# hsinnan75/GSAlign

Measured on AMD Instinct MI355X. Metric: aligned query Gbp/s (whole node), higher is better.
Workload: dtype u8; 1 GPU; full-human-sized pair (BASELINE configs[4]): 24 contigs with GRCh38 chromosome lengths, 3.08 Gbp, repeat injection, vs 1; inflight_contexts_per_gpu=8, world_size=1, parallelism=one GPU

## Files before the change

gsalign_amd/csrc/gsa_api.hip:

```cpp
#include <algorithm>
#include <atomic>
#include <chrono>
#include <cstring>
#include <mutex>
#include <thread>
#include <pthread.h>
#include <sched.h>
#include "gsa_ctx.h"

static thread_local std::string g_create_error;

int gsa_fail(gsa_ctx *ctx, int code, const std::string &msg)
{
	if (ctx) ctx->err = msg; else g_create_error = msg;
	return code;
}

int host_stage4_5_6(gsa_ctx *c, int stage);
int host_stage8_finish(gsa_ctx *c);
int build_block_view(gsa_ctx *c);
void bundle_split_lists(gsa_ctx *c);
void bundle_join_lists(gsa_ctx *c);

void collect_events(gsa_ctx *c)
{
	if (!c->profiling && !c->prof_seed) { c->ev_pending = 0; return; }
	float ms;
	if ((c->ev_pending & 1) && !c->profiling) { if (hipEventElapsedTime(&ms, c->ev[0], c->ev[1]) == hipSuccess) { c->kernel_ms[0] = ms; c->acc_seed_ms += ms; } c->ev_pending = 0; (void)hipGetLastError(); return; }
	if (c->ev_pending & 1) {
		if (hipEventElapsedTime(&ms, c->ev[0], c->ev[1]) == hipSuccess) c->kernel_ms[0] = ms;
		if (hipEventElapsedTime(&ms, c->ev[1], c->ev[2]) == hipSuccess) c->kernel_ms[1] = ms;
		if (hipEventElapsedTime(&ms, c->ev[2], c->ev[3]) == hipSuccess) c->kernel_ms[2] = ms;
	}
	if (c->ev_pending & 2) { if (hipEventElapsedTime(&ms, c->ev[4], c->ev[5]) == hipSuccess) c->kernel_ms[3] = ms; }
	c->ev_pending = 0;
	(void)hipGetLastError();
}

void Uploader::run()
{
	(void)hipSetDevice(device);
	for (;;) {
		Job j;
		{ std::unique_lock<std::mutex> g(mu); cv.wait(g, [&] { return stop || !q.empty(); }); if (q.empty()) return; j = std::move(q.front()); q.pop_front(); if (n_demand > 0) n_demand--; }
		const auto t0 = std::chrono::steady_clock::now();
		hipError_t e_first = hipSuccess;
		for (const Piece &p : j.pieces) if (p.n) { const hipError_t e = hipMemcpyAsync(p.dst, p.src, p.n, hipMemcpyHostToDevice, st); if (e != hipSuccess && e_first == hipSuccess) e_first = e; bytes += p.n; }
		{ const hipError_t e = hipStreamSynchronize(st); if (e != hipSuccess && e_first == hipSuccess) e_first = e; }
		(void)hipGetLastError();
		if (e_first != hipSuccess && j.err) { int none = 0; j.err->compare_exchange_strong(none, (int)e_first); }
		const auto t1 = std::chrono::steady_clock::now();
		{ std::lock_guard<std::mutex> g(mu); copy_ms += std::chrono::duration<double, std::milli>(t1 - t0).count(); wait_ms += std::chrono::duration<double, std::milli>(t0 - j.t_push).count(); jobs++; }
		j.busy->fetch_sub(1, std::memory_order_release);
	}
}

static int uploader_start(gsa_ctx *c)
{
	Uploader *u = new Uploader(); u->device = c->device;
	if (hipStreamCreateWithFlags(&u->st, hipStreamNonBlocking) != hipSuccess) { delete u; return gsa_fail(c, GSA_ERR_HIP, "hipStreamCreate (upload stream)"); }
	u->th = std::thread([u] { u->run(); });
	c->up = u; c->own_up = true;
	return GSA_OK;
}

static void uploader_stop(gsa_ctx *c)
{
	if (!c->up || !c->own_up) { c->up = nullptr; return; }
	Uploader *u = c->up;
	{ std::lock_guard<std::mutex> g(u->mu); u->stop = true; }
	u->cv.notify_all();
	if (u->th.joinable()) u->th.join();
#ifdef GSA_EXPERIMENTS
	if (getenv("GSA_UP_STATS") && u->jobs) fprintf(stderr, "[uploader] %lld jobs, %.1f MB each, %.2f ms in the queue, %.2f ms copying (%.1f GB/s)\n", (long long)u->jobs, u->bytes / 1e6 / u->jobs, u->wait_ms / u->jobs, u->copy_ms / u->jobs, u->bytes / 1e6 / u->copy_ms);
#endif
	if (u->st) hipStreamDestroy(u->st);
	delete u; c->up = nullptr;
}

static inline void slot_wait(QuerySlot &s) { while (s.busy.load(std::memory_order_acquire) > 0) std::this_thread::yield(); }
static void slot_demand(gsa_ctx *c, QuerySlot &s)
{
	if (s.busy.load(std::memory_order_acquire) > 0 && c->up) {
		Uploader *u = c->up;
		std::lock_guard<std::mutex> g(u->mu);
		for (size_t k = u->n_demand; k < u->q.size(); k++) if (u->q[k].busy == &s.busy) {
			Uploader::Job j = std::move(u->q[k]); u->q.erase(u->q.begin() + (long)k); u->q.insert(u->q.begin() + (long)u->n_demand, std::move(j)); u->n_demand++;
			break;
		}
	}
	slot_wait(s);
}

static int ctx_private_init(gsa_ctx *c, gsa_ctx *share = nullptr)
{
#ifdef GSA_EXPERIMENTS
	static const int prio = [] { const char *e = getenv("GSA_STREAM_PRIO"); return e ? atoi(e) : 0; }();
	if (prio) {
		int lo = 0, hi = 0; GSA_CHECK(c, hipDeviceGetStreamPriorityRange(&lo, &hi));
		GSA_CHECK(c, hipStreamCreateWithPriority(&c->stream, hipStreamDefault, hi));
		for (int i = 0; i < 4; i++) GSA_CHECK(c, hipStreamCreateWithPriority(&c->stream_aux[i], hipStreamDefault, (i == 0 || i == 3 || (prio > 1 && i == 1)) ? lo : hi));
	} else
#endif
	if (c->prio_mode > 0) {
		int lo = 0, hi = 0; GSA_CHECK(c, hipDeviceGetStreamPriorityRange(&lo, &hi));
		const int mid = (lo + hi) / 2;
		GSA_CHECK(c, hipStreamCreateWithPriority(&c->stream, hipStreamDefault, hi));
		GSA_CHECK(c, hipStreamCreateWithPriority(&c->stream_seed, hipStreamDefault, c->prio_mode == 2 ? lo : mid));
		GSA_CHECK(c, hipEventCreateWithFlags(&c->ev_seed_fork, hipEventDisableTiming));
		for (int i = 0; i < 4; i++) GSA_CHECK(c, hipStreamCreateWithPriority(&c->stream_aux[i], hipStreamDefault, (c->prio_mode == 3 && (i == 0 || i == 3)) ? lo : mid));
	} else {
	GSA_CHECK(c, hipStreamCreate(&c->stream));
	for (int i = 0; i < 4; i++) GSA_CHECK(c, hipStreamCreate(&c->stream_aux[i]));
	}
	if (share) { c->up = share->up; c->own_up = false; } else if (int rc = uploader_start(c)) return rc;
	for (int i = 0; i < 28; i++) GSA_CHECK(c, hipEventCreate(&c->ev[i]));
	GSA_CHECK(c, hipMalloc(&c->d_zero.p, 256)); c->d_zero.cap = 256; GSA_CHECK(c, hipMemset(c->d_zero.p, 0, 256));
	GSA_CHECK(c, hipMalloc(&c->d_cnt.p, 32 * sizeof(u64))); c->d_cnt.cap = 32 * sizeof(u64); GSA_CHECK(c, hipMemset(c->d_cnt.p, 0, 32 * sizeof(u64)));
	GSA_CHECK(c, hipHostMalloc((void **)&c->h_cnt, 16 * sizeof(u64)));
	GSA_CHECK(c, hipMalloc(&c->d_mail.p, MAIL_N * sizeof(i32))); c->d_mail.cap = MAIL_N * sizeof(i32);
	GSA_CHECK(c, hipMemset(c->d_mail.p, 0, MAIL_N * sizeof(i32)));
	GSA_CHECK(c, hipHostMalloc((void **)&c->h_mail, MAIL_N * sizeof(i32)));
	return GSA_OK;
}

static hipError_t h2d_big(void *dst, const void *src, size_t bytes)
{
	if (bytes >= ((size_t)64 << 20) && hipHostRegister(const_cast<void *>(src), bytes, hipHostRegisterDefault) == hipSuccess) {
		const hipError_t e = hipMemcpy(dst, src, bytes, hipMemcpyHostToDevice);
		(void)hipHostUnregister(const_cast<void *>(src));
		return e;
	}
	(void)hipGetLastError();
	return hipMemcpy(dst, src, bytes, hipMemcpyHostToDevice);
}

struct ReservedBuf { void *p = nullptr; size_t bytes = 0; };
static std::mutex g_res_mu; static ReservedBuf g_res[64][2];
void *dev_take_reserved(int device, size_t bytes, size_t *got)
{
	std::lock_guard<std::mutex> g(g_res_mu);
	for (int k = 0; k < 2; k++) { ReservedBuf &r = g_res[device & 63][k]; if (r.p && r.bytes >= bytes && r.bytes <= bytes + bytes / 8 + 4096) { void *p = r.p; *got = r.bytes; r.p = nullptr; r.bytes = 0; return p; } }
	return nullptr;
}

extern "C" {

void gsa_default_params(gsa_params *p)
{
	p->min_seed_len = 15; p->max_indel = 25; p->min_block_score = 200; p->min_aln_len = 200; p->min_identity = 70;
	p->sensitive = 0; p->one_on_one = 0;
}

const char *gsa_last_error(gsa_ctx *ctx) { return ctx ? ctx->err.c_str() : g_create_error.c_str(); }

static int reset_run_state(gsa_ctx *c)
{
	if (c->early_in_flight) { GSA_CHECK(c, hipStreamSynchronize(c->stream_aux[0])); c->early_in_flight = false; }
	c->n_early = 0; c->early_listed = false; c->early_consumed = false;
	c->stage = 0; c->split = false; c->b_lists.clear();
	c->n_seeds = 0; c->n_groups = 0; c->n_blocks2 = 0; c->blocks.clear(); c->frags_stage = 0; c->have_host_seeds = false; c->ev_pending = 0; c->s2_host = false;
	memset(c->counters, 0, sizeof(c->counters)); memset(c->kernel_ms, 0, sizeof(c->kernel_ms));
	return GSA_OK;
}

int gsa_set_params(gsa_ctx *c, const gsa_params *p)
{
	if (!c || !p) return GSA_ERR_ARG;
	if (p->min_seed_len < 1 || p->max_indel < 0) return gsa_fail(c, GSA_ERR_ARG, "bad parameter");
	GSA_CHECK(c, hipSetDevice(c->device));
	if (c->n_borrowers.load() > 0 && (p->sensitive ? 10 : p->min_seed_len) != c->prm.MinSeedLength)
		return gsa_fail(c, GSA_ERR_STATE, "gsa_set_params: contexts cloned from this one read its seed tables -- change -slen / -sen on the clones, or destroy them first");
	if (int rc = reset_run_state(c)) return rc;
	c->prm.MinSeedLength = p->sensitive ? 10 : p->min_seed_len;
	c->prm.MaxIndelSize = p->max_indel; c->prm.MinAlnBlockScore = p->min_block_score; c->prm.MinAlnLength = p->min_aln_len;
	c->prm.MinSeqIdy = p->min_identity; c->prm.bSensitive = p->sensitive ? 1 : 0; c->prm.OneOnOne = p->one_on_one ? 1 : 0;
	return build_presence(c);
}

int gsa_create(int device, const gsa_index_view *idx, const gsa_params *prm, gsa_ctx **out)
{
	return gsa_create_opts(device, idx, prm, 0u, out);
}

int gsa_create_opts(int device, const gsa_index_view *idx, const gsa_params *prm, uint32_t flags, gsa_ctx **out)
{
	if (!idx || !out || !idx->bwt || !idx->sa || !idx->ref || !idx->chr_len || idx->n_chr <= 0 || idx->G <= 0) return gsa_fail(nullptr, GSA_ERR_ARG, "gsa_create: bad index view");
	if (idx->L2[4] != (uint64_t)(2 * idx->G)) return gsa_fail(nullptr, GSA_ERR_ARG, "gsa_create: L2[4] != 2G");
	int ndev = 0;
	if (hipGetDeviceCount(&ndev) != hipSuccess || ndev <= 0) return gsa_fail(nullptr, GSA_ERR_HIP, "no HIP device available (libgsa_hip.so has no CPU path)");
	if (device < 0 || device >= ndev) return gsa_fail(nullptr, GSA_ERR_ARG, "gsa_create: bad device ordinal");
	if (flags & ~(uint32_t)(GSA_CREATE_WIDE | GSA_CREATE_KMER_K(15) | GSA_CREATE_PRIO(3) | GSA_CREATE_REF_PAC)) return gsa_fail(nullptr, GSA_ERR_ARG, "gsa_create_opts: unknown flag");
	{ const uint32_t kk = (flags >> 8) & 15u; if (kk == 1) return gsa_fail(nullptr, GSA_ERR_ARG, "gsa_create_opts: GSA_CREATE_KMER_K takes 2 .. 15 (0: chosen by text length and free memory)"); }
	gsa_ctx *c = new gsa_ctx();
	c->device = device; c->force_wide = (flags & GSA_CREATE_WIDE) != 0; c->opt.kmer_k = (int)((flags >> 8) & 15u); c->prio_mode = (int)((flags >> 16) & 3u);
	memset(c->kernel_ms, 0, sizeof(c->kernel_ms)); memset(c->counters, 0, sizeof(c->counters));
#define CK(call) do { hipError_t e_ = (call); if (e_ != hipSuccess) { gsa_fail(nullptr, GSA_ERR_HIP, std::string(#call) + ": " + hipGetErrorString(e_)); gsa_destroy(c); return GSA_ERR_HIP; } } while (0)
	CK(hipSetDevice(device));
	(void)hipSetDeviceFlags(hipDeviceScheduleSpin);
	(void)hipGetLastError();
	if (int rcp = ctx_private_init(c)) { g_create_error = c->err; gsa_destroy(c); return rcp; }
	const size_t bwt_bytes = ((idx->bwt_words + 15) / 16) * 64;
	CK(hipMalloc(&c->d_bwt_ref.p, bwt_bytes + 64)); c->d_bwt_ref.cap = bwt_bytes + 64;
	CK(hipMemset(c->d_bwt_ref.p, 0, bwt_bytes + 64));
	CK(h2d_big(c->d_bwt_ref.p, idx->bwt, idx->bwt_words * 4));
	CK(hipMalloc(&c->d_sa.p, idx->n_sa * 8)); c->d_sa.cap = idx->n_sa * 8;
	CK(h2d_big(c->d_sa.p, idx->sa, idx->n_sa * 8));
	CK(hipMalloc(&c->d_ref.p, (size_t)2 * idx->G + 64)); c->d_ref.cap = (size_t)2 * idx->G + 64;
	if (flags & GSA_CREATE_REF_PAC) {
		const size_t pac_bytes = ((size_t)idx->G + 3) / 4;
		void *d_pac = nullptr;
		CK(hipMalloc(&d_pac, pac_bytes + 64));
		if (h2d_big(d_pac, idx->ref, pac_bytes) != hipSuccess) { hipFree(d_pac); gsa_fail(nullptr, GSA_ERR_HIP, "hipMemcpy (.pac)"); gsa_destroy(c); return GSA_ERR_HIP; }
		const int rcu = unpack_pac(c, (const uint8_t *)d_pac, idx->G, (uint8_t *)c->d_ref.p);
		(void)hipStreamSynchronize(c->stream); hipFree(d_pac);
		if (rcu) { g_create_error = c->err; gsa_destroy(c); return rcu; }
	} else
	CK(h2d_big(c->d_ref.p, idx->ref, (size_t)2 * idx->G));
	c->G = idx->G;
	{
		i64 tot = 0; std::vector<std::pair<i64, i32> > ends;
		for (int i = 0; i < idx->n_chr; i++) {
			c->h_chr_len.push_back(idx->chr_len[i]); c->h_chr_fwd.push_back(tot); tot += idx->chr_len[i];
			ends.push_back(std::make_pair(c->h_chr_fwd[i] + idx->chr_len[i] - 1, i));
			ends.push_back(std::make_pair(2 * idx->G - tot + idx->chr_len[i] - 1, i));
		}
		if (tot != idx->G) { gsa_fail(nullptr, GSA_ERR_ARG, "gsa_create: sum(chr_len) != G"); gsa_destroy(c); return GSA_ERR_ARG; }
		std::sort(ends.begin(), ends.end());
		for (size_t i = 0; i < ends.size(); i++) { c->h_chr_end.push_back(ends[i].first); c->h_chr_of_end.push_back(ends[i].second); }
	}
	c->d_chr_end.cap = c->h_chr_end.size() * 8; c->d_chr_of_end.cap = c->h_chr_of_end.size() * 4;
	CK(hipMalloc(&c->d_chr_end.p, c->h_chr_end.size() * 8)); CK(hipMemcpy(c->d_chr_end.p, c->h_chr_end.data(), c->h_chr_end.size() * 8, hipMemcpyHostToDevice));
	CK(hipMalloc(&c->d_chr_of_end.p, c->h_chr_of_end.size() * 4)); CK(hipMemcpy(c->d_chr_of_end.p, c->h_chr_of_end.data(), c->h_chr_of_end.size() * 4, hipMemcpyHostToDevice));
#undef CK
	c->di.primary = idx->primary; for (int i = 0; i < 5; i++) c->di.L2[i] = idx->L2[i]; c->di.L2[0] = 0;
	c->di.seq_len = idx->L2[4];
	c->di.bwt = nullptr; c->di.occ_base = nullptr; c->di.occ_shift = 0; c->di.sa = c->d_sa.as<u64>(); c->di.ref = c->d_ref.as<uint8_t>(); c->di.G = idx->G;
	c->di.chr_end = c->d_chr_end.as<i64>(); c->di.chr_of_end = c->d_chr_of_end.as<i32>(); c->di.n_ends = (i32)c->h_chr_end.size();
	c->di.sa32 = nullptr; c->di.sa64 = nullptr; c->di.kmer = nullptr; c->di.kmer_k = 0; c->di.kmer_lo = nullptr; c->di.kmer_lo_k = 0; c->di.kmer_e16 = 0; c->di.ref2 = nullptr; c->di.pres = nullptr; c->di.pres_k = 0;
	{
		const int rco = build_occ(c, c->d_bwt_ref.p, bwt_bytes / 64);
		hipFree(c->d_bwt_ref.p); c->d_bwt_ref.p = nullptr; c->d_bwt_ref.cap = 0;
		if (rco) { g_create_error = c->err; gsa_destroy(c); return rco; }
	}
	if (int rcd = build_dense_sa(c, idx->n_sa)) { g_create_error = c->err; gsa_destroy(c); return rcd; }
	gsa_params dp; gsa_default_params(&dp);
	int rc = gsa_set_params(c, prm ? prm : &dp);
	if (rc) { g_create_error = c->err; gsa_destroy(c); return rc; }
	gsa_release_reserved(device);
	if (const unsigned long long ov = gsa_take_grid_overflow()) { gsa_fail(nullptr, GSA_ERR_LIMIT, "gsa_create: a table build needed a launch of " + std::to_string(ov) + " work-items (>= 2^32)"); gsa_destroy(c); return GSA_ERR_LIMIT; }
	*out = c;
	return GSA_OK;
}

#define GSA_DEVBUFS(X) X(d_bwt) X(d_bwt_ref) X(d_occ_base) X(d_sa) X(d_ref) X(d_chr_end) X(d_chr_of_end) X(qs[0].d_query) X(qs[1].d_query) X(qs[0].d_bndtab) X(qs[1].d_bndtab) X(tmp) X(d_cnt) X(d_zero) X(d_mail) X(d_lb_status[0]) X(d_lb_status[1]) X(d_sa_dense) X(d_kmer) X(d_kmer_lo) X(d_pres) X(d_ref2) X(d_cand_s) X(d_cand_len) X(d_cand_x0) X(d_cand_freq) X(d_onpath) X(d_cand_cnt) X(d_heavy) X(dn_lf) X(dn_x0) X(d_chunk_hits) X(d_chunk_base) X(d_key_a) X(d_key_b) X(d_val_a) X(d_val_b) X(s_q) X(s_len) X(s_r) X(s_gid) X(d_flag) X(d_scan) X(g_beg) X(w_j0) X(d_pdbm) X(d_pdby) X(d_pdcb) X(d_gpre) X(d_key_c) X(d_val_c) X(a_q) X(a_len) X(a_r) X(a_gb) X(a_ge) X(a_uniq) X(a_cu) X(a_alive) X(a_ws) X(a_wid) X(a_next) X(a_brk) X(a_aurank) X(a_aulist) X(a_runinfo) X(w_best) X(w_sum) X(w_n) X(d_btab) X(d_flag2) X(d_scan2) X(d_i64a) X(b_q) X(b_len) X(b_r) X(b_gb) X(b_ge) X(c_q) X(c_len) X(c_r) X(c_gb) X(c_ge) X(c_bid) X(blk_beg) X(blk_end) X(blk_score) X(r_q) X(r_len) X(r_r) X(r_bid) X(r_tmp_q) X(r_tmp_len) X(r_tmp_r) X(r_tmp_bid) X(r_cut4) X(r_cut5) X(r_simjob) X(r_simres) X(d_leaf) X(fb_seedbase) X(fb_sbeg) X(fb_fragbase) X(f_rec) X(f_rec16) X(f_type) X(f_mism) X(f_alnlen) X(f_job) X(f_score) X(d_dp_tiny) X(d_dp_bnd) X(d_dp_ctr) X(d_dp_jobs) X(d_dp_large) X(d_tail) X(e_id) X(e_rec) X(e_list) X(e_off1) X(e_off2) X(e_opsoff) X(e_nops) X(e_ops) X(e_rev) X(r_head) X(f_early) X(r_orig) X(r_tmp_orig) X(j_frag) X(j_opsoff) X(j_nops) X(d_ops) X(j_cells) X(d_alnoff) X(bl_alnlen) X(bl_score) X(d_bblk) X(d_dp_arena) X(leaf[0]) X(leaf[1]) X(leaf[2]) X(leaf[3]) X(leaf[4]) X(leaf[5]) X(leaf[6]) X(leaf[7]) X(leaf[8])
void gsa_destroy(gsa_ctx *c)
{
	if (!c) return;
	hipSetDevice(c->device);
	if (c->stream) hipStreamSynchronize(c->stream);
	for (int i = 0; i < 2; i++) slot_wait(c->qs[i]);
	uploader_stop(c);
	if (c->lender) c->lender->n_borrowers.fetch_sub(1);
#define X(n) &c->n,
	DevBuf *bufs[] = { GSA_DEVBUFS(X) };
#undef X
	for (DevBuf *b : bufs) if (b->p) hipFree(b->p);
	if (c->h_cnt) hipHostFree(c->h_cnt);
	if (c->h_mail) hipHostFree(c->h_mail);
	for (DevBuf *b : { &c->p_frags, &c->p_tail, &c->p_leaf, &c->p_blk, &c->p_dp, &c->p_sj, &c->p_sj_early, &c->p_jpatch, &c->p_early, &c->qs[0].p_bndtab, &c->qs[1].p_bndtab, &c->p_bblk, &c->p_ba0 }) if (b->p) hipHostFree(b->p);
	for (int i = 0; i < 28; i++) if (c->ev[i]) hipEventDestroy(c->ev[i]);
	for (int i = 0; i < 4; i++) if (c->stream_aux[i]) hipStreamDestroy(c->stream_aux[i]);
	if (c->stream_seed) hipStreamDestroy(c->stream_seed);
	if (c->ev_seed_fork) hipEventDestroy(c->ev_seed_fork);
	if (c->stream) hipStreamDestroy(c->stream);
	delete c;
}

int gsa_clone(gsa_ctx *parent, gsa_ctx **out)
{
	if (!parent || !out) return GSA_ERR_ARG;
	if (hipSetDevice(parent->device) != hipSuccess) return gsa_fail(nullptr, GSA_ERR_HIP, "hipSetDevice");
	gsa_ctx *c = new gsa_ctx();
	c->device = parent->device; c->force_wide = parent->force_wide; c->prio_mode = parent->prio_mode;
	c->index_owner = parent->index_owner ? parent->index_owner : parent; c->seed_budget = parent->seed_budget; c->opt = parent->opt;
	memset(c->kernel_ms, 0, sizeof(c->kernel_ms)); memset(c->counters, 0, sizeof(c->counters));
	if (int rc = ctx_private_init(c, c->index_owner)) { g_create_error = c->err; gsa_destroy(c); return rc; }
	c->di = parent->di; c->G = parent->G;
	c->lender = parent; parent->n_borrowers.fetch_add(1);
	c->h_chr_end = parent->h_chr_end; c->h_chr_fwd = parent->h_chr_fwd; c->h_chr_of_end = parent->h_chr_of_end; c->h_chr_len = parent->h_chr_len;
	c->prm = parent->prm;
	*out = c;
	return GSA_OK;
}

int gsa_clone_to_device(gsa_ctx *parent, int device, gsa_ctx **out)
{
	if (!parent || !out) return GSA_ERR_ARG;
	int ndev = 0;
	if (hipGetDeviceCount(&ndev) != hipSuccess || device < 0 || device >= ndev) { (void)hipGetLastError(); return gsa_fail(nullptr, GSA_ERR_ARG, "gsa_clone_to_device: bad device ordinal"); }
	gsa_ctx *own = parent->index_owner ? parent->index_owner : parent;
	if (hipSetDevice(parent->device) != hipSuccess) return gsa_fail(nullptr, GSA_ERR_HIP, "hipSetDevice");
	if (hipStreamSynchronize(parent->stream) != hipSuccess || hipStreamSynchronize(own->stream) != hipSuccess) return gsa_fail(nullptr, GSA_ERR_HIP, "gsa_clone_to_device: the parent's stream");
	if (hipSetDevice(device) != hipSuccess) return gsa_fail(nullptr, GSA_ERR_HIP, "hipSetDevice");
	(void)hipSetDeviceFlags(hipDeviceScheduleSpin); (void)hipGetLastError();
	gsa_ctx *c = new gsa_ctx();
	c->device = device; c->force_wide = parent->force_wide; c->prio_mode = parent->prio_mode; c->seed_budget = parent->seed_budget; c->opt = parent->opt;
	memset(c->kernel_ms, 0, sizeof(c->kernel_ms)); memset(c->counters, 0, sizeof(c->counters));
	if (int rc = ctx_private_init(c)) { g_create_error = c->err; gsa_destroy(c); return rc; }
	struct Pair { const DevBuf *src; DevBuf *dst; };
	std::vector<Pair> tab = { { &own->d_bwt, &c->d_bwt }, { &own->d_occ_base, &c->d_occ_base }, { &own->d_sa, &c->d_sa }, { &own->d_ref, &c->d_ref }, { &own->d_chr_end, &c->d_chr_end },
		{ &own->d_chr_of_end, &c->d_chr_of_end }, { &own->d_sa_dense, &c->d_sa_dense }, { &own->d_kmer, &c->d_kmer }, { &own->d_ref2, &c->d_ref2 } };
	for (gsa_ctx *src = parent; src; src = src->lender) {
		if (!c->d_pres.cap && src->d_pres.p && (const void *)parent->di.pres == src->d_pres.p) { tab.push_back({ &src->d_pres, &c->d_pres }); c->d_pres.cap = 1; }
		if (!c->d_kmer_lo.cap && src->d_kmer_lo.p && (const void *)parent->di.kmer_lo == src->d_kmer_lo.p) { tab.push_back({ &src->d_kmer_lo, &c->d_kmer_lo }); c->d_kmer_lo.cap = 1; }
	}
	c->d_pres.cap = c->d_kmer_lo.cap = 0;
	auto fail = [&](int code, const std::string &m) { gsa_fail(nullptr, code, m); gsa_destroy(c); return code; };
	for (const Pair &t : tab) {
		if (!t.src->p) continue;
		const size_t bytes = t.src->len ? t.src->len : t.src->cap;
		if (bytes == 0) return fail(GSA_ERR_STATE, "gsa_clone_to_device: an index table of unknown size");
		if (hipMalloc(&t.dst->p, bytes + 256) != hipSuccess) { (void)hipGetLastError(); return fail(GSA_ERR_NOMEM, "gsa_clone_to_device: hipMalloc of an index table"); }
		t.dst->cap = bytes + 256; t.dst->len = bytes;
		const hipError_t e = (device == own->device) ? hipMemcpyAsync(t.dst->p, t.src->p, bytes, hipMemcpyDeviceToDevice, c->stream)
		                                             : hipMemcpyPeerAsync(t.dst->p, device, t.src->p, own->device, bytes, c->stream);
		if (e != hipSuccess) return fail(GSA_ERR_HIP, std::string("gsa_clone_to_device: device-to-device copy: ") + hipGetErrorString(e));
	}
	c->di = parent->di;
	auto move_ptr = [&](const void *p) -> const void * {
		if (!p) return nullptr;
		for (const Pair &t : tab) if (t.src->p && (const char *)p >= (const char *)t.src->p && (const char *)p < (const char *)t.src->p + (t.src->len ? t.src->len : t.src->cap)) return (const char *)t.dst->p + ((const char *)p - (const char *)t.src->p);
		return (const void *)~(uintptr_t)0;
	};
	bool lost = false;
#define MOVE(field, T) do { const void *q_ = move_ptr((const void *)c->di.field); if (q_ == (const void *)~(uintptr_t)0) lost = true; c->di.field = (T)q_; } while (0)
	MOVE(bwt, const uint4 *); MOVE(occ_base, const u64 *); MOVE(sa, const u64 *); MOVE(sa32, const u32 *); MOVE(sa64, const u64 *); MOVE(ref, const uint8_t *); MOVE(ref2, const u32 *);
	MOVE(chr_end, const i64 *); MOVE(chr_of_end, const i32 *); MOVE(kmer, const u64 *); MOVE(kmer_lo, const u64 *); MOVE(pres, const u32 *);
#undef MOVE
	if (lost) return fail(GSA_ERR_STATE, "gsa_clone_to_device: an index pointer outside the tables of its owner");
	c->G = parent->G;
	c->h_chr_end = parent->h_chr_end; c->h_chr_fwd = parent->h_chr_fwd; c->h_chr_of_end = parent->h_chr_of_end; c->h_chr_len = parent->h_chr_len;
	c->prm = parent->prm;
	if (hipStreamSynchronize(c->stream) != hipSuccess) return fail(GSA_ERR_HIP, "gsa_clone_to_device: waiting for the copies");
	*out = c;
	return GSA_OK;
}

static bool device_local_cpus(int device, cpu_set_t *set)
{
	char bus[64] = { 0 };
	if (hipDeviceGetPCIBusId(bus, (int)sizeof(bus) - 1, device) != hipSuccess) { (void)hipGetLastError(); return false; }
	for (char *p = bus; *p; p++) if (*p >= 'A' && *p <= 'Z') *p = (char)(*p - 'A' + 'a');
	char path[160]; snprintf(path, sizeof(path), "/sys/bus/pci/devices/%s/local_cpulist", bus);
	FILE *f = fopen(path, "r"); if (!f) return false;
	char line[4096]; const bool got = fgets(line, sizeof(line), f) != nullptr; fclose(f);
	if (!got) return false;
	CPU_ZERO(set); int n = 0;
	for (char *p = line; *p;) {
		while (*p == ',' || *p == ' ' || *p == '\n') p++;
		if (!*p) break;
		char *e; long a = strtol(p, &e, 10), b = a; if (e == p) break;
		if (*e == '-') { p = e + 1; b = strtol(p, &e, 10); if (e == p) break; }
		for (long k = a; k <= b && k < CPU_SETSIZE; k++) { CPU_SET((int)k, set); n++; }
		p = e;
	}
	return n > 0;
}
int gsa_reserve_index(int device, uint64_t seq_len, uint32_t flags)
{
	int ndev = 0;
	if (hipGetDeviceCount(&ndev) != hipSuccess || device < 0 || device >= ndev || seq_len == 0) { (void)hipGetLastError(); return GSA_ERR_ARG; }
	if (hipSetDevice(device) != hipSuccess) return GSA_ERR_HIP;
	const bool wide = (flags & GSA_CREATE_WIDE) != 0 || seq_len >= 0xFFFFFFF0ull;
	size_t want[2];
	want[0] = ((size_t)seq_len + 1 + 32) * (wide ? 8 : 4) + 256;
	{
		int k = 0; while ((1ull << (2 * k)) < seq_len) k++;
		k += 2; if (k > 15) k = 15;
		size_t fr = 0, tot = 0; if (hipMemGetInfo(&fr, &tot) != hipSuccess) { (void)hipGetLastError(); fr = 8ull << 30; }
		const size_t esz = wide ? 32 : 16;
		while (k > 2 && ((size_t)esz << (2 * k)) > fr / 4) k--;
		const int kk = (int)((flags >> 8) & 15u); if (kk >= 2 && kk <= 15 && ((size_t)esz << (2 * kk)) <= fr / 2) k = kk;
		want[1] = k >= 2 ? ((size_t)esz << (2 * k)) : 0;
	}
	gsa_release_reserved(device);
	for (int k = 0; k < 2; k++) {
		if (!want[k]) continue;
		void *p = nullptr;
		if (hipMalloc(&p, want[k]) != hipSuccess) { (void)hipGetLastError(); continue; }
		std::lock_guard<std::mutex> g(g_res_mu);
		g_res[device & 63][k].p = p; g_res[device & 63][k].bytes = want[k];
	}
	return GSA_OK;
}
void gsa_release_reserved(int device)
{
	void *f[2] = { nullptr, nullptr };
	{ std::lock_guard<std::mutex> g(g_res_mu); for (int k = 0; k < 2; k++) { f[k] = g_res[device & 63][k].p; g_res[device & 63][k].p = nullptr; g_res[device & 63][k].bytes = 0; } }
	if (f[0] || f[1]) { (void)hipSetDevice(device); for (int k = 0; k < 2; k++) if (f[k]) hipFree(f[k]); }
}

int gsa_bind_host_thread(int device)
{
	cpu_set_t set;
	if (!device_local_cpus(device, &set)) return GSA_OK;
	(void)pthread_setaffinity_np(pthread_self(), sizeof(set), &set);
	return GSA_OK;
}

void *gsa_host_alloc(size_t bytes)
{
	void *p = nullptr;
	if (hipHostMalloc(&p, bytes ? bytes : 1) != hipSuccess) { (void)hipGetLastError(); return nullptr; }
	return p;
}
void gsa_host_free(void *p) { if (p) (void)hipHostFree(p); }
int gsa_host_register(void *p, size_t bytes)
{
	if (!p || !bytes) return GSA_ERR_ARG;
	if (hipHostRegister(p, bytes, hipHostRegisterDefault) != hipSuccess) { (void)hipGetLastError(); return GSA_ERR_HIP; }
	return GSA_OK;
}
int gsa_host_unregister(void *p)
{
	if (!p) return GSA_ERR_ARG;
	if (hipHostUnregister(p) != hipSuccess) { (void)hipGetLastError(); return GSA_ERR_HIP; }
	return GSA_OK;
}

int gsa_set_option(gsa_ctx *c, const char *name, int64_t value)
{
	if (!c || !name) return GSA_ERR_ARG;
	const std::string k(name);
	auto in = [&](int64_t lo, int64_t hi) { return value >= lo && value <= hi; };
	const int64_t BIG = (int64_t)1 << 40;
	if (k == "split_min") { if (!in(0, BIG)) return gsa_fail(c, GSA_ERR_ARG, "split_min: 0 .. 2^40 bases"); c->opt.split_min = value; }
	else if (k == "bundle_contig") { if (!in(0, BIG)) return gsa_fail(c, GSA_ERR_ARG, "bundle_contig: 0 (no bundles) .. 2^40 bases"); c->opt.bundle_contig = value; }
	else if (k == "bundle_cap") { if (!in(1, BIG)) return gsa_fail(c, GSA_ERR_ARG, "bundle_cap: 1 .. 2^40 bases"); c->opt.bundle_cap = value; }
	else if (k == "seed_budget") { if (!in(1, 0xffffffffll)) return gsa_fail(c, GSA_ERR_ARG, "seed_budget: 1 .. 2^32 - 1 wave-iterations"); c->seed_budget = (u32)value; }
	else if (k == "dp_lane") { if (!in(0, 1 << 20)) return gsa_fail(c, GSA_ERR_ARG, "dp_lane: 0 (round 2's tiny / small split) .. 2^20 cells"); c->opt.dp_lane = (int)value; }
	else if (k == "seed_mode") { if (value < 0 || value > 2) return gsa_fail(c, GSA_ERR_ARG, "seed_mode: 0 sweep, 1 speculative, 2 search"); c->opt.seed_mode = (int)value; }
	else if (k == "pd_bitmap") c->opt.pd_bitmap = value != 0;
	else if (k == "dp_side") c->opt.dp_side = value != 0;
	else if (k == "dp_small_side") c->opt.dp_small_side = value != 0;
	else if (k == "pd_two_level_min") { if (!in(0, BIG)) return gsa_fail(c, GSA_ERR_ARG, "pd_two_level_min: >= 0 blocks"); c->opt.pd_two_level_min = value; }
	else if (k == "dp_occupancy") { if (!in(0, 16)) return gsa_fail(c, GSA_ERR_ARG, "dp_occupancy: 0 (off) .. 16 workgroups per CU"); c->opt.dp_occupancy = (int)value; }
	else if (k == "pd_bytes") { if (!in(0, 2)) return gsa_fail(c, GSA_ERR_ARG, "pd_bytes: 0 never, 1 by the hit count, 2 always"); c->opt.pd_bytes = (int)value; }
	else if (k == "pres_from_kmer") c->opt.pres_from_kmer = value != 0;
	else if (k == "walk_chain_min") { if (!in(0, BIG)) return gsa_fail(c, GSA_ERR_ARG, "walk_chain_min: >= 0 seeds"); c->opt.walk_chain_min = value; }
	else if (k == "sweep_shape") { if (value < -1 || value > 1) return gsa_fail(c, GSA_ERR_ARG, "sweep_shape: -1, 0 or 1"); c->opt.sweep_shape = (int)value; }
	else if (k == "dp_safe") c->dp_safe = value != 0;
	else if (k == "dp_fake_timeout") { if (!in(0, 1 << 20)) return gsa_fail(c, GSA_ERR_ARG, "dp_fake_timeout: >= 0"); c->dp_fake_timeout = (int)value; }
	else return gsa_fail(c, GSA_ERR_ARG, "gsa_set_option: unknown option " + k);
	return GSA_OK;
}

int gsa_get_wall_sums(gsa_ctx *c, double ms[10], int64_t *n)
{
	if (!c || !ms || !n) return GSA_ERR_ARG;
	memcpy(ms, c->wall_ms, sizeof(c->wall_ms)); *n = c->wall_n;
	if (c->up && c->own_up) { std::lock_guard<std::mutex> g(c->up->mu); ms[9] = c->up->jobs ? c->up->copy_ms / (double)c->up->jobs * (double)c->wall_n : 0.0; }
	return GSA_OK;
}

int gsa_get_alloc_stats(gsa_ctx *c, double *ms, int64_t *n, int64_t *bytes)
{
	if (!c) return GSA_ERR_ARG;
	if (ms) *ms = c->alloc_ms; if (n) *n = c->alloc_n; if (bytes) *bytes = c->alloc_bytes;
	return GSA_OK;
}
int gsa_debug_buffers(gsa_ctx *c, int top)
{
	if (!c) return GSA_ERR_ARG;
	struct E { const char *name; size_t cap, len; };
	std::vector<E> v;
#define X(n) if (c->n.p) v.push_back({ #n, c->n.cap, c->n.len });
	GSA_DEVBUFS(X)
#undef X
	std::sort(v.begin(), v.end(), [](const E &a, const E &b) { return a.cap > b.cap; });
	size_t tot = 0; for (const E &e : v) tot += e.cap;
	fprintf(stderr, "[gsa_debug_buffers] %zu device buffers, %.2f GB held\n", v.size(), (double)tot / 1e9);
	for (size_t k = 0; k < v.size() && (int)k < top; k++) fprintf(stderr, "  %-16s %10.1f MB held  %10.1f MB asked\n", v[k].name, (double)v[k].cap / 1e6, (double)v[k].len / 1e6);
	return GSA_OK;
}
int gsa_set_profiling(gsa_ctx *c, int enable) { if (!c) return GSA_ERR_ARG; c->acc_seed_ms = 0.0; memset(c->wall_ms, 0, sizeof(c->wall_ms)); c->wall_n = 0; if (c->up && c->own_up) { std::lock_guard<std::mutex> g(c->up->mu); c->up->copy_ms = c->up->wait_ms = c->up->bytes = 0; c->up->jobs = 0; } c->profiling = (enable & 1) != 0; c->count_blocks = (enable & 2) != 0; c->prof_seed = (enable & 4) != 0; return GSA_OK; }

static int query_geometry(gsa_ctx *c, int32_t qlen)
{
	c->qlen = qlen;
	c->bnd.n = 0; c->bnd.lmax = qlen; c->bnd.pds = 0; c->bnd.off = (const i32 *)c->d_zero.p; c->bnd.chunk_contig = (const uint16_t *)c->d_zero.p;
	c->qbits = ceil_log2_u64((u64)qlen + 1); if (c->qbits < 1) c->qbits = 1;
	c->pd_span = 2 * c->G + (i64)qlen + 2;
	c->pdbits = ceil_log2_u64((u64)c->pd_span);
	if (c->qbits + c->pdbits > 64) return gsa_fail(c, GSA_ERR_LIMIT, "contig too long for the 64-bit seed key");
	return GSA_OK;
}

#define GSA_BUNDLE_MAX_CONTIGS 4096
static void *slot_ensure_bytes(gsa_ctx *c, DevBuf &b, size_t bytes, bool pinned)
{
	if (bytes && bytes <= b.cap) return b.p;
	return pinned ? (void *)pin_ensure<uint8_t>(c, b, bytes) : (void *)dev_ensure<uint8_t>(c, b, bytes);
}

static int slot_layout(gsa_ctx *c, QuerySlot &s, const char *const *query, const int32_t *qlen, int32_t n)
{
	s.b_off.assign((size_t)n + 1, 0); s.b_qlen.assign(qlen, qlen + n); s.src.assign(query, query + n);
	i64 tot = 0; i32 lmax = 0;
	for (int k = 0; k < n; k++) {
		if (qlen[k] < 0 || (qlen[k] > 0 && !query[k])) return GSA_ERR_ARG;
		s.b_off[(size_t)k] = (i32)tot;
		tot += ((i64)qlen[k] + GSA_CHUNK - 1) / GSA_CHUNK * GSA_CHUNK;
		if (tot >= (1ll << 31) - 2 * GSA_CHUNK) return gsa_fail(c, GSA_ERR_LIMIT, "bundle longer than 2^31 bases");
		if (qlen[k] > lmax) lmax = qlen[k];
	}
	s.b_off[(size_t)n] = (i32)tot; s.tot = tot; s.lmax = lmax; s.n = n;
	return GSA_OK;
}

__global__ void __launch_bounds__(256) k_bundle_pad(const i32 *__restrict__ off, const i32 *__restrict__ len, uint8_t *dst)
{
	const i32 k = blockIdx.x; const i64 b = (i64)off[k] + len[k], e = off[k + 1];
	for (i64 t = b + threadIdx.x; t < e; t += 256) dst[t] = (uint8_t)'N';
}

static int slot_upload(gsa_ctx *c, QuerySlot &s, const char *const *query, const int32_t *qlen, int32_t n)
{
	slot_wait(s);
	s.up_err.store(0);
	Uploader::Job job; job.busy = &s.busy; job.err = &s.up_err;
	if (n == 0) {
		s.n = 0; s.tot = qlen[0]; s.lmax = qlen[0]; s.src.assign(1, query[0]); s.b_qlen.assign(1, qlen[0]); s.b_off.clear();
		if (!slot_ensure_bytes(c, s.d_query, (size_t)qlen[0] + 64, false)) return GSA_ERR_NOMEM;
		size_t nb = (size_t)qlen[0];
#ifdef GSA_EXPERIMENTS
		{ static const long long cap = [] { const char *e = getenv("GSA_X_UPBYTES"); return e ? atoll(e) : -1ll; }(); if (cap >= 0 && (size_t)cap < nb) nb = (size_t)cap; }
#endif
		if (nb > 0) { job.pieces.push_back({ s.d_query.p, query[0], nb }); c->up->push(std::move(job)); }
		return GSA_OK;
	}
	if (int rc = slot_layout(c, s, query, qlen, n)) return rc;
	const i64 n_chunks = s.tot / GSA_CHUNK;
	s.o_cc = ((size_t)n + 1) * 4; s.o_src = (s.o_cc + (size_t)n_chunks * 2 + 15) & ~(size_t)15;
	const size_t t_bytes = s.o_src + (size_t)n * 4;
	if (!slot_ensure_bytes(c, s.p_bndtab, t_bytes + 16, true) || !slot_ensure_bytes(c, s.d_bndtab, t_bytes + 16, false) || !slot_ensure_bytes(c, s.d_query, (size_t)s.tot + 64, false)) return GSA_ERR_NOMEM;
	uint8_t *ht = s.p_bndtab.as<uint8_t>();
	memcpy(ht, s.b_off.data(), s.o_cc);
	{ uint16_t *cc = (uint16_t *)(ht + s.o_cc); for (int k = 0; k < n; k++) for (i64 ch = s.b_off[(size_t)k] / GSA_CHUNK; ch < s.b_off[(size_t)k + 1] / GSA_CHUNK; ch++) cc[ch] = (uint16_t)k; }
	memcpy(ht + s.o_src, qlen, (size_t)n * 4);
	job.pieces.push_back({ s.d_bndtab.p, ht, t_bytes });
	for (int k = 0; k < n; k++) if (qlen[k] > 0) job.pieces.push_back({ s.d_query.as<uint8_t>() + s.b_off[(size_t)k], query[k], (size_t)qlen[k] });
	c->up->push(std::move(job));
	return GSA_OK;
}

static int slot_finish(gsa_ctx *c, QuerySlot &s)
{
	slot_demand(c, s);
	if (const int e = s.up_err.exchange(0)) return gsa_fail(c, GSA_ERR_HIP, std::string("query upload (hipMemcpyAsync H2D): ") + hipGetErrorString((hipError_t)e));
	if (s.n > 0 && s.tot > 0) {
		const uint8_t *dt = s.d_bndtab.as<uint8_t>();
		hipLaunchKernelGGL(k_bundle_pad, dim3((unsigned)s.n), dim3(256), 0, c->stream, (const i32 *)dt, (const i32 *)(dt + s.o_src), s.d_query.as<uint8_t>());
		GSA_CHECK(c, hipGetLastError());
	}
	return GSA_OK;
}

static bool slot_holds(const QuerySlot &s, const char *const *query, const int32_t *qlen, int32_t n)
{
	if (!s.pending || s.n != n) return false;
	const int32_t m = n ? n : 1;
	if ((int32_t)s.src.size() != m || (int32_t)s.b_qlen.size() != m) return false;
	for (int32_t k = 0; k < m; k++) if (s.src[(size_t)k] != query[k] || s.b_qlen[(size_t)k] != qlen[k]) return false;
	return true;
}

static int slot_acquire(gsa_ctx *c, const char *const *query, const int32_t *qlen, int32_t n, int *which)
{
	for (int i = 0; i < 2; i++) if (slot_holds(c->qs[i], query, qlen, n)) {
		c->qs[i].pending = false; *which = i;
		return slot_finish(c, c->qs[i]);
	}
	int i = (c->q_cur == 1 && !c->qs[1].pending) ? 1 : 0;
	if (c->qs[i].pending) i ^= 1;
	if (c->qs[i].pending) return gsa_fail(c, GSA_ERR_STATE, "both query slots hold prefetched contigs: align them (or gsa_cancel_prefetch) first");
	*which = i;
	if (int rc = slot_upload(c, c->qs[i], query, qlen, n)) return rc;
	return slot_finish(c, c->qs[i]);
}

static int prefetch(gsa_ctx *c, const char *const *query, const int32_t *qlen, int32_t n)
{
	GSA_CHECK(c, hipSetDevice(c->device));
	int i = c->q_cur == 0 ? 1 : 0;
	if (c->qs[i].pending) i ^= 1;
	if (c->qs[i].pending) return gsa_fail(c, GSA_ERR_STATE, "gsa_prefetch: two contigs are waiting already");
	if (i == c->q_cur && c->stage > 0 && c->stage < 8) return gsa_fail(c, GSA_ERR_STATE, "gsa_prefetch: the free query slot holds the contig whose stages are still running (finish it with gsa_run_to(8) or gsa_set_query first)");
	if (i == c->q_cur) c->q_cur = -2;
	int rc = slot_upload(c, c->qs[i], query, qlen, n);
	if (rc == GSA_OK) c->qs[i].pending = true;
	return rc;
}

int gsa_prefetch_contig(gsa_ctx *c, const char *query, int32_t qlen)
{
	if (!c || !query || qlen < 0) return GSA_ERR_ARG;
	return prefetch(c, &query, &qlen, 0);
}

int gsa_prefetch_bundle(gsa_ctx *c, const char *const *query, const int32_t *qlen, int32_t n)
{
	if (!c || !query || !qlen) return GSA_ERR_ARG;
	if (n < 1 || n > GSA_BUNDLE_MAX_CONTIGS) return gsa_fail(c, GSA_ERR_ARG, "gsa_prefetch_bundle: 1 .. 4096 contigs");
	return prefetch(c, query, qlen, n);
}

int gsa_cancel_prefetch(gsa_ctx *c)
{
	if (!c) return GSA_ERR_ARG;
	if (!c->qs[0].pending && !c->qs[1].pending) return GSA_OK;
	c->qs[0].pending = c->qs[1].pending = false;
	return GSA_OK;
}

int gsa_set_query(gsa_ctx *c, const char *query, int32_t qlen)
{
	if (!c || !query || qlen < 0) return GSA_ERR_ARG;
	GSA_CHECK(c, hipSetDevice(c->device));
	if (int rc = reset_run_state(c)) return rc;
	int w = 0;
	const auto t0 = std::chrono::steady_clock::now();
	if (int rc = slot_acquire(c, &query, &qlen, 0, &w)) return rc;
	c->wall_ms[0] += std::chrono::duration<double, std::milli>(std::chrono::steady_clock::now() - t0).count();
	c->q_cur = w; c->q_dev = c->qs[w].d_query.as<uint8_t>();
	return query_geometry(c, qlen);
}

int gsa_set_query_device(gsa_ctx *c, const char *d_query, int32_t qlen)
{
	if (!c || !d_query || qlen < 0) return GSA_ERR_ARG;
	if (((uintptr_t)d_query & 15) != 0) return gsa_fail(c, GSA_ERR_ARG, "gsa_set_query_device: the buffer must be 16-byte aligned");
	GSA_CHECK(c, hipSetDevice(c->device));
	hipPointerAttribute_t at;
	if (hipPointerGetAttributes(&at, d_query) != hipSuccess || at.type != hipMemoryTypeDevice || at.device != c->device) { (void)hipGetLastError(); return gsa_fail(c, GSA_ERR_ARG, "gsa_set_query_device: not a device buffer of this context's GPU"); }
	if (int rc = reset_run_state(c)) return rc;
	c->q_dev = (const uint8_t *)d_query; c->q_cur = -1;
	return query_geometry(c, qlen);
}

void *gsa_device_alloc(int device, size_t bytes)
{
	void *p = nullptr;
	if (hipSetDevice(device) != hipSuccess || hipMalloc(&p, (bytes ? bytes : 1) + 64) != hipSuccess) { (void)hipGetLastError(); return nullptr; }
	return p;
}
void gsa_device_free(int device, void *p) { if (p && hipSetDevice(device) == hipSuccess) (void)hipFree(p); }
int gsa_device_upload(int device, void *dst, const void *src, size_t bytes)
{
	if (!dst || (!src && bytes)) return GSA_ERR_ARG;
	if (hipSetDevice(device) != hipSuccess || hipMemcpy(dst, src, bytes, hipMemcpyHostToDevice) != hipSuccess) { (void)hipGetLastError(); return GSA_ERR_HIP; }
	return GSA_OK;
}

static int rewind_to_hits(gsa_ctx *c)
{
	const i64 n_seeds = c->n_seeds; const i32 n_groups = c->n_groups;
	if (int rc = reset_run_state(c)) return rc;
	GSA_CHECK(c, hipStreamSynchronize(c->stream));
	c->n_seeds = n_seeds; c->n_groups = n_groups; c->counters[2] = c->counters[3] = (u64)n_seeds;
	c->stage = 1;
	return stage1_restore_pdbm(c);
}

int gsa_rewind(gsa_ctx *c)
{
	if (!c) return GSA_ERR_ARG;
	if (c->qlen <= 0) return gsa_fail(c, GSA_ERR_STATE, "gsa_set_query first");
	if (c->q_cur == -2) return gsa_fail(c, GSA_ERR_STATE, "gsa_rewind: the contig's device copy was overwritten by a prefetch");
	GSA_CHECK(c, hipSetDevice(c->device));
	return reset_run_state(c);
}

int gsa_run_to(gsa_ctx *c, int stage)
{
	if (!c || stage < 0 || stage > 8) return GSA_ERR_ARG;
	if (c->bnd.n && stage < 8 && !c->bundle_call) return gsa_fail(c, GSA_ERR_STATE, "gsa_run_to: the context holds a bundle (gsa_align_bundle runs it); gsa_set_query first");
	if (c->split) return gsa_fail(c, GSA_ERR_STATE, "gsa_run_to: a split contig is finished with gsa_finish_contig");
	GSA_CHECK(c, hipSetDevice(c->device));
	int rc = GSA_OK;
	auto t_prev = std::chrono::steady_clock::now();
	while (c->stage < stage && rc == GSA_OK) {
		const int next = c->stage + 1;
		switch (next) {
		case 1: rc = stage1_seed(c); break;
		case 2: rc = stage2_chain(c); break;
		case 3: rc = stage345_refine(c); if (rc == GSA_OK && c->bnd.n) bundle_split_lists(c); break;
		case 4: case 5: case 6: rc = host_stage4_5_6(c, next); break;
		case 7: if (c->bnd.n) bundle_join_lists(c); rc = stage7_fill(c); break;
		case 8: rc = stage78_extend(c); if (rc == GSA_OK) rc = host_stage8_finish(c); break;
		}
		if (rc == GSA_OK) { c->stage = next; c->frags_stage = (next == 8) ? 8 : 0; }
		{ const auto t_now = std::chrono::steady_clock::now(); c->wall_ms[next] += std::chrono::duration<double, std::milli>(t_now - t_prev).count(); t_prev = t_now; }
	}
	if (stage == 8) c->wall_n++;
	if (const unsigned long long ov = gsa_take_grid_overflow()) rc = gsa_fail(c, GSA_ERR_LIMIT, "a kernel launch of " + std::to_string(ov) + " work-items (>= 2^32) was needed: contig too large for this build");
	if (rc == GSA_OK) { GSA_CHECK(c, hipStreamSynchronize(c->stream)); collect_events(c); }
	if (c->early_in_flight && (rc != GSA_OK || !c->early_consumed)) GSA_CHECK(c, hipStreamSynchronize(c->stream_aux[0]));
	return rc;
}

static int align_uploaded(gsa_ctx *c, gsa_result *out);
int gsa_align_contig(gsa_ctx *c, const char *query, int32_t qlen, gsa_result *out)
{
	if (!c || !out) return GSA_ERR_ARG;
	int rc = gsa_set_query(c, query, qlen); if (rc) return rc;
	return align_uploaded(c, out);
}
int gsa_align_contig_device(gsa_ctx *c, const char *d_query, int32_t qlen, gsa_result *out)
{
	if (!c || !out) return GSA_ERR_ARG;
	int rc = gsa_set_query_device(c, d_query, qlen); if (rc) return rc;
	return align_uploaded(c, out);
}
static int align_uploaded(gsa_ctx *c, gsa_result *out)
{
	int rc;
	c->dp_timeout = false;
	rc = gsa_run_to(c, 8);
	if (rc == GSA_ERR_STATE && c->dp_timeout && !c->dp_safe) {
		c->dp_timeout = false; c->dp_safe = true;
		rc = gsa_rewind(c);
		if (rc == GSA_OK) rc = gsa_run_to(c, 8);
		c->dp_safe = false;
	}
	if (rc) return rc;
	return gsa_get_blocks(c, out);
}

struct BundleSrc { const uint8_t *p; i32 len, _pad; };
__global__ void __launch_bounds__(256) k_bundle_gather(const i32 *__restrict__ off, const uint16_t *__restrict__ chunk_contig, const BundleSrc *__restrict__ src, uint8_t *dst)
{
	const i32 chunk = blockIdx.x, ci = chunk_contig[chunk];
	const i64 g0 = (i64)chunk * GSA_CHUNK; const i32 l0 = (i32)(g0 - off[ci]);
	const BundleSrc sc = src[ci];
	const i32 have = sc.len - l0 < GSA_CHUNK ? sc.len - l0 : GSA_CHUNK;
	for (i32 t = threadIdx.x; t < GSA_CHUNK; t += 256) dst[g0 + t] = t < have ? sc.p[l0 + t] : (uint8_t)'N';
}

static int set_query_bundle(gsa_ctx *c, const char *const *query, const int32_t *qlen, int32_t n, bool dev_q)
{
	if (n < 1 || n > GSA_BUNDLE_MAX_CONTIGS) return gsa_fail(c, GSA_ERR_ARG, "gsa_align_bundle: 1 .. 4096 contigs");
	GSA_CHECK(c, hipSetDevice(c->device));
	if (int rc = reset_run_state(c)) return rc;
	int w = 0;
	if (!dev_q) { if (int rc = slot_acquire(c, query, qlen, n, &w)) return rc; }
	else {
		w = (c->q_cur == 1 && !c->qs[1].pending) ? 1 : 0;
		if (c->qs[w].pending) w ^= 1;
		if (c->qs[w].pending) return gsa_fail(c, GSA_ERR_STATE, "both query slots hold prefetched contigs");
		QuerySlot &s = c->qs[w];
		slot_wait(s);
		for (int k = 0; k < n; k++) if (qlen[k] > 0) {
			hipPointerAttribute_t at;
			if (!query[k] || hipPointerGetAttributes(&at, query[k]) != hipSuccess || at.type != hipMemoryTypeDevice || at.device != c->device) { (void)hipGetLastError(); return gsa_fail(c, GSA_ERR_ARG, "gsa_align_bundle (GSA_MANY_DEVICE): not a device buffer of this context's GPU"); }
		}
		if (int rc = slot_layout(c, s, query, qlen, n)) return rc;
		const i64 n_chunks = s.tot / GSA_CHUNK;
		s.o_cc = ((size_t)n + 1) * 4; s.o_src = (s.o_cc + (size_t)n_chunks * 2 + 15) & ~(size_t)15;
		const size_t t_bytes = s.o_src + (size_t)n * sizeof(BundleSrc);
		if (!slot_ensure_bytes(c, s.p_bndtab, t_bytes + 16, true) || !slot_ensure_bytes(c, s.d_bndtab, t_bytes + 16, false) || !slot_ensure_bytes(c, s.d_query, (size_t)s.tot + 64, false)) return GSA_ERR_NOMEM;
		uint8_t *ht = s.p_bndtab.as<uint8_t>();
		memcpy(ht, s.b_off.data(), s.o_cc);
		{ uint16_t *cc = (uint16_t *)(ht + s.o_cc); for (int k = 0; k < n; k++) for (i64 ch = s.b_off[(size_t)k] / GSA_CHUNK; ch < s.b_off[(size_t)k + 1] / GSA_CHUNK; ch++) cc[ch] = (uint16_t)k; }
		{ BundleSrc *bs = (BundleSrc *)(ht + s.o_src); for (int k = 0; k < n; k++) { bs[k].p = (const uint8_t *)query[k]; bs[k].len = qlen[k]; bs[k]._pad = 0; } }
		GSA_CHECK(c, hipMemcpyAsync(s.d_bndtab.p, ht, t_bytes, hipMemcpyHostToDevice, c->stream));
		const uint8_t *dt = s.d_bndtab.as<uint8_t>();
		if (s.tot > 0) {
			hipLaunchKernelGGL(k_bundle_gather, dim3((unsigned)n_chunks), dim3(256), 0, c->stream, (const i32 *)dt, (const uint16_t *)(dt + s.o_cc), (const BundleSrc *)(dt + s.o_src), s.d_query.as<uint8_t>());
			GSA_CHECK(c, hipGetLastError());
		}
	}
	const QuerySlot &s = c->qs[w];
	c->q_cur = w; c->b_off = s.b_off; c->b_qlen = s.b_qlen;
	const uint8_t *dt = s.d_bndtab.as<uint8_t>();
	c->q_dev = s.d_query.as<uint8_t>();
	c->qlen = (i32)s.tot;
	c->bnd.n = n; c->bnd.lmax = s.lmax; c->bnd.off = (const i32 *)dt; c->bnd.chunk_contig = (const uint16_t *)(dt + s.o_cc);
	c->bnd.pds = (2 * c->G + (i64)s.lmax + (i64)c->prm.MaxIndelSize + 64 + 31) & ~31ll;
	c->qbits = ceil_log2_u64((u64)s.tot + 1); if (c->qbits < 1) c->qbits = 1;
	c->pd_span = (i64)n * c->bnd.pds + 2;
	c->pdbits = ceil_log2_u64((u64)c->pd_span);
	if (c->qbits + c->pdbits > 64) return gsa_fail(c, GSA_ERR_LIMIT, "bundle too long for the 64-bit seed key");
	return GSA_OK;
}

static void bundle_result(gsa_ctx *c, int k, const std::vector<i64> &a0, size_t blk_at, gsa_result *out)
{
	out->n_blocks = c->b_nblk[(size_t)k]; out->blocks = c->h_blocks.data() + blk_at;
	out->n_frags = c->b_frag0[(size_t)k + 1] - c->b_frag0[(size_t)k]; out->recs = c->p_frags.as<gsa_rec>() + c->b_frag0[(size_t)k];
	out->n_aln = a0[(size_t)k + 1] - a0[(size_t)k]; out->aln1 = c->h_taln1 + a0[(size_t)k]; out->aln2 = c->h_taln2 + a0[(size_t)k];
}

int gsa_align_bundle(gsa_ctx *c, const char *const *query, const int32_t *qlen, int32_t n, uint32_t flags, gsa_result *out)
{
	if (!c || !query || !qlen || !out || (flags & ~(uint32_t)GSA_MANY_DEVICE)) return GSA_ERR_ARG;
	int rc = set_query_bundle(c, query, qlen, n, (flags & GSA_MANY_DEVICE) != 0); if (rc) return rc;
	c->dp_timeout = false;
	c->bundle_call = true;
	struct Clear { gsa_ctx *c; ~Clear() { c->bundle_call = false; } } clear_{ c };
	rc = gsa_run_to(c, 8);
	if (rc == GSA_ERR_STATE && c->dp_timeout && !c->dp_safe) {
		c->dp_timeout = false; c->dp_safe = true;
		{ const Bundle keep = c->bnd; rc = reset_run_state(c); c->bnd = keep; }
		if (rc == GSA_OK) rc = gsa_run_to(c, 8);
		c->dp_safe = false;
	}
	if (rc) return rc;
	const size_t nfb = c->b_blk0.empty() ? 0 : (size_t)c->b_blk0[(size_t)n];
	if (nfb == 0 || c->n_frags == 0) {
		for (int k = 0; k < n; k++) { out[k].n_blocks = 0; out[k].n_frags = 0; out[k].n_aln = 0; out[k].blocks = nullptr; out[k].recs = nullptr; out[k].aln1 = out[k].aln2 = nullptr; }
		return GSA_OK;
	}
	std::vector<i64> a0((size_t)n + 1, c->n_aln);
	for (int k = n - 1; k >= 0; k--) a0[(size_t)k] = c->b_blk0[(size_t)k] < c->b_blk0[(size_t)k + 1] ? c->p_ba0.as<i64>()[k] : a0[(size_t)k + 1];
	size_t at = 0;
	for (int k = 0; k < n; k++) { bundle_result(c, k, a0, at, &out[k]); at += (size_t)c->b_nblk[(size_t)k]; }
	return GSA_OK;
}

int gsa_seed_chunks(gsa_ctx *c, const char *query, int32_t qlen, int32_t chunk_beg, int32_t chunk_end)
{
	if (!c || chunk_beg < 0 || chunk_end < chunk_beg) return GSA_ERR_ARG;
	int rc = gsa_set_query(c, query, qlen); if (rc) return rc;
	c->split = true; c->rng_beg = chunk_beg; c->rng_end = chunk_end;
	rc = stage1_seed(c);
	if (rc == GSA_OK) GSA_CHECK(c, hipStreamSynchronize(c->stream));
	collect_events(c);
	return rc;
}

int64_t gsa_hit_count(gsa_ctx *c) { return (c && c->split) ? c->n_seeds : 0; }

int gsa_export_hits(gsa_ctx *c, uint64_t *keys, uint32_t *vals)
{
	if (!c || !c->split) return c ? gsa_fail(c, GSA_ERR_STATE, "gsa_seed_chunks first") : GSA_ERR_ARG;
	if (c->n_seeds == 0) return GSA_OK;
	if (!keys || !vals) return GSA_ERR_ARG;
	GSA_CHECK(c, hipSetDevice(c->device));
	GSA_CHECK(c, hipMemcpyAsync(keys, c->d_key_a.p, (size_t)c->n_seeds * 8, hipMemcpyDefault, c->stream));
	GSA_CHECK(c, hipMemcpyAsync(vals, c->d_val_a.p, (size_t)c->n_seeds * 4, hipMemcpyDefault, c->stream));
	GSA_CHECK(c, hipStreamSynchronize(c->stream));
	return GSA_OK;
}

int gsa_import_hits(gsa_ctx *c, const uint64_t *keys, const uint32_t *vals, int64_t n)
{
	if (!c || n < 0 || (n > 0 && (!keys || !vals))) return GSA_ERR_ARG;
	if (!c->split || c->stage != 0) return gsa_fail(c, GSA_ERR_STATE, "gsa_seed_chunks first");
	GSA_CHECK(c, hipSetDevice(c->device));
	return stage1_import_hits(c, (const u64 *)keys, (const u32 *)vals, n);
}

int gsa_finish_contig(gsa_ctx *c, gsa_result *out)
{
	if (!c || !out) return GSA_ERR_ARG;
	if (!c->split || c->stage != 0) return gsa_fail(c, GSA_ERR_STATE, "gsa_seed_chunks first");
	GSA_CHECK(c, hipSetDevice(c->device));
	int rc = stage1_finish_split(c); if (rc) return rc;
	c->stage = 1; c->split = false;
	c->dp_timeout = false;
	rc = gsa_run_to(c, 8);
	if (rc == GSA_ERR_STATE && c->dp_timeout && !c->dp_safe) {
		c->dp_timeout = false; c->dp_safe = true;
		rc = rewind_to_hits(c);
		if (rc == GSA_OK) rc = gsa_run_to(c, 8);
		c->dp_safe = false;
	}
	if (rc) return rc;
	return gsa_get_blocks(c, out);
}

int gsa_hit_buffers(gsa_ctx *c, const uint64_t **keys, const uint32_t **vals)
{
	if (!c || !keys || !vals) return GSA_ERR_ARG;
	if (!c->split) return gsa_fail(c, GSA_ERR_STATE, "gsa_seed_chunks first");
	*keys = c->d_key_a.as<uint64_t>(); *vals = c->d_val_a.as<uint32_t>();
	return GSA_OK;
}

static int align_split(gsa_ctx *const *grp, int n_grp, const char *query, int32_t qlen, gsa_result *out)
{
	const int32_t n_chunks = (int32_t)(((int64_t)qlen + GSA_CHUNK - 1) / GSA_CHUNK);
	std::vector<int> rcs((size_t)n_grp, GSA_OK);
	std::vector<std::thread> th;
	auto range = [&](int k, int32_t &b, int32_t &e) { const int32_t base = n_chunks / n_grp, extra = n_chunks % n_grp; b = k * base + (k < extra ? k : extra); e = b + base + (k < extra ? 1 : 0); };
	for (int k = 1; k < n_grp; k++) th.emplace_back([&, k] { int32_t b, e; range(k, b, e); rcs[(size_t)k] = gsa_seed_chunks(grp[k], query, qlen, b, e); });
	{ int32_t b, e; range(0, b, e); rcs[0] = gsa_seed_chunks(grp[0], query, qlen, b, e); }
	for (std::thread &t : th) t.join();
	for (int k = 0; k < n_grp; k++) if (rcs[(size_t)k] != GSA_OK) { if (k) gsa_fail(grp[0], rcs[(size_t)k], std::string("helper context: ") + gsa_last_error(grp[k])); return rcs[(size_t)k]; }
	for (int k = 1; k < n_grp; k++) {
		const uint64_t *kp = nullptr; const uint32_t *vp = nullptr;
		int rc = gsa_hit_buffers(grp[k], &kp, &vp);
		if (rc == GSA_OK) rc = gsa_import_hits(grp[0], kp, vp, gsa_hit_count(grp[k]));
		if (rc != GSA_OK) return rc;
	}
	return gsa_finish_contig(grp[0], out);
}

int gsa_align_many(gsa_ctx *const *ctx, int32_t n_ctx, const char *const *query, const int32_t *qlen, int32_t n, uint32_t flags, gsa_result_fn on_result, void *user)
{
	if (flags & ~(uint32_t)(GSA_MANY_IN_ORDER | GSA_MANY_DEVICE | GSA_MANY_NO_SPLIT | GSA_MANY_NO_BUNDLE | GSA_MANY_NO_PREFETCH)) return GSA_ERR_ARG;
	if (!ctx || n_ctx <= 0 || n < 0 || (n > 0 && (!query || !qlen))) return GSA_ERR_ARG;
	for (int k = 0; k < n_ctx; k++) if (!ctx[k]) return GSA_ERR_ARG;
	const bool dev_q = (flags & GSA_MANY_DEVICE) != 0;
	if (dev_q) for (int k = 1; k < n_ctx; k++) if (ctx[k]->device != ctx[0]->device) return gsa_fail(ctx[0], GSA_ERR_ARG, "GSA_MANY_DEVICE: the contexts must share one GPU (the contigs live in its memory)");
	if (n == 0) return GSA_OK;
	std::vector<int32_t> order((size_t)n);
	for (int32_t i = 0; i < n; i++) order[(size_t)i] = i;
	if (!(flags & GSA_MANY_IN_ORDER)) std::stable_sort(order.begin(), order.end(), [&](int32_t a, int32_t b) { return qlen[a] > qlen[b]; });
	std::atomic<int> err(GSA_OK);
	const int64_t split_min = ctx[0]->opt.split_min;
	int64_t longest = 0; for (int32_t i = 0; i < n; i++) if (qlen[i] > longest) longest = qlen[i];
	if (n < n_ctx && !dev_q && !(flags & GSA_MANY_NO_SPLIT) && longest >= split_min) {
		std::vector<int> gsz((size_t)n, 1);
		for (int left = n_ctx - n; left > 0; left--) {
			int best = -1; double load = 0;
			for (int i = 0; i < n; i++) { const int32_t ci = order[(size_t)i]; if ((int64_t)qlen[ci] < split_min) continue; const double l = (double)qlen[ci] / gsz[(size_t)i]; if (l > load) { load = l; best = i; } }
			if (best < 0) break;
			gsz[(size_t)best]++;
		}
		std::vector<std::thread> th; int at = 0;
		for (int i = 0; i < n; i++) {
			const int32_t ci = order[(size_t)i]; gsa_ctx *const *grp = ctx + at; const int ng = gsz[(size_t)i]; at += ng;
			th.emplace_back([&, ci, grp, ng] {
				gsa_result res;
				int rc = ng > 1 ? align_split(grp, ng, query[ci], qlen[ci], &res) : gsa_align_contig(grp[0], query[ci], qlen[ci], &res);
				if (rc == GSA_OK && on_result) rc = on_result(user, ci, &res);
				if (rc != GSA_OK) { int ok = GSA_OK; err.compare_exchange_strong(ok, rc); }
			});
		}
		for (std::thread &t : th) t.join();
		return err.load();
	}
	const int64_t bundle_contig = ctx[0]->opt.bundle_contig, bundle_cap = ctx[0]->opt.bundle_cap;
	std::vector<std::vector<int32_t> > units;
	{
		bool may = !(flags & GSA_MANY_NO_BUNDLE) && bundle_contig > 0;
		for (int k = 0; k < n_ctx; k++) if (ctx[k]->profiling || ctx[k]->count_blocks) may = false;
		int64_t small_total = 0; int32_t n_small = 0;
		for (int32_t i = 0; i < n; i++) if ((int64_t)qlen[i] <= bundle_contig) { small_total += qlen[i]; n_small++; }
		if (n_small < 2) may = false;
		size_t max_contigs = GSA_BUNDLE_MAX_CONTIGS;
		{
			const int qb = ceil_log2_u64((u64)(bundle_cap + bundle_cap / 8 + bundle_contig) + 1);
			const u64 stride = (u64)(2 * ctx[0]->G) + (u64)bundle_contig + (u64)ctx[0]->prm.MaxIndelSize + 96;
			const u64 fit = qb < 62 ? (1ull << (63 - qb)) / stride : 0;
			if (fit < max_contigs) max_contigs = (size_t)fit;
			if (max_contigs < 2) may = false;
		}
#ifdef GSA_EXPERIMENTS
		static const int64_t bundle_target = [] { const char *e = getenv("GSA_BUNDLE_TARGET"); return e ? (int64_t)atoll(e) : 0ll; }();
#else
		const int64_t bundle_target = 0;
#endif
		int64_t n_bundles = (small_total + bundle_cap - 1) / (bundle_cap > 0 ? bundle_cap : 1); if (n_bundles < 1) n_bundles = 1;
		n_bundles = (n_bundles + n_ctx - 1) / n_ctx * n_ctx;
		int64_t target = small_total / n_bundles + 1;
		if (bundle_target > 0) target = bundle_target;
		int64_t cur = 0;
		for (int32_t i = 0; i < n; i++) {
			const int32_t ci = order[(size_t)i];
			const bool small = may && (int64_t)qlen[ci] <= bundle_contig;
			if (!small) { units.push_back(std::vector<int32_t>(1, ci)); cur = 0; continue; }
			const int64_t padded = ((int64_t)qlen[ci] + GSA_CHUNK - 1) / GSA_CHUNK * GSA_CHUNK;
			if (cur > 0 && (cur + padded / 2 > target || cur + padded > bundle_cap + bundle_cap / 8 || units.back().size() >= max_contigs)) cur = 0;
			if (cur == 0) units.push_back(std::vector<int32_t>());
			units.back().push_back(ci); cur += padded > 0 ? padded : 1;
		}
	}
	const int32_t n_units = (int32_t)units.size();
	std::atomic<int32_t> next(0);
	auto one = [&](gsa_ctx *c, int32_t ci) {
		gsa_result res;
		int rc = dev_q ? gsa_align_contig_device(c, query[ci], qlen[ci], &res) : gsa_align_contig(c, query[ci], qlen[ci], &res);
		if (rc == GSA_OK && on_result) rc = on_result(user, ci, &res);
		return rc;
	};
	const bool pre = !dev_q && !(flags & GSA_MANY_NO_PREFETCH);
	auto loop = [&](gsa_ctx *c) {
		std::vector<const char *> bq, pq; std::vector<int32_t> bl, pl; std::vector<gsa_result> br;
		auto fetch = [&](int32_t u) {
			if (!pre || u >= n_units) return;
			const std::vector<int32_t> &un = units[(size_t)u];
			if (un.size() == 1) (void)gsa_prefetch_contig(c, query[un[0]], qlen[un[0]]);
			else { pq.clear(); pl.clear(); for (int32_t ci : un) { pq.push_back(query[ci]); pl.push_back(qlen[ci]); } (void)gsa_prefetch_bundle(c, pq.data(), pl.data(), (int32_t)un.size()); }
		};
		(void)gsa_cancel_prefetch(c);
		int32_t u = next.fetch_add(1);
		fetch(u);
		for (;;) {
			if (u >= n_units || err.load() != GSA_OK) { (void)gsa_cancel_prefetch(c); return; }
			const int32_t u_next = next.fetch_add(1);
			fetch(u_next);
			const std::vector<int32_t> &un = units[(size_t)u];
			int rc = GSA_OK;
			if (un.size() == 1) rc = one(c, un[0]);
			else {
				bq.clear(); bl.clear(); br.resize(un.size());
				for (int32_t ci : un) { bq.push_back(query[ci]); bl.push_back(qlen[ci]); }
				rc = gsa_align_bundle(c, bq.data(), bl.data(), (int32_t)un.size(), dev_q ? GSA_MANY_DEVICE : 0u, br.data());
				if (rc == GSA_OK) { for (size_t k = 0; k < un.size() && rc == GSA_OK && on_result; k++) rc = on_result(user, un[k], &br[k]); }
				else if (rc == GSA_ERR_LIMIT) { rc = GSA_OK; for (size_t k = 0; k < un.size() && rc == GSA_OK; k++) rc = one(c, un[k]); }
			}
			if (rc != GSA_OK) { int ok = GSA_OK; err.compare_exchange_strong(ok, rc); (void)gsa_cancel_prefetch(c); return; }
			u = u_next;
		}
	};
	std::vector<std::thread> th;
	for (int k = 1; k < n_ctx && k < n_units; k++) th.emplace_back(loop, ctx[k]);
	loop(ctx[0]);
	for (std::thread &t : th) t.join();
	return err.load();
}

int64_t gsa_seed_count(gsa_ctx *c) { return c ? c->n_seeds : 0; }

int gsa_get_seeds(gsa_ctx *c, gsa_seed *out)
{
	if (!c || (!out && c->n_seeds)) return GSA_ERR_ARG;
	if (c->stage < 1) return gsa_fail(c, GSA_ERR_STATE, "run stage 1 first");
	const size_t n = (size_t)c->n_seeds; if (!n) return GSA_OK;
	{ int rc = seed_view_sort(c); if (rc) return rc; GSA_CHECK(c, hipStreamSynchronize(c->stream)); }
	std::vector<i32> q(n), l(n); std::vector<i64> r(n);
	GSA_CHECK(c, hipMemcpy(q.data(), c->s_q.p, n * 4, hipMemcpyDeviceToHost));
	GSA_CHECK(c, hipMemcpy(l.data(), c->s_len.p, n * 4, hipMemcpyDeviceToHost));
	GSA_CHECK(c, hipMemcpy(r.data(), c->s_r.p, n * 8, hipMemcpyDeviceToHost));
	for (size_t i = 0; i < n; i++) { out[i].qpos = q[i]; out[i].len = l[i]; out[i].rpos = r[i]; }
	return GSA_OK;
}

int gsa_group_count(gsa_ctx *c)
{
	if (!c) return 0;
	if (c->n_groups < 0) {
		if (seed_view_sort(c) != GSA_OK) return 0;
		hipStreamSynchronize(c->stream);
		i32 ng = 0;
		if (hipMemcpy(&ng, c->d_mail.as<i32>() + M_NG, 4, hipMemcpyDeviceToHost) != hipSuccess) return 0;
		c->n_groups = ng;
	}
	return c->n_groups;
}

int gsa_get_groups(gsa_ctx *c, int32_t *beg, int32_t *end)
{
	if (!c) return GSA_ERR_ARG;
	if (c->stage < 1) return gsa_fail(c, GSA_ERR_STATE, "run stage 1 first");
	const size_t ng = (size_t)gsa_group_count(c); if (!ng) return GSA_OK;
	std::vector<i32> gb(ng + 1);
	GSA_CHECK(c, hipMemcpy(gb.data(), c->g_beg.p, (ng + 1) * 4, hipMemcpyDeviceToHost));
	for (size_t i = 0; i < ng; i++) { beg[i] = gb[i]; end[i] = gb[i + 1]; }
	return GSA_OK;
}

int gsa_get_blocks(gsa_ctx *c, gsa_result *out)
{
	if (!c || !out) return GSA_ERR_ARG;
	if (c->stage < 2) return gsa_fail(c, GSA_ERR_STATE, "run stage 2 first");
	if (c->bnd.n && c->stage < 8) return gsa_fail(c, GSA_ERR_STATE, "gsa_get_blocks: the context holds a bundle -- only its finished result (gsa_align_bundle's out[]) is defined per contig");
	if (c->frags_stage != c->stage) { int rc = build_block_view(c); if (rc) return rc; }
	out->n_blocks = (int32_t)c->h_blocks.size(); out->blocks = c->h_blocks.data();
	if (c->result_pinned && c->stage == 8) {
		out->n_frags = c->n_frags; out->n_aln = c->n_aln;
		out->recs = c->p_frags.as<gsa_rec>(); out->aln1 = c->h_taln1; out->aln2 = c->h_taln2;
	} else {
		out->n_frags = (int64_t)c->h_frags.size(); out->n_aln = (int64_t)c->h_aln1.size();
		out->recs = c->h_frags.data(); out->aln1 = c->h_aln1.data(); out->aln2 = c->h_aln2.data();
	}
	return GSA_OK;
}

int gsa_get_counters(gsa_ctx *c, uint64_t counters[8]) { if (!c) return GSA_ERR_ARG; memcpy(counters, c->counters, sizeof(c->counters)); return GSA_OK; }
int gsa_get_timings(gsa_ctx *c, float ms[8]) { if (!c) return GSA_ERR_ARG; memcpy(ms, c->kernel_ms, sizeof(c->kernel_ms)); if (c->prof_seed && !c->profiling) ms[6] = (float)c->acc_seed_ms; return GSA_OK; }
int gsa_get_seed_stats(gsa_ctx *c, uint64_t st[8]) { if (!c) return GSA_ERR_ARG; memcpy(st, c->dbg, sizeof(c->dbg)); return GSA_OK; }

}
```

gsalign_amd/csrc/gsa_ctx.h:

```cpp
#ifndef GSA_CTX_H
#define GSA_CTX_H
#include <atomic>
#include <chrono>
#include <condition_variable>
#include <deque>
#include <mutex>
#include <thread>
#include "gsa_internal.h"

struct Leaf {
	i32 beg, end;
	i32 sumlen;
	i32 q_first, q_last_end;
	i64 r_first, r_last_end;
	i32 blk;
	i32 cut4, cut5;
	i32 blk_score;
};

enum { M_NB = 0, M_NC = 1, M_NBLK = 2, M_NG = 3, M_NR = 4, M_NJ = 5, M_NL = 6, M_LBERR = 7, M_ANY = 8, M_NTINY = 40, M_TICKET = 48, M_NBRAW = 49, M_NR2 = 50, M_NF = 51, M_NJOB = 52, M_OPSTOT = 53, M_NALN = 54, M_DPERR = 64, M_NLARGE = 65, M_DPERR2 = 66, M_CELLS = 68  , M_DPERR3 = 41, M_LBDONE = 42, M_LFSTEPS = 44 , M_NEARLY = 62, M_EOPS = 63, M_NTOUCH = 46 , M_MAXBLK = 56 , MAIL_N = 72 };
#define LEAF_CHUNK 1024

struct HostBlock {
	i32 leaf_beg, leaf_end;
	i32 score;
	i32 bdup;
	i32 aln_len, bdir, gpos, chr;
};

struct QuerySlot {
	DevBuf d_query;
	DevBuf d_bndtab, p_bndtab;
	std::vector<i32> b_off, b_qlen;
	std::vector<const char *> src;
	i32 n = 0;
	i32 lmax = 0; i64 tot = 0; size_t o_cc = 0, o_src = 0;
	bool pending = false;
	std::atomic<int> busy{0};
	std::atomic<int> up_err{0};
};

struct Uploader {
	struct Piece { void *dst; const void *src; size_t n; };
	struct Job { std::vector<Piece> pieces; std::atomic<int> *busy; std::atomic<int> *err; std::chrono::steady_clock::time_point t_push; };
	double copy_ms = 0, wait_ms = 0, bytes = 0; long long jobs = 0;
	int device = 0; hipStream_t st = nullptr;
	std::thread th; std::mutex mu; std::condition_variable cv; std::deque<Job> q; bool stop = false;
	size_t n_demand = 0;
	void run();
	void push(Job &&j) { j.busy->fetch_add(1); j.t_push = std::chrono::steady_clock::now(); { std::lock_guard<std::mutex> g(mu); q.push_back(std::move(j)); } cv.notify_one(); }
};

struct Options {
	int64_t split_min = 20000000;
	int64_t bundle_contig = 16000000;
	int64_t bundle_cap = 64000000;
	int dp_lane = 512;
	int seed_mode = 1;
	int pd_bitmap = 1;
	int sweep_shape = -1;
	int dp_small_side = 0;
	int dp_side = 0;
	int64_t walk_chain_min = 100000;
	int64_t pd_two_level_min = 2000000;
	int dp_occupancy = 0;
	int pd_bytes = 1;
	int pres_from_kmer = 1;
	int kmer_k = 0;
};

struct gsa_ctx {
	int device = 0;
	Options opt;
	Uploader *up = nullptr; bool own_up = false;
	hipStream_t stream = nullptr;
	hipStream_t stream_seed = nullptr;
	hipEvent_t ev_seed_fork = nullptr;
	u64 seed_ticket = 0;
	int n_cus = 0;
	hipStream_t stream_aux[4] = {nullptr, nullptr, nullptr, nullptr};
	std::string err;
	Params prm;
	DevIndex di;
	gsa_ctx *index_owner = nullptr;
	gsa_ctx *lender = nullptr;
	std::atomic<int> n_borrowers{0};
	int prio_mode = 0;
	bool force_wide = false;
	bool profiling = false;
	bool prof_seed = false;
	bool count_blocks = false;
	u64 dbg[8] = {0, 0, 0, 0, 0, 0, 0, 0};
	hipEvent_t ev[28];
	float kernel_ms[8];
	double wall_ms[10] = {0, 0, 0, 0, 0, 0, 0, 0, 0, 0}; int64_t wall_n = 0;
	double acc_seed_ms = 0.0;
	u64 counters[8];

	DevBuf d_bwt, d_bwt_ref, d_occ_base, d_sa, d_ref, d_chr_end, d_chr_of_end;
	std::vector<i64> h_chr_end, h_chr_fwd; std::vector<i32> h_chr_of_end, h_chr_len;
	i64 G = 0;

	QuerySlot qs[2]; int q_cur = -1;
	i32 qlen = 0; int stage = 0;
	const uint8_t *q_dev = nullptr;
	bool split = false; i64 rng_beg = 0, rng_end = 0;
	int qbits = 1, pdbits = 1;
	i64 pd_span = 0;

	Bundle bnd = { 0, 0, 0, nullptr, nullptr }; bool bundle_call = false;
	std::vector<i32> b_off, b_qlen;
	std::vector<std::vector<HostBlock> > b_lists;
	std::vector<i32> b_blk0;
	DevBuf d_bblk, p_bblk, p_ba0;
	std::vector<i32> b_nblk; std::vector<i64> b_frag0;

	DevBuf tmp;
	DevBuf leaf[9];
	DevBuf d_cnt; u64 *h_cnt = nullptr;
	DevBuf d_mail; i32 *h_mail = nullptr;
	DevBuf d_lb_status[2]; u32 lb_epoch = 0, lb_base = 0;
	DevBuf p_leaf;
	int ev_pending = 0;
	bool s2_host = false;

	DevBuf d_ref2;
	DevBuf d_kmer;
	DevBuf d_kmer_lo;
	DevBuf d_pres;
	DevBuf d_sa_dense;
	DevBuf d_cand_s, d_cand_len, d_cand_x0, d_cand_freq, d_onpath, d_cand_cnt;
	size_t cand_cap_per_chunk = 1536;
	DevBuf d_heavy, dn_lf, dn_x0;
	bool seed_sweep_next = false, seed_sweep_probe = false; int seed_sweep_run = 0, seed_sweep_period = 8;
	u32 seed_budget = 256;
	DevBuf d_chunk_hits, d_chunk_base;
	DevBuf d_key_a, d_key_b, d_val_a, d_val_b;
	i64 n_seeds = 0; bool hits_sorted = false;
	DevBuf s_q, s_len, s_r, s_gid;
	DevBuf d_flag, d_scan;
	i32 n_groups = 0;
	bool pd_path = false, seed_view_ready = false, pdbm_dirty = true; i64 pd_words = 0;
	DevBuf w_j0; u32 walk_ticket = 0, walk_epoch = 0;
	DevBuf d_zero;
	DevBuf d_pdby; bool pd_bytes = false;
	DevBuf d_pdcb;
	DevBuf d_pdbm, d_gpre, d_key_c, d_val_c;
	DevBuf g_beg;

	i64 n_a = 0;
	DevBuf a_q, a_len, a_r, a_gb, a_ge;
	DevBuf a_uniq, a_cu, a_alive, a_ws, a_wid;
	DevBuf a_next, a_brk, a_aurank, a_aulist, a_runinfo;
	DevBuf w_best, w_sum, w_n;
	DevBuf d_btab;
	DevBuf d_flag2, d_scan2, d_i64a;
	i64 n_b = 0, n_c = 0;
	DevBuf b_q, b_len, b_r, b_gb, b_ge;
	DevBuf c_q, c_len, c_r, c_gb, c_ge;
	DevBuf c_bid;
	i32 n_blocks2 = 0;
	DevBuf blk_beg, blk_end, blk_score;
	std::vector<i32> h_blk_beg, h_blk_end, h_blk_score;

	i64 n_r = 0;
	DevBuf r_q, r_len, r_r, r_bid, r_tmp_q, r_tmp_len, r_tmp_r, r_tmp_bid;
	DevBuf r_cut4, r_cut5, r_simjob, r_simres;
	DevBuf d_leaf; std::vector<Leaf> h_leaf;
	std::vector<HostBlock> blocks;
	std::vector<i32> h_r_q, h_r_len; std::vector<i64> h_r_r;
	bool have_host_seeds = false;

	i64 n_frags = 0, n_aln = 0;
	i32 n_large = 0;
	DevBuf p_jpatch; i32 n_jobs = 0;
	DevBuf d_tail, p_tail;
	const i32 *h_tmail = nullptr, *h_tpatch = nullptr; char *h_taln1 = nullptr, *h_taln2 = nullptr;
	i64 nf_ub = 0, span_ub = 0;
	DevBuf fb_seedbase, fb_sbeg, fb_fragbase;
	DevBuf f_rec;
	DevBuf f_rec16;
	DevBuf f_type, f_mism, f_alnlen, f_job, f_score;
	DevBuf j_frag, j_opsoff, j_nops, d_ops, j_cells;
	DevBuf d_dp_tiny;
	DevBuf d_dp_arena;
	DevBuf d_dp_bnd, d_dp_ctr, d_dp_jobs, d_dp_large;
	DevBuf e_id, e_rec, e_list, e_off1, e_off2, e_opsoff, e_nops, e_ops, e_rev, r_head, f_early, r_orig, r_tmp_orig, p_early;
	bool early_consumed = false;
	bool early_listed = false;
	i32 n_early = 0; bool early_in_flight = false; std::vector<i32> h_early;
	bool dp_dirty = true;
	bool dp_timeout = false, dp_safe = false;
	int dp_fake_timeout = 0;
	u32 dp_epoch = 0;
	DevBuf p_dp, p_sj, p_sj_early;
	DevBuf d_alnoff;
	DevBuf bl_alnlen, bl_score;
	std::vector<gsa_rec> h_frags; std::vector<gsa_block> h_blocks; std::vector<char> h_aln1, h_aln2;
	int frags_stage = 0;
	DevBuf p_frags, p_blk; bool result_pinned = false;
	double alloc_ms = 0; long long alloc_n = 0, alloc_bytes = 0;
};

static inline void ctx_quiesce(gsa_ctx *c)
{
	hipStreamSynchronize(c->stream);
	for (int i = 0; i < 4; i++) if (c->stream_aux[i]) hipStreamSynchronize(c->stream_aux[i]);
}

void *dev_take_reserved(int device, size_t bytes, size_t *got);
template <class T> static inline T *dev_ensure(gsa_ctx *c, DevBuf &b, size_t n, bool exact = false)
{
	size_t bytes = (n ? n : 1) * sizeof(T);
	b.len = bytes;
	if (bytes <= b.cap) return (T *)b.p;
	const auto t0_ = std::chrono::steady_clock::now();
	if (b.p) { ctx_quiesce(c); hipFree(b.p); b.p = nullptr; b.cap = 0; }
	size_t want = exact ? bytes + 256 : bytes + bytes / 2 + 256;
	if (exact && bytes >= ((size_t)1 << 30)) { size_t got = 0; if (void *r = dev_take_reserved(c->device, want, &got)) { b.p = r; b.cap = got; return (T *)b.p; } }
	if (hipMalloc(&b.p, want) != hipSuccess) { gsa_fail(c, GSA_ERR_NOMEM, "hipMalloc"); return nullptr; }
	b.cap = want;
	c->alloc_ms += std::chrono::duration<double, std::milli>(std::chrono::steady_clock::now() - t0_).count(); c->alloc_n++; c->alloc_bytes += (long long)want;
	return (T *)b.p;
}

template <class T> static inline T *pin_ensure(gsa_ctx *c, DevBuf &b, size_t n)
{
	size_t bytes = (n ? n : 1) * sizeof(T);
	if (bytes <= b.cap) return (T *)b.p;
	const auto t0_ = std::chrono::steady_clock::now();
	if (b.p) { ctx_quiesce(c); hipHostFree(b.p); b.p = nullptr; b.cap = 0; }
	size_t want = bytes + bytes / 4 + 4096;
	if (hipHostMalloc(&b.p, want) != hipSuccess) { gsa_fail(c, GSA_ERR_NOMEM, "hipHostMalloc"); return nullptr; }
	b.cap = want;
	c->alloc_ms += std::chrono::duration<double, std::milli>(std::chrono::steady_clock::now() - t0_).count(); c->alloc_n++; c->alloc_bytes += (long long)want;
	return (T *)b.p;
}

int build_dense_sa(gsa_ctx *c, u64 n_sa);
int unpack_pac(gsa_ctx *c, const uint8_t *d_pac, i64 G, uint8_t *d_ref);
int build_occ(gsa_ctx *c, const void *ref_layout, u64 n_blocks128);
int build_presence(gsa_ctx *c);
int stage1_seed(gsa_ctx *c);
int stage1_import_hits(gsa_ctx *c, const u64 *keys, const u32 *vals, i64 n);
int stage1_finish_split(gsa_ctx *c);
int stage1_restore_pdbm(gsa_ctx *c);
int seed_view_sort(gsa_ctx *c);
int stage2_chain(gsa_ctx *c);
int launch_early_dp(gsa_ctx *c);
int stage2_fetch_host(gsa_ctx *c);
void collect_events(gsa_ctx *c);
int stage345_refine(gsa_ctx *c);
int stage7_fill(gsa_ctx *c);
i64 frags_count(gsa_ctx *c);
int stage78_extend(gsa_ctx *c);
int run_gapsim_jobs(gsa_ctx *c, i32 n, const i32 *d_n, const i32 *d_q1, const i32 *d_q2, const i64 *d_r1, const i64 *d_r2, i32 *d_res, const i32 *d_jseed, i32 *d_cut4);
void dp_count_cells(gsa_ctx *c, i32 n_ub, const i32 *len1, const i32 *len2, hipStream_t stream);
struct LgJob { i32 job, m, n; };
int launch_stripes(gsa_ctx *c, hipStream_t ss, std::vector<LgJob> &large, const uint8_t *pool1, const i64 *off1, const uint8_t *pool2, const i64 *off2,
                   uint8_t *ops, const i64 *ops_off, i32 *ops_len, uint8_t *rev, int err_slot);
struct Ksw2Launch { i32 n = 0, nsmall = 0, nlarge = 0; bool small_in_flight = false; };
int run_ksw2_jobs(gsa_ctx *c, i32 n_ub, const uint8_t *pool1, const i64 *off1, const i32 *len1,
                  const uint8_t *pool2, const i64 *off2, const i32 *len2, uint8_t *ops, const i64 *ops_off, i32 *ops_len, i64 ops_total, Ksw2Launch *out,
                  const i32 *jfrag = nullptr, gsa_frag *frag = nullptr, bool mail_clean = false);

#endif
```

gsalign_amd/csrc/k_chain.hip:

```cpp
#include "gsa_ctx.h"
#include "gsa_scan.h"
#include "gsa_gap.h"

#define TPB 256
#define GID(n) i64 i = (i64)blockIdx.x * blockDim.x + threadIdx.x; if (i >= (n)) return

__device__ __forceinline__ i64 d_llabs(i64 v) { return v < 0 ? -v : v; }

__global__ void k_group_keys(i64 n, const i32 *__restrict__ s_q, const i32 *__restrict__ s_gid, int qbits, u64 *key, u32 *val)
{
	GID(n);
	key[i] = ((u64)(u32)s_gid[i] << qbits) | (u32)s_q[i];
	val[i] = (u32)i;
}

__global__ void k_gather_active(i64 na, const u32 *__restrict__ perm, const i32 *__restrict__ s_q, const i32 *__restrict__ s_len, const i64 *__restrict__ s_r,
                                const i32 *__restrict__ s_gid, const i32 *__restrict__ g_beg, i32 *a_q, i32 *a_len, i64 *a_r, i32 *a_gb, i32 *a_ge)
{
	GID(na);
	const u32 s = perm[i];
	a_q[i] = s_q[s]; a_len[i] = s_len[s]; a_r[i] = s_r[s];
	const i32 g = s_gid[s];
	a_gb[i] = g_beg[g]; a_ge[i] = g_beg[g + 1];
}

__device__ __forceinline__ u32 pd_starts(const u32 *__restrict__ bm, i64 w, int max_indel)
{
	const u64 m = ((u64)bm[w] << 32) | (w > 0 ? bm[w - 1] : 0u);
	if (max_indel <= 0) return (u32)(m >> 32);
	u64 sm = m << 1; int cov = 1;
	while (2 * cov <= max_indel) { sm |= sm << cov; cov *= 2; }
	if (cov < max_indel) sm |= sm << (max_indel - cov);
	return (u32)((m & ~sm) >> 32);
}
__device__ __forceinline__ u32 pd_starts_pair(u32 cur, u32 prev, int max_indel)
{
	const u64 m = ((u64)cur << 32) | prev;
	if (max_indel <= 0) return cur;
	u64 sm = m << 1; int cov = 1;
	while (2 * cov <= max_indel) { sm |= sm << cov; cov *= 2; }
	if (cov < max_indel) sm |= sm << (max_indel - cov);
	return (u32)((m & ~sm) >> 32);
}
__device__ __forceinline__ void pd_block_load(const u32 *__restrict__ bm, i64 blk, u32 (&w)[33])
{
	const uint4 *p = (const uint4 *)(bm + (blk << 5));
	w[0] = blk > 0 ? bm[(blk << 5) - 1] : 0u;
#pragma unroll
	for (int k = 0; k < 8; k++) { const uint4 q = p[k]; w[1 + 4 * k] = q.x; w[2 + 4 * k] = q.y; w[3 + 4 * k] = q.z; w[4 + 4 * k] = q.w; }
}
struct OpPdScan {
#ifdef LB_BISECT
	static constexpr int lb_id = 0;
#endif
	const u32 *bm, *cb; int max_indel; i32 *gpre, *mail; i64 nw;
	__device__ i32 value(i64 blk, int) const
	{
		if (!((cb[blk >> 5] >> (blk & 31)) & 1u)) return 0;
		u32 w[33]; pd_block_load(bm, blk, w);
		i32 n = 0;
#pragma unroll
		for (int k = 0; k < 32; k++) n += __popc(pd_starts_pair(w[k + 1], w[k], max_indel));
		return n;
	}
	__device__ void emit(i64 blk, const i32 *v, const i32 *ex) const { if (v[0] || ((cb[blk >> 5] >> (blk & 31)) & 1u)) gpre[blk] = ex[0]; }
	__device__ void done(const i32 *t) const { mail[M_NG] = t[0]; }
};
struct OpPdTouched {
#ifdef LB_BISECT
	static constexpr int lb_id = 1;
#endif
	const u32 *cb; i64 nblk; i32 *tlist, *mail;
	__device__ i32 value(i64 w, int) const { u32 x = cb[w]; const i64 left = nblk - (w << 5); if (left < 32) x &= left <= 0 ? 0u : ((1u << left) - 1u); return __popc(x); }
	__device__ void emit(i64 w, const i32 *v, const i32 *ex) const
	{
		if (!v[0]) return;
		u32 x = cb[w]; const i64 left = nblk - (w << 5); if (left < 32) x &= left <= 0 ? 0u : ((1u << left) - 1u);
		i32 at = ex[0];
		while (x) { const int b = __ffs((int)x) - 1; x &= x - 1; tlist[at++] = (i32)((w << 5) + b); }
	}
	__device__ void done(const i32 *t) const { mail[M_NTOUCH] = t[0]; }
};
struct OpPdScanList {
#ifdef LB_BISECT
	static constexpr int lb_id = 2;
#endif
	const u32 *bm; const i32 *tlist; int max_indel; i32 *gpre, *mail;
	struct Item { i32 blk, n; };
	__device__ Item load(i64 j) const
	{
		Item it; it.blk = -1; it.n = 0;
		if (j >= mail[M_NTOUCH]) return it;
		it.blk = tlist[j];
		u32 w[33]; pd_block_load(bm, it.blk, w);
#pragma unroll
		for (int k = 0; k < 32; k++) it.n += __popc(pd_starts_pair(w[k + 1], w[k], max_indel));
		return it;
	}
	__device__ i32 value(const Item &it, i64, int) const { return it.n; }
	__device__ void emit(const Item &it, i64, const i32 *, const i32 *ex) const { if (it.blk >= 0) gpre[it.blk] = ex[0]; }
	__device__ void done(const i32 *t) const { mail[M_NG] = t[0]; }
};
__global__ void k_pd_keys(i64 n, const u64 *__restrict__ hkey, const u32 *__restrict__ hval, const u32 *__restrict__ bm, const i32 *__restrict__ gpre, int max_indel, int qbits,
                          u64 *key, u32 *val)
{
	GID(n);
	const u64 k = hkey[i];
	const i64 pd = (i64)(k >> qbits); const u32 q = (u32)(k & ((1ull << qbits) - 1));
	const i64 w = pd >> 5; const int b = (int)(pd & 31);
	u32 wd[33]; pd_block_load(bm, w >> 5, wd);
	const int wi = (int)(w & 31);
	i32 below = 0; u32 st = 0;
#pragma unroll
	for (int k = 0; k < 32; k++) { const u32 sk = pd_starts_pair(wd[k + 1], wd[k], max_indel); below += k < wi ? __popc(sk) : 0; st = k == wi ? sk : st; }
	const i32 gid = gpre[w >> 5] + below + __popc(st & (b == 31 ? ~0u : ((2u << b) - 1))) - 1;
	key[i] = ((u64)(u32)gid << (qbits + 7)) | ((u64)q << 7) | (hval[i] >> 16);
	val[i] = (u32)i;
}
__global__ void k_pd_heads(i64 n, const u64 *__restrict__ key, int gshift, i32 *g_beg)
{
	GID(n);
	const i32 g = (i32)(key[i] >> gshift);
	if (i == 0 || (i32)(key[i - 1] >> gshift) != g) g_beg[g] = (i32)i;
	if (i == n - 1) g_beg[g + 1] = (i32)n;
}
__global__ void k_pd_gather(i64 n, const u64 *__restrict__ key, const u32 *__restrict__ perm, const u64 *__restrict__ hkey, const u32 *__restrict__ hval, int gshift, int qbits, Bundle bnd,
                            const i32 *__restrict__ g_beg, i32 *a_q, i32 *a_len, i64 *a_r, i32 *a_gb, i32 *a_ge, u32 *bm, u32 *cb)
{
	GID(n);
	const u32 src = perm[i];
	const u64 k = hkey[src];
	const i32 q = (i32)(k & ((1ull << qbits) - 1)); const i64 pdk = (i64)(k >> qbits);
	i64 pd = pdk - bnd.lmax;
	if (bnd.n) { const i32 ci = bnd.chunk_contig[q / GSA_CHUNK]; pd -= (i64)bnd.off[ci] + (i64)ci * bnd.pds; }
	a_q[i] = q; a_len[i] = (i32)(hval[src] & 0xffffu); a_r[i] = pd + q;
	bm[pdk >> 5] = 0; cb[pdk >> 15] = 0;
	const i32 g = (i32)(key[i] >> gshift);
	a_gb[i] = g_beg[g]; a_ge[i] = g_beg[g + 1];
}

struct OpUniqBrk {
#ifdef LB_BISECT
	static constexpr int lb_id = 3;
#endif
	static constexpr bool clamped = true;
	i64 na; const i32 *a_q; const i64 *a_r; const i32 *a_gb, *a_ge;
	i32 *uniq, *brk, *alive, *cuEx, *brkEx, *blist;
	struct Item { i32 gb, ge, q, qm, qp, u, b; i64 r, rm; };
	__device__ Item load(i64 i) const
	{
		const i64 im = i > 0 ? i - 1 : 0, ip = i + 1 < na ? i + 1 : i;
		Item it; it.gb = a_gb[i]; it.ge = a_ge[i]; it.q = a_q[i]; it.qm = a_q[im]; it.qp = a_q[ip]; it.r = a_r[i]; it.rm = a_r[im]; it.u = it.b = 0;
		return it;
	}
	__device__ void prep(Item &it, i64 i) const
	{
		const bool u = !(i > it.gb && it.qm == it.q) && !(i + 1 < it.ge && it.qp == it.q);
		it.u = u ? 1 : 0; it.b = (u && i > it.gb && (it.r - it.q) != (it.rm - it.qm)) ? 1 : 0;
	}
	__device__ i32 value(const Item &it, i64, int c) const { return c == 0 ? it.u : it.b; }
	__device__ void emit(const Item &, i64 i, const i32 *v, const i32 *ex) const
	{
		uniq[i] = v[0]; brk[i] = v[1]; alive[i] = 1; cuEx[i] = ex[0]; brkEx[i] = ex[1];
		if (v[1]) blist[ex[1]] = (i32)i;
	}
	__device__ void done(const i32 *t) const { cuEx[na] = t[0]; brkEx[na] = t[1]; uniq[na] = 0; brk[na] = 0; }
};

struct OpCand {
#ifdef LB_BISECT
	static constexpr int lb_id = 4;
#endif
	static constexpr bool clamped = true;
	i64 na; const i32 *a_gb, *a_ge, *cuEx, *brk;
	i32 *candf, *candEx, *clist, *ws;
	struct Item { i32 cand, head, gb, b, ce, cb; };
	__device__ Item load(i64 i) const
	{
		Item it; it.gb = a_gb[i]; it.b = brk[i]; it.ce = cuEx[a_ge[i]]; it.cb = cuEx[it.gb]; it.cand = it.head = 0;
		return it;
	}
	__device__ void prep(Item &it, i64 i) const { it.head = i == it.gb ? 1 : 0; it.cand = (it.ce - it.cb >= GSA_WIN_SEEDS && (i == it.gb || it.b)) ? 1 : 0; }
	__device__ i32 value(const Item &it, i64, int) const { return it.cand; }
	__device__ void emit(const Item &it, i64 i, const i32 *v, const i32 *ex) const
	{
		candf[i] = v[0]; candEx[i] = ex[0]; ws[i] = it.head;
		if (v[0]) clist[ex[0]] = (i32)i;
	}
	__device__ void done(const i32 *t) const { candEx[na] = t[0]; candf[na] = 0; ws[na] = 0; }
};

__global__ void k_next_window(i64 na, const i32 *__restrict__ a_q, const i32 *__restrict__ a_gb, const i32 *__restrict__ a_ge,
                              const i32 *__restrict__ uniq, const i32 *__restrict__ cuEx, const i32 *__restrict__ brk, const i32 *__restrict__ brkEx,
                              const i32 *__restrict__ blist, const i32 *__restrict__ candf, const i32 *__restrict__ candEx, const i32 *__restrict__ clist, i32 *next, i32 *nextk,
                              uint4 *tab_clear, i64 tab_cap)
{
	for (i64 j = (i64)blockIdx.x * blockDim.x + threadIdx.x; j < tab_cap; j += (i64)gridDim.x * blockDim.x) tab_clear[j] = make_uint4(~0u, ~0u, ~0u, ~0u);
	GID(na);
	if (!candf[i]) { next[i] = -1; return; }
	const i32 gb = a_gb[i], ge = a_ge[i];
	const i32 base = (i == gb) ? cuEx[gb] : cuEx[i] + uniq[i];
	i32 lo = (i32)i + 1, hi = ge;
	while (lo < hi) { i32 mid = (lo + hi) >> 1; if (cuEx[mid + 1] - base >= GSA_WIN_SEEDS) hi = mid; else lo = mid + 1; }
	const i32 j1 = lo;
	lo = (i32)i + 1; hi = ge;
	const i32 qi = a_q[i];
	while (lo < hi) { i32 mid = (lo + hi) >> 1; if (a_q[mid] - qi > GSA_WIN_SPAN) hi = mid; else lo = mid + 1; }
	const i32 j0 = j1 > lo ? j1 : lo;
	i32 nx = ge;
	if (j0 < ge) { const i32 nB = brkEx[na]; const i32 k = brkEx[j0]; if (k < nB) { const i32 cand = blist[k]; if (cand < ge) nx = cand; } }
	i32 nk = candEx[nx];
	if (nx == ge) { nk = candEx[ge]; nx = nk < candEx[na] ? clist[nk] : (i32)na; }
	next[i] = nx; nextk[candEx[i]] = nk;
}

#define WALK_T 1024
#define WALK_MAXTILES 8192
#define WALK_LDS_CAND 20480
__global__ void __launch_bounds__(WALK_T) k_walk_windows(i64 na, const i32 *__restrict__ candEx, const i32 *__restrict__ clist, const i32 *__restrict__ next, const i32 *__restrict__ nextk, i32 *ws)
{
	__shared__ __attribute__((aligned(16))) i32 buf[2 * 2048 + 3 * WALK_LDS_CAND / 2 + 2 * WALK_LDS_CAND / 32];
	static_assert(sizeof(buf) >= 2 * WALK_MAXTILES * sizeof(i32), "arena too small for the global-memory path");
	uint16_t *s_nk = (uint16_t *)(buf + 2 * 2048);
	uint16_t (*s_J)[WALK_LDS_CAND] = (uint16_t (*)[WALK_LDS_CAND])(s_nk + WALK_LDS_CAND);
	u32 *s_on = (u32 *)(s_nk + 3 * WALK_LDS_CAND), *s_start = s_on + WALK_LDS_CAND / 32;
	__shared__ int changed;
	const int tid = threadIdx.x;
	const i32 nC = candEx[na];
	if (nC <= WALK_LDS_CAND) {
		uint16_t *nk = s_nk;
		i32 *tile_kb = buf, *tile_ke = buf + 2048;
		i64 ts = 256; while ((na + ts - 1) / ts > 2048) ts <<= 1;
		const int nt = (int)((na + ts - 1) / ts);
		for (int k0 = tid; k0 < nC; k0 += 8 * WALK_T) {
			i32 d[8];
#pragma unroll
			for (int u = 0; u < 8; u++) { const int k = k0 + u * WALK_T; d[u] = k < nC ? nextk[k] - k : 0; }
#pragma unroll
			for (int u = 0; u < 8; u++) { const int k = k0 + u * WALK_T; if (k < nC) nk[k] = (uint16_t)(d[u] < 0xffff ? d[u] : 0xffff); }
		}
		for (int w = tid; w < (nC + 31) / 32; w += WALK_T) { s_on[w] = 0; s_start[w] = 0; }
		for (int t = tid; t < nt; t += WALK_T) {
			const i64 pe = (i64)(t + 1) * ts < na ? (i64)(t + 1) * ts : na;
			tile_kb[t] = candEx[(i64)t * ts]; tile_ke[t] = candEx[pe];
		}
		__syncthreads();
#define WALK_NEXT(k) (nk[k] != 0xffff ? (k) + (i32)nk[k] : nextk[k])
		for (int t = tid; t < nt; t += WALK_T) {
			const i32 kb = tile_kb[t], ke = tile_ke[t];
			for (i32 k = ke - 1; k >= kb; k--) {
				const i32 nx = WALK_NEXT(k);
				s_J[0][k] = nx >= ke ? (uint16_t)(nx < nC ? nx : 0xffff) : s_J[0][nx];
			}
		}
		__syncthreads();
		if (tid == 0 && nC > 0) {
			for (u32 k = 0; k != 0xffff; k = s_J[0][k]) s_on[k >> 5] |= 1u << (k & 31);
		}
		__syncthreads();
		for (int t = tid; t < nt; t += WALK_T) {
			const i32 kb = tile_kb[t], ke = tile_ke[t];
			i32 e = -1;
			for (i32 k = kb; k < ke; k++) if ((s_on[k >> 5] >> (k & 31)) & 1u) { e = k; break; }
			if (e < 0) continue;
			for (i32 k = e; k < ke; k = WALK_NEXT(k)) atomicOr(&s_start[k >> 5], 1u << (k & 31));
		}
		__syncthreads();
		for (int k0 = tid; k0 < nC; k0 += 8 * WALK_T) {
			i32 p[8];
#pragma unroll
			for (int u = 0; u < 8; u++) { const int k = k0 + u * WALK_T; p[u] = (k < nC && ((s_start[k >> 5] >> (k & 31)) & 1u)) ? clist[k] : -1; }
#pragma unroll
			for (int u = 0; u < 8; u++) if (p[u] >= 0) ws[p[u]] = 1;
		}
#undef WALK_NEXT
		return;
	}
	i32 *entry = buf, *exit_ = buf + WALK_MAXTILES;
	i64 ts = 256; while ((na + ts - 1) / ts > WALK_MAXTILES) ts <<= 1;
	const int nt = (int)((na + ts - 1) / ts);
	for (int t = tid; t < nt; t += WALK_T) {
		const i32 k = candEx[(i64)t * ts];
		entry[t] = k < nC ? clist[k] : (i32)na; exit_[t] = -1;
	}
	__syncthreads();
	for (;;) {
		for (int t = tid; t < nt; t += WALK_T) {
			if (exit_[t] >= 0) continue;
			const i64 e = (i64)(t + 1) * ts < na ? (i64)(t + 1) * ts : na;
			i64 p = entry[t];
			while (p < e) { const i32 nx = next[p]; p = nx >= 0 ? nx : p + 1; }
			exit_[t] = (i32)p;
		}
		if (tid == 0) changed = 0;
		__syncthreads();
		bool moved[WALK_MAXTILES / WALK_T];
		for (int t = tid, k = 0; t < nt; t += WALK_T, k++) {
			moved[k] = false;
			if (t == 0) continue;
			const i32 ne = exit_[t - 1];
			if (ne != entry[t]) { entry[t] = ne; moved[k] = true; changed = 1; }
		}
		__syncthreads();
		const int again = changed;
		for (int t = tid, k = 0; t < nt; t += WALK_T, k++) if (moved[k]) exit_[t] = -1;
		__syncthreads();
		if (!again) break;
	}
	for (int t = tid; t < nt; t += WALK_T) {
		const i64 e = (i64)(t + 1) * ts < na ? (i64)(t + 1) * ts : na;
		for (i64 p = entry[t]; p < e; p = next[p]) ws[p] = 1;
	}
}

struct Bucket { unsigned long long key; u32 cnt; u32 pad; };
#define BKT_EMPTY (~0ull)
__device__ __forceinline__ u32 bkt_hash(unsigned long long k, u32 cap) { return (u32)((((k * 0x9E3779B97F4A7C15ull) >> 32) * (unsigned long long)cap) >> 32); }

struct OpWindowBuckets {
#ifdef LB_BISECT
	static constexpr int lb_id = 5;
#endif
	static constexpr bool clamped = true;
	i64 na; const i32 *a_q; const i64 *a_r; const i32 *uniq, *ws; i64 bmin; u32 cap;
	i32 *wsEx, *slot_of; Bucket *tab; unsigned long long *wbest, *wsum; i32 *wn;
	struct Item { i32 ws, uniq; i64 pd; };
	__device__ Item load(i64 i) const { Item it; it.ws = ws[i]; it.uniq = uniq[i]; it.pd = a_r[i] - a_q[i]; return it; }
	__device__ i32 value(const Item &it, i64, int) const { return it.ws; }
	__device__ void emit(const Item &it, i64 i, const i32 *v, const i32 *ex) const
	{
		wsEx[i] = ex[0];
		if (it.ws) { wbest[ex[0]] = 0; wsum[ex[0]] = 0; wn[ex[0]] = 0; }
		i32 slot = -1;
		const u32 w = (u32)(ex[0] + v[0] - 1);
		const u32 b = (u32)((it.pd >> 4) - bmin);
		const unsigned long long key = ((unsigned long long)w << 32) | b;
		bool pend = it.uniq != 0;
		for (int round = 0; round < 2 && __any(pend); round++) {
			const unsigned long long live = __ballot(pend);
			const int lead = __ffsll((long long)live) - 1;
			const unsigned long long k0 = __shfl(key, lead);
			const bool mine = pend && key == k0;
			const unsigned long long grp = __ballot(mine);
			u32 h = 0;
			if ((int)(threadIdx.x & 63) == lead) {
				h = bkt_hash(key, cap);
				for (;;) {
					const unsigned long long old = atomicCAS(&tab[h].key, BKT_EMPTY, key);
					if (old == BKT_EMPTY || old == key) break;
					h = h + 1 == cap ? 0u : h + 1;
				}
				atomicAdd(&tab[h].cnt, (u32)__popcll(grp));
			}
			h = __shfl(h, lead);
			if (mine) { slot = (i32)h; pend = false; }
		}
		if (pend) {
			u32 h = bkt_hash(key, cap);
			for (;;) {
				const unsigned long long old = atomicCAS(&tab[h].key, BKT_EMPTY, key);
				if (old == BKT_EMPTY || old == key) break;
				h = h + 1 == cap ? 0u : h + 1;
			}
			atomicAdd(&tab[h].cnt, 1u);
			slot = (i32)h;
		}
		slot_of[i] = slot;
	}
	static constexpr bool has_emit_all = true;
	template <int ITEMS>
	__device__ void emit_all(const Item (&it)[ITEMS], i64 i0, const bool (&in)[ITEMS], const i32 (&v)[ITEMS], const i32 (&ex)[ITEMS]) const
	{
		const int lane = (int)(threadIdx.x & 63);
		unsigned long long key[ITEMS]; bool pend[ITEMS]; i32 slot[ITEMS];
#pragma unroll
		for (int k = 0; k < ITEMS; k++) {
			const i64 i = i0 + (i64)k * LB_TPB;
			slot[k] = -1; pend[k] = false; key[k] = 0;
			if (in[k]) {
				wsEx[i] = ex[k];
				if (it[k].ws) { wbest[ex[k]] = 0; wsum[ex[k]] = 0; wn[ex[k]] = 0; }
				const u32 w = (u32)(ex[k] + v[k] - 1);
				const u32 b = (u32)((it[k].pd >> 4) - bmin);
				key[k] = ((unsigned long long)w << 32) | b;
				pend[k] = it[k].uniq != 0;
			}
		}
		for (int round = 0; round < 2; round++) {
			int lead[ITEMS]; unsigned long long k0[ITEMS], old[ITEMS]; u32 h[ITEMS]; unsigned long long grp[ITEMS]; bool act[ITEMS], mine[ITEMS];
#pragma unroll
			for (int k = 0; k < ITEMS; k++) {
				const unsigned long long live = __ballot(pend[k]);
				act[k] = live != 0;
				lead[k] = act[k] ? __ffsll((long long)live) - 1 : 0;
				k0[k] = __shfl(key[k], lead[k]);
				mine[k] = pend[k] && key[k] == k0[k];
				grp[k] = __ballot(mine[k]);
				h[k] = bkt_hash(k0[k], cap);
				old[k] = k0[k];
			}
#pragma unroll
			for (int k = 0; k < ITEMS; k++) if (act[k] && lane == lead[k]) old[k] = atomicCAS(&tab[h[k]].key, BKT_EMPTY, k0[k]);
#pragma unroll
			for (int k = 0; k < ITEMS; k++) {
				if (act[k] && lane == lead[k]) {
					while (old[k] != BKT_EMPTY && old[k] != k0[k]) { h[k] = h[k] + 1 == cap ? 0u : h[k] + 1; old[k] = atomicCAS(&tab[h[k]].key, BKT_EMPTY, k0[k]); }
					atomicAdd(&tab[h[k]].cnt, (u32)__popcll(grp[k]));
				}
				const u32 hs = __shfl(h[k], lead[k]);
				if (mine[k]) { slot[k] = (i32)hs; pend[k] = false; }
			}
		}
		{
			u32 h[ITEMS]; unsigned long long old[ITEMS];
#pragma unroll
			for (int k = 0; k < ITEMS; k++) { h[k] = bkt_hash(key[k], cap); old[k] = key[k]; if (pend[k]) old[k] = atomicCAS(&tab[h[k]].key, BKT_EMPTY, key[k]); }
#pragma unroll
			for (int k = 0; k < ITEMS; k++) if (pend[k]) {
				while (old[k] != BKT_EMPTY && old[k] != key[k]) { h[k] = h[k] + 1 == cap ? 0u : h[k] + 1; old[k] = atomicCAS(&tab[h[k]].key, BKT_EMPTY, key[k]); }
				atomicAdd(&tab[h[k]].cnt, 1u);
				slot[k] = (i32)h[k];
			}
		}
#pragma unroll
		for (int k = 0; k < ITEMS; k++) if (in[k]) slot_of[i0 + (i64)k * LB_TPB] = slot[k];
	}
	__device__ void done(const i32 *t) const { wsEx[na] = t[0]; wbest[na] = 0; wsum[na] = 0; wn[na] = 0; }
};

__global__ void k_window_mode(i64 cap, const Bucket *__restrict__ tab, unsigned long long *wbest)
{
	GID(cap);
	const unsigned long long k = tab[i].key;
	if (k == BKT_EMPTY) return;
	atomicMax(&wbest[(u32)(k >> 32)], ((unsigned long long)(tab[i].cnt + 1u) << 32) | (0xFFFFFFFFu - (u32)k));
}

__global__ void k_window_avg(i64 na, const i32 *__restrict__ slot_of, const Bucket *__restrict__ tab, const i32 *__restrict__ a_q, const i64 *__restrict__ a_r,
                             const unsigned long long *__restrict__ wbest, const i32 *__restrict__ ws, const i32 *__restrict__ wsEx, unsigned long long *wsum, i32 *wn, Bundle bnd)
{
	const i64 i = (i64)blockIdx.x * blockDim.x + threadIdx.x;
	const int lane = threadIdx.x & 63;
	u32 w = 0xffffffffu; unsigned long long vs = 0; i32 vn = 0;
	if (i < na) {
		w = (u32)(wsEx[i] + ws[i] - 1);
		const i32 sl = slot_of[i];
		if (sl >= 0) {
			const i64 kk = (i64)(u32)tab[sl].key, mode = (i64)(0xFFFFFFFFu - (u32)wbest[w]);
			if (d_llabs(kk - mode) < 3) { vs = (unsigned long long)(a_r[i] - a_q[i] + bundle_off(bnd, a_q[i])); vn = 1; }
		}
	}
	for (int d = 1; d < 64; d <<= 1) {
		const u32 ow = __shfl_up(w, d); const unsigned long long os = __shfl_up(vs, d); const i32 on = __shfl_up(vn, d);
		if (lane >= d && ow == w) { vs += os; vn += on; }
	}
	const u32 nw = __shfl_down(w, 1);
	if (i < na && vn > 0 && (lane == 63 || nw != w)) { atomicAdd(&wsum[w], vs); atomicAdd(&wn[w], vn); }
}

struct OpAliveUnique {
#ifdef LB_BISECT
	static constexpr int lb_id = 6;
#endif
	static constexpr bool clamped = true;
	i64 na; const i32 *uniq; i32 *alive, *auEx, *aulist;
	const i32 *slot_of; const Bucket *tab; const i32 *a_q; const i64 *a_r; const unsigned long long *wbest, *wsum; const i32 *wn; i64 G; i32 max_indel; Bundle bnd;
	struct Item { i32 alive, uniq, sl, q, wn, boff; u32 cnt; unsigned long long key, wbest, wsum; i64 r; };
	__device__ Item load(i64 i) const
	{
		Item it; it.uniq = uniq[i]; it.alive = 1;
		it.sl = slot_of[i]; it.q = a_q[i]; it.r = a_r[i];
		const uint4 e = *(const uint4 *)&tab[it.sl < 0 ? 0 : it.sl];
		it.key = ((unsigned long long)e.y << 32) | e.x; it.cnt = e.z;
		const u32 w = it.sl < 0 ? 0u : e.y;
		it.wbest = wbest[w]; it.wsum = wsum[w]; it.wn = wn[w];
		it.boff = bundle_off_flat(bnd, it.q);
		return it;
	}
	__device__ void prep(Item &it, i64) const
	{
		if (it.sl < 0) return;
		const i64 kk = (i64)(u32)it.key, mode = (i64)(0xFFFFFFFFu - (u32)it.wbest);
		const i32 cnt = d_llabs(kk - mode) < 3 ? (i32)(it.cnt + 1u) : 0;
		const i64 avg = it.wn > 0 ? (i64)it.wsum / it.wn : G;
		const i64 pd = it.r - it.q + it.boff;
		if (d_llabs(avg - pd) > max_indel && cnt < 3) it.alive = 0;
	}
	__device__ i32 value(const Item &it, i64, int) const { return (it.uniq && it.alive) ? 1 : 0; }
	__device__ void emit(const Item &it, i64 i, const i32 *v, const i32 *ex) const { alive[i] = it.alive; auEx[i] = ex[0]; if (v[0]) aulist[ex[0]] = (i32)i; }
	__device__ void done(const i32 *t) const { auEx[na] = t[0]; }
};

__device__ __forceinline__ i32 multihit_keep(i64 i, const i32 *__restrict__ a_q, const i64 *__restrict__ a_r, i32 gb, i32 ge, const i32 *__restrict__ auEx, const i32 *__restrict__ aulist,
                                             i64 G, i32 max_indel, const Bundle &bnd)
{
	const i32 q = a_q[i];
	i32 h = (i32)i; while (h > gb && a_q[h - 1] == q) h--;
	i32 j = (i32)i + 1; while (j < ge && a_q[j] == q) j++;
	i64 s1 = 0, s2 = 0; i32 n1 = 0, n2 = 0;
	for (i32 k = auEx[h] - 1; k >= auEx[gb] && n1 < 5; k--) { const i32 s = aulist[k]; s1 += a_r[s] - a_q[s]; n1++; }
	for (i32 k = auEx[j]; k < auEx[ge] && n2 < 5; k++) { const i32 s = aulist[k]; s2 += a_r[s] - a_q[s]; n2++; }
	const i64 o = bundle_off(bnd, q);
	const i64 avg = (n1 > 0 || n2 > 0) ? (s1 + s2 + o * (n1 + n2)) / (n1 + n2) : (a_r[h] - q + o);
	i32 idx = -1; i64 md = G;
	for (i32 k = h; k < j; k++) { const i64 d = d_llabs((a_r[k] - q + o) - avg); if (d < max_indel && d < md) { md = d; idx = k; } }
	return idx;
}

struct OpCompactAlive {
#ifdef LB_BISECT
	static constexpr int lb_id = 7;
#endif
	static constexpr bool clamped = true;
	const i32 *alive, *a_q, *a_len; const i64 *a_r; const i32 *a_gb, *a_ge, *auEx, *aulist; i64 G; i32 max_indel; Bundle bnd;
	i32 *b_q, *b_len; i64 *b_r; i32 *b_g, *mail; i64 na;
	struct Item { i32 alive, q, len, g, ge, qm, qp; i64 r; };
	__device__ Item load(i64 i) const
	{
		const i64 im = i > 0 ? i - 1 : 0, ip = i + 1 < na ? i + 1 : i;
		Item it; it.alive = alive[i]; it.q = a_q[i]; it.g = a_gb[i]; it.ge = a_ge[i]; it.len = a_len[i]; it.r = a_r[i]; it.qm = a_q[im]; it.qp = a_q[ip];
		return it;
	}
	__device__ void prep(Item &it, i64 i) const
	{
		it.alive = it.alive ? 1 : 0;
		const bool multi = it.alive && ((i + 1 < it.ge && it.qp == it.q) || (i > it.g && it.qm == it.q));
		if (multi && multihit_keep(i, a_q, a_r, it.g, it.ge, auEx, aulist, G, max_indel, bnd) != (i32)i) it.alive = 0;
	}
	__device__ i32 value(const Item &it, i64, int) const { return it.alive; }
	__device__ void emit(const Item &it, i64, const i32 *v, const i32 *ex) const
	{
		if (!v[0]) return;
		const i32 p = ex[0];
		b_q[p] = it.q; b_len[p] = it.len; b_r[p] = it.r; b_g[p] = it.g;
	}
	__device__ void done(const i32 *t) const { mail[M_NB] = t[0]; }
};

struct OpNoise {
#ifdef LB_BISECT
	static constexpr int lb_id = 8;
#endif
	static constexpr bool clamped = true;
	const i32 *b_q, *b_len; const i64 *b_r; const i32 *b_g;
	i32 *c_q, *c_len; i64 *c_r; i32 *c_g, *mail; i64 na;
	struct Item { i32 keep, q, len, g, gm, gp, qm, qp, nb; i64 r, rm, rp; };
	__device__ Item load(i64 i) const
	{
		const i64 im = i > 0 ? i - 1 : 0, ip = i + 1 < na ? i + 1 : i;
		Item it; it.nb = mail[M_NB]; it.q = b_q[i]; it.len = b_len[i]; it.r = b_r[i]; it.g = b_g[i];
		it.gm = b_g[im]; it.gp = b_g[ip]; it.qm = b_q[im]; it.qp = b_q[ip]; it.rm = b_r[im]; it.rp = b_r[ip]; it.keep = 0;
		return it;
	}
	__device__ void prep(Item &it, i64 i) const
	{
		it.keep = i < it.nb ? 1 : 0;
		if (i > 0 && i + 1 < it.nb && it.gm == it.g && it.gp == it.g) {
			const i64 pd = it.r - it.q, p0 = it.rm - it.qm, p1 = it.rp - it.qp;
			if (d_llabs(pd - p0) > 5 && d_llabs(pd - p1) > 5) it.keep = 0;
		}
	}
	__device__ i32 value(const Item &it, i64, int) const { return it.keep; }
	__device__ void emit(const Item &it, i64, const i32 *v, const i32 *ex) const
	{
		if (!v[0]) return;
		const i32 p = ex[0];
		c_q[p] = it.q; c_len[p] = it.len; c_r[p] = it.r; c_g[p] = it.g;
	}
	__device__ void done(const i32 *t) const { mail[M_NC] = t[0]; mail[M_MAXBLK] = 0; mail[M_MAXBLK + 1] = 0; }
};

struct OpBlockHeads {
#ifdef LB_BISECT
	static constexpr int lb_id = 9;
#endif
	static constexpr bool clamped = true;
	i64 na; const i32 *c_q, *c_len; const i64 *c_r; const i32 *c_g;
	i32 *bhead, *bheadEx, *bstart; u32 *ps; i32 *mail;
	struct Item { i32 h, len, nc, q, qm, lenm, g, gm; i64 r, rm; };
	__device__ Item load(i64 i) const
	{
		const i64 im = i > 0 ? i - 1 : 0;
		Item it; it.nc = mail[M_NC]; it.q = c_q[i]; it.qm = c_q[im]; it.len = c_len[i]; it.lenm = c_len[im]; it.g = c_g[i]; it.gm = c_g[im]; it.r = c_r[i]; it.rm = c_r[im]; it.h = 0;
		return it;
	}
	__device__ void prep(Item &it, i64 i) const
	{
		const i64 pd = it.r - it.q, p0 = it.rm - it.qm;
		const bool head = i == 0 || it.gm != it.g || it.q - it.qm - it.lenm > GSA_MAX_SEED_GAP || d_llabs(p0 - pd) > 100;
		it.h = (i < it.nc && head) ? 1 : 0; if (i >= it.nc) it.len = 0;
	}
	__device__ i32 value(const Item &it, i64, int c) const { return c == 1 ? it.len : it.h; }
	__device__ void emit(const Item &, i64 i, const i32 *v, const i32 *ex) const { bhead[i] = v[0]; bheadEx[i] = ex[0]; ps[i] = (u32)ex[1]; if (v[0]) bstart[ex[0]] = (i32)i; }
	__device__ void done(const i32 *t) const { bheadEx[na] = t[0]; bhead[na] = 0; ps[na] = (u32)t[1]; mail[M_NBRAW] = t[0]; }
};

struct OpBlockFilter {
#ifdef LB_BISECT
	static constexpr int lb_id = 10;
#endif
	static constexpr bool clamped = true;
	i64 na; const i32 *bstart, *c_q, *c_len; const u32 *ps; Params prm;
	i32 *bkeep, *bkeepEx, *blk_beg, *blk_end, *blk_score, *mail;
	__device__ void span(i64 b, i32 &s, i32 &e) const { const i32 nAll = mail[M_NBRAW]; s = bstart[b]; e = (b + 1 < nAll) ? bstart[b + 1] : mail[M_NC]; }
	struct Item { i32 keep, s, e, score; };
	__device__ Item load(i64 b) const
	{
		const i32 nAll = mail[M_NBRAW], nc = mail[M_NC];
		const i32 s0 = bstart[b], sn = bstart[b + 1];
		Item it; it.s = s0; it.e = (b + 1 < nAll) ? sn : nc;
		const i64 sc = it.s < 0 ? 0 : (it.s < na ? it.s : na - 1), ec = it.e < 1 ? 1 : (it.e <= na ? it.e : na);
		it.score = (i32)(ps[ec] - ps[sc]);
		const i32 region = c_q[ec - 1] + c_len[ec - 1] - c_q[sc];
		const bool drop = it.score < prm.MinAlnBlockScore || region < prm.MinAlnLength || (it.score < 1000 && (double)it.score < region * 0.05);
		it.keep = (b < nAll && !drop) ? 1 : 0;
		return it;
	}
	__device__ i32 value(const Item &it, i64, int) const { return it.keep; }
	__device__ void emit(const Item &it, i64 b, const i32 *v, const i32 *ex) const
	{
		bkeep[b] = v[0]; bkeepEx[b] = ex[0];
		if (!v[0]) return;
		blk_beg[ex[0]] = it.s; blk_end[ex[0]] = it.e; blk_score[ex[0]] = it.score;
		atomicMax((unsigned long long *)(mail + M_MAXBLK), ((unsigned long long)(u32)it.score << 32) | (u32)ex[0]);
	}
	__device__ void done(const i32 *t) const { mail[M_NBLK] = t[0]; }
};

struct OpEarlyGaps {
#ifdef LB_BISECT
	static constexpr int lb_id = 11;
#endif
	const i32 *q, *len; const i64 *r; const i32 *head, *headEx, *bkeep, *bkeepEx; i32 *bid; const uint8_t *query, *ref;
	__device__ i32 bid_of(i64 i) const { const i32 b = headEx[i] + head[i] - 1; return bkeep[b] ? bkeepEx[b] : -1; }
	i32 *e_id, *e_list; i64 *off1, *off2, *opsoff; i32 *mail;
	const i32 *blk_beg, *blk_end, *blk_score;
	__device__ bool early_block(i32 b) const
	{
		const unsigned long long mx = *(const unsigned long long *)(mail + M_MAXBLK);
		const i32 bm = (i32)(u32)mx; const i64 sm = (i64)(mx >> 32);
		if (b == bm || (i64)blk_score[b] * 4 >= sm) return true;
		if ((i64)blk_score[b] * 16 < sm) return false;
		const i32 qs = q[blk_beg[b]], qe = q[blk_end[b] - 1] + len[blk_end[b] - 1];
		const i32 ms = q[blk_beg[bm]], me = q[blk_end[bm] - 1] + len[blk_end[bm] - 1];
		return !(qs >= ms && qe <= me);
	}
	i32 *e_rec;
	__device__ bool gap(i64 s, i32 &qp, i64 &rp, i32 &qg, i32 &rg) const
	{
		if (s + 1 >= mail[M_NC]) return false;
		{ const i32 b0 = bid_of(s); if (b0 < 0 || bid_of(s + 1) != b0 || !early_block(b0)) return false; }
		qp = q[s] + len[s]; rp = r[s] + len[s];
		qg = q[s + 1] - qp; if (qg < 0) qg = 0;
		const i64 rg64 = r[s + 1] - rp; rg = rg64 < 0 ? 0 : (i32)rg64;
		if (qg > GSA_MAX_SEED_GAP || rg64 > GSA_MAX_SEED_GAP || !dp_is_large(rg, qg)) return false;
		i32 mism;
		return classify_gap(query, ref, qp, rp, qg, rg, mism) == FT_DP;
	}
#ifndef EG_CLAMPED
#define EG_CLAMPED false
#endif
	static constexpr bool clamped = EG_CLAMPED;
	struct Item { i32 in, bid, g, qp, qg, rg; i64 rp;
	              i32 q0, len0, q1, k0, x0, k1, x1, sc0; i64 r0, r1; };
	__device__ Item load(i64 s) const
	{
		const i64 sp = s + 1 < na ? s + 1 : s;
		Item it; it.in = 0; it.bid = -1; it.g = 0; it.qp = it.qg = it.rg = 0; it.rp = 0;
		it.q0 = q[s]; it.len0 = len[s]; it.r0 = r[s]; it.q1 = q[sp]; it.r1 = r[sp];
		i64 b0 = (i64)headEx[s] + head[s] - 1, b1 = (i64)headEx[sp] + head[sp] - 1;
		b0 = b0 < 0 ? 0 : (b0 < na ? b0 : na - 1); b1 = b1 < 0 ? 0 : (b1 < na ? b1 : na - 1);
		it.k0 = bkeep[b0]; it.x0 = bkeepEx[b0]; it.k1 = bkeep[b1]; it.x1 = bkeepEx[b1];
		const i64 kb = it.x0 < 0 ? 0 : (it.x0 <= na ? it.x0 : na);
		it.sc0 = blk_score[kb];
		return it;
	}
	__device__ void prep(Item &it, i64 s) const
	{
		const i32 nc = mail[M_NC];
		if (s >= nc) return;
		it.in = 1; it.bid = it.k0 ? it.x0 : -1;
		if (s + 1 >= nc) return;
		const i32 b0 = it.bid, b1 = it.k1 ? it.x1 : -1;
		if (b0 < 0 || b1 != b0) return;
		{
			const unsigned long long mx = *(const unsigned long long *)(mail + M_MAXBLK);
			const i32 bm = (i32)(u32)mx; const i64 sm = (i64)(mx >> 32);
			if (!(b0 == bm || (i64)it.sc0 * 4 >= sm)) {
				if ((i64)it.sc0 * 16 < sm) return;
				const i32 qs = q[blk_beg[b0]], qe = q[blk_end[b0] - 1] + len[blk_end[b0] - 1];
				const i32 ms = q[blk_beg[bm]], me = q[blk_end[bm] - 1] + len[blk_end[bm] - 1];
				if (qs >= ms && qe <= me) return;
			}
		}
		const i32 qp = it.q0 + it.len0; const i64 rp = it.r0 + it.len0;
		i32 qg = it.q1 - qp; if (qg < 0) qg = 0;
		const i64 rg64 = it.r1 - rp; const i32 rg = rg64 < 0 ? 0 : (i32)rg64;
		if (qg > GSA_MAX_SEED_GAP || rg64 > GSA_MAX_SEED_GAP || !dp_is_large(rg, qg)) return;
		i32 mism;
		if (classify_gap(query, ref, qp, rp, qg, rg, mism) != FT_DP) return;
		it.g = 1; it.qp = qp; it.rp = rp; it.qg = it.q1 - qp; it.rg = (i32)(it.r1 - rp);
	}
	__device__ i32 value(const Item &it, i64, int c) const { return c == 1 ? (it.g ? it.qg + it.rg : 0) : it.g; }
	__device__ void emit(const Item &it, i64 s, const i32 *v, const i32 *ex) const
	{
		if (it.in) bid[s] = it.bid;
		e_id[s] = v[0] ? ex[0] : -1;
		if (!v[0]) return;
		const i32 e = ex[0];
		lb_pub(&e_list[3 * e], e); lb_pub(&e_list[3 * e + 1], it.rg); lb_pub(&e_list[3 * e + 2], it.qg);
		off1[e] = it.rp; off2[e] = it.qp; opsoff[e] = ex[1]; e_rec[e] = -1;
	}
	__device__ void done(const i32 *t) const { lb_pub(&mail[M_NEARLY], t[0]); lb_pub(&mail[M_EOPS], t[1]); lb_pub(&mail[M_DPERR3], 0); }
	i32 *h_early; i32 h_cap;
	i64 na;
	__device__ void finish(int tid) const
	{
		const i32 ne = __hip_atomic_load(&mail[M_NEARLY], __ATOMIC_RELAXED, __HIP_MEMORY_SCOPE_AGENT);
		if (tid == 0) { h_early[0] = ne; h_early[1] = __hip_atomic_load(&mail[M_EOPS], __ATOMIC_RELAXED, __HIP_MEMORY_SCOPE_AGENT); }
		const i32 w = 3 * (ne < h_cap ? ne : h_cap);
		lb_copy_out(h_early + 4, e_list, w, tid);
	}
};
#define EARLY_CHUNK 4096

int launch_early_dp(gsa_ctx *c)
{
	if (!c->early_listed) return GSA_OK;
	c->early_listed = false;
	GSA_CHECK(c, hipEventSynchronize(c->ev[16]));
	const i32 *h = c->p_early.as<i32>();
	const i32 ne = h[0]; const i64 eops = h[1];
	if (ne <= 0) return GSA_OK;
	const size_t first_e = (size_t)std::min<i64>(c->n_a, EARLY_CHUNK);
	hipStream_t sa = c->stream_aux[0];
	if ((size_t)ne > first_e) {
		if (!pin_ensure<i32>(c, c->p_early, 4 + 3 * (size_t)ne)) return GSA_ERR_NOMEM;
		h = c->p_early.as<i32>();
		GSA_CHECK(c, hipMemcpyAsync(c->p_early.as<i32>() + 4, c->e_list.p, (size_t)ne * 12, hipMemcpyDeviceToHost, sa));
		GSA_CHECK(c, hipStreamSynchronize(sa));
	}
	c->h_early.assign(h + 4, h + 4 + 3 * (size_t)ne);
	std::vector<LgJob> large((const LgJob *)(h + 4), (const LgJob *)(h + 4) + ne);
	if (!dev_ensure<uint8_t>(c, c->e_ops, (size_t)eops + 64) || !dev_ensure<uint8_t>(c, c->e_rev, (size_t)eops + 64) || !dev_ensure<i32>(c, c->e_nops, (size_t)ne + 1) || !dev_ensure<i32>(c, c->e_rec, (size_t)ne + 1)) return GSA_ERR_NOMEM;
	GSA_CHECK(c, hipStreamWaitEvent(sa, c->ev[16], 0));
	int rc = launch_stripes(c, sa, large, c->di.ref, c->e_off1.as<i64>(), c->q_dev, c->e_off2.as<i64>(),
	                        c->e_ops.as<uint8_t>(), c->e_opsoff.as<i64>(), c->e_nops.as<i32>(), c->e_rev.as<uint8_t>(), M_DPERR3);
	if (rc) return rc;
	GSA_CHECK(c, hipEventRecord(c->ev[14], sa));
	c->n_early = ne; c->early_in_flight = true; c->dbg[6] = (u64)ne;
	return GSA_OK;
}

#define LAUNCH(k, n, ...) hipLaunchKernelGGL(k, dim3(grid_for((size_t)(n), TPB)), dim3(TPB), 0, st, __VA_ARGS__)
#define ENS(T, buf, n) do { if (!dev_ensure<T>(c, c->buf, (size_t)(n))) return GSA_ERR_NOMEM; } while (0)
#define RC(x) do { int rc_ = (x); if (rc_) return rc_; } while (0)

#define WC_SL 16384
#if defined(__HIP_DEVICE_COMPILE__) && !defined(__gfx950__)
#error "k_walk_chain keeps 4 x 32 KB of slice tables in LDS: gfx950 (160 KB of LDS per CU) only"
#endif
#define WC_T 1024
__global__ void __launch_bounds__(WC_T) k_walk_chain(i64 na, const i32 *__restrict__ candEx, const i32 *__restrict__ clist, const i32 *__restrict__ nextk, i32 *ws,
                                                     u32 *ticket, u32 ticket0, unsigned long long *entry_w, u32 epoch, i32 *err)
{
	__shared__ uint16_t h[WC_SL], E1[WC_SL], E2[WC_SL], E3[WC_SL];
	__shared__ u32 on[WC_SL / 32];
	__shared__ uint16_t mid_e[WC_SL / 1024], sub_e[WC_SL / 64];
	__shared__ u32 s_slice; __shared__ i32 s_entry;
	const int tid = threadIdx.x;
	const i32 nC = candEx[na];
	if (tid == 0) s_slice = atomicAdd(ticket, 1u) - ticket0;
	__syncthreads();
	const i32 sl = (i32)s_slice, base = sl * WC_SL;
	const i32 nsl = (nC + WC_SL - 1) / WC_SL;
	if (sl >= nsl) return;
	const i32 cnt = nC - base < WC_SL ? nC - base : WC_SL;
	for (int k = tid; k < WC_SL; k += WC_T) {
		u32 v = 0xffffu;
		if (k < cnt) { const i32 nx = nextk[base + k] - base; if (nx < cnt) v = (u32)nx; }
		h[k] = (uint16_t)v;
	}
	for (int w = tid; w < WC_SL / 32; w += WC_T) on[w] = 0;
	if (tid < WC_SL / 1024) mid_e[tid] = 0xffff;
	if (tid < WC_SL / 64) sub_e[tid] = 0xffff;
	__syncthreads();
	if (tid < WC_SL / 64) {
		const int b = tid * 64;
		for (int k = b + 63; k >= b; k--) { const u32 nx = h[k]; E1[k] = (uint16_t)((nx != 0xffffu && (nx >> 6) == (u32)tid) ? E1[nx] : (u32)k); }
	}
	__syncthreads();
	{
		const u32 w = (u32)tid >> 6, l = (u32)tid & 63u;
		for (int j = 15; j >= 0; j--) {
			const u32 k = w * 1024u + (u32)j * 64u + l;
			const u32 e1 = E1[k], nx = h[e1];
			E2[k] = (uint16_t)((nx != 0xffffu && (nx >> 10) == w) ? E2[nx] : e1);
			__syncthreads();
		}
	}
	for (int j = WC_SL / 1024 - 1; j >= 0; j--) {
		const u32 k = (u32)j * 1024u + (u32)tid;
		const u32 e2 = E2[k], nx = h[e2];
		E3[k] = (uint16_t)(nx != 0xffffu ? E3[nx] : e2);
		__syncthreads();
	}
	if (tid == 0) {
		i32 e = -2;
		if (sl == 0) e = 0;
		else {
			u32 spins = 0; unsigned long long t_spin0 = 0;
			for (;;) {
				const unsigned long long wv = __hip_atomic_load(&entry_w[sl], __ATOMIC_RELAXED, __HIP_MEMORY_SCOPE_AGENT);
				if ((u32)(wv >> 32) == epoch) { e = (i32)(u32)wv - 2; break; }
				if ((++spins & 1023u) == 0 && (t_spin0 == 0 ? (t_spin0 = wall_clock64(), false) : wall_clock64() - t_spin0 > LB_WAIT_TICKS)) { __hip_atomic_store(err, 1, __ATOMIC_RELAXED, __HIP_MEMORY_SCOPE_AGENT); break; }
				__builtin_amdgcn_s_sleep(1);
			}
		}
		s_entry = e;
		if (e >= 0) {
			const i32 x = nextk[base + (i32)E3[e - base]];
			const i32 t = x < nC ? x / WC_SL : nsl;
			if (t < nsl) __hip_atomic_store(&entry_w[t], ((unsigned long long)epoch << 32) | (u32)(x + 2), __ATOMIC_RELAXED, __HIP_MEMORY_SCOPE_AGENT);
			for (i32 s2 = sl + 1; s2 < t; s2++) __hip_atomic_store(&entry_w[s2], (unsigned long long)epoch << 32, __ATOMIC_RELAXED, __HIP_MEMORY_SCOPE_AGENT);
		}
	}
	__syncthreads();
	const i32 e = s_entry;
	if (e < 0) return;
	if (tid == 0) { u32 x = (u32)(e - base); for (;;) { mid_e[x >> 10] = (uint16_t)x; const u32 nx = h[E2[x]]; if (nx == 0xffffu) break; x = nx; } }
	__syncthreads();
	if (tid < WC_SL / 1024 && mid_e[tid] != 0xffff) { u32 x = mid_e[tid]; for (;;) { sub_e[x >> 6] = (uint16_t)x; const u32 nx = h[E1[x]]; if (nx == 0xffffu || (nx >> 10) != (u32)tid) break; x = nx; } }
	__syncthreads();
	if (tid < WC_SL / 64 && sub_e[tid] != 0xffff) { u32 x = sub_e[tid]; for (;;) { atomicOr(&on[x >> 5], 1u << (x & 31)); const u32 nx = h[x]; if (nx == 0xffffu || (nx >> 6) != (u32)tid) break; x = nx; } }
	__syncthreads();
	for (int k0 = tid; k0 < cnt; k0 += 8 * WC_T) {
		i32 p[8];
#pragma unroll
		for (int u = 0; u < 8; u++) { const int k = k0 + u * WC_T; p[u] = (k < cnt && ((on[k >> 5] >> (k & 31)) & 1u)) ? clist[base + k] : -1; }
#pragma unroll
		for (int u = 0; u < 8; u++) if (p[u] >= 0) ws[p[u]] = 1;
	}
}

int stage2_chain(gsa_ctx *c)
{
	hipStream_t st = c->stream;
	c->n_blocks2 = 0; c->n_c = 0; c->n_b = 0; c->n_a = 0; c->blocks.clear(); c->s2_host = true;
	c->n_early = 0; c->early_listed = false;
	c->h_blk_beg.clear(); c->h_blk_end.clear(); c->h_blk_score.clear();
	const i64 n = c->n_seeds;
	if (n == 0) return GSA_OK;
	c->s2_host = false;
	if (c->profiling) hipEventRecord(c->ev[4], st);
	const i64 na = n; c->n_a = na;
	ENS(i64, d_i64a, n + 2); ENS(i32, d_flag2, n + 2); ENS(i32, d_scan2, n + 2); ENS(i32, d_flag, n + 1); ENS(i32, d_scan, n + 1);
	const int gbits = ceil_log2_u64((u64)n + 1);
	ENS(i32, a_q, na); ENS(i32, a_len, na); ENS(i64, a_r, na); ENS(i32, a_gb, na); ENS(i32, a_ge, na);
	if (c->pd_path && c->qbits + 7 + gbits <= 64) {
		const i64 nw = c->pd_words;
		const i64 nblk = (nw + 31) >> 5;
		ENS(i32, d_gpre, ((nw + 31) >> 5) + 2); ENS(u64, d_key_c, n); ENS(u32, d_val_c, n); ENS(u64, d_key_b, n); ENS(u32, d_val_b, n); ENS(i32, g_beg, n + 2);
		i32 *mail_ = c->d_mail.as<i32>();
		if (nblk > c->opt.pd_two_level_min) {
			const i64 nw2 = (nblk + 31) >> 5;
			{ OpPdTouched op = { c->d_pdcb.as<u32>(), nblk, c->d_flag.as<i32>(), mail_ }; RC((lb_launch<1, 4>(c, nw2, op))); }
			{ OpPdScanList op = { c->d_pdbm.as<u32>(), c->d_flag.as<i32>(), c->prm.MaxIndelSize, c->d_gpre.as<i32>(), mail_ }; RC((lb_launch<1, 4>(c, n < nblk ? n : nblk, op, nullptr, 8))); }
		} else
		{ OpPdScan op = { c->d_pdbm.as<u32>(), c->d_pdcb.as<u32>(), c->prm.MaxIndelSize, c->d_gpre.as<i32>(), mail_, nw };
		  if (nblk <= (1 << 20)) RC((lb_launch<1, 1>(c, nblk, op, nullptr, 8))); else RC((lb_launch<1, 4>(c, nblk, op, nullptr, 8))); }
		{}
		LAUNCH(k_pd_keys, n, n, c->d_key_a.as<u64>(), c->d_val_a.as<u32>(), c->d_pdbm.as<u32>(), c->d_gpre.as<i32>(), c->prm.MaxIndelSize, c->qbits, c->d_key_c.as<u64>(), c->d_val_c.as<u32>());
		RC(gsa_sort_pairs_u64_u32(c, c->d_key_c.as<u64>(), c->d_key_b.as<u64>(), c->d_val_c.as<u32>(), c->d_val_b.as<u32>(), (size_t)na, c->hits_sorted ? c->qbits + 7 : 0, c->qbits + 7 + gbits));
		LAUNCH(k_pd_heads, n, n, c->d_key_b.as<u64>(), c->qbits + 7, c->g_beg.as<i32>());
		LAUNCH(k_pd_gather, n, n, c->d_key_b.as<u64>(), c->d_val_b.as<u32>(), c->d_key_a.as<u64>(), c->d_val_a.as<u32>(), c->qbits + 7, c->qbits, c->bnd, c->g_beg.as<i32>(),
		       c->a_q.as<i32>(), c->a_len.as<i32>(), c->a_r.as<i64>(), c->a_gb.as<i32>(), c->a_ge.as<i32>(), c->d_pdbm.as<u32>(), c->d_pdcb.as<u32>());
		c->pdbm_dirty = false;
	} else {
		RC(seed_view_sort(c));
		ENS(u64, d_key_a, n); ENS(u64, d_key_b, n); ENS(u32, d_val_a, n); ENS(u32, d_val_b, n);
		LAUNCH(k_group_keys, n, n, c->s_q.as<i32>(), c->s_gid.as<i32>(), c->qbits, c->d_key_a.as<u64>(), c->d_val_a.as<u32>());
		RC(gsa_sort_pairs_u64_u32(c, c->d_key_a.as<u64>(), c->d_key_b.as<u64>(), c->d_val_a.as<u32>(), c->d_val_b.as<u32>(), (size_t)na, 0, c->qbits + gbits));
		LAUNCH(k_gather_active, na, na, c->d_val_b.as<u32>(), c->s_q.as<i32>(), c->s_len.as<i32>(), c->s_r.as<i64>(), c->s_gid.as<i32>(), c->g_beg.as<i32>(),
		       c->a_q.as<i32>(), c->a_len.as<i32>(), c->a_r.as<i64>(), c->a_gb.as<i32>(), c->a_ge.as<i32>());
	}
	ENS(i32, a_uniq, na + 1); ENS(i32, a_cu, na + 1); ENS(i32, a_alive, na + 1); ENS(i32, a_brk, na + 1); ENS(i32, a_aurank, na + 1);
	ENS(i32, a_aulist, na + 1); ENS(i32, a_next, na + 1); ENS(i32, a_ws, na + 1); ENS(i32, a_wid, na + 1); ENS(i32, a_runinfo, na + 1);
	i32 *uniq = c->a_uniq.as<i32>(), *cuEx = c->a_cu.as<i32>(), *alive = c->a_alive.as<i32>(), *brk = c->a_brk.as<i32>();
	i32 *brkEx = c->a_aurank.as<i32>(), *blist = c->a_aulist.as<i32>(), *next = c->a_next.as<i32>(), *ws = c->a_ws.as<i32>(), *wsEx = c->a_wid.as<i32>();
	i32 *mail = c->d_mail.as<i32>();
	{ OpUniqBrk op = { na, c->a_q.as<i32>(), c->a_r.as<i64>(), c->a_gb.as<i32>(), c->a_ge.as<i32>(), uniq, brk, alive, cuEx, brkEx, blist }; RC((lb_launch<2>(c, na, op))); }
	i32 *candf = c->d_flag.as<i32>(), *candEx = c->d_scan.as<i32>(), *clist = c->a_runinfo.as<i32>();
	{ OpCand op = { na, c->a_gb.as<i32>(), c->a_ge.as<i32>(), cuEx, brk, candf, candEx, clist, ws }; RC((lb_launch<1>(c, na, op))); }
	const i64 cap = na + na / 4 + 1024;
	ENS(Bucket, d_btab, cap);
	static_assert(sizeof(Bucket) == 16, "the table is cleared as uint4s");
	LAUNCH(k_next_window, na, na, c->a_q.as<i32>(), c->a_gb.as<i32>(), c->a_ge.as<i32>(), uniq, cuEx, brk, brkEx, blist, candf, candEx, clist, next, c->d_flag2.as<i32>(), c->d_btab.as<uint4>(), cap);
	if (na <= c->opt.walk_chain_min) hipLaunchKernelGGL(k_walk_windows, dim3(1), dim3(WALK_T), 0, st, na, candEx, clist, next, c->d_flag2.as<i32>(), ws);
	else {
		const u32 grid = (u32)((na + WC_SL - 1) / WC_SL);
		const size_t cap0 = c->w_j0.cap;
		ENS(unsigned long long, w_j0, (size_t)grid + 8);
		if (c->w_j0.cap != cap0) { GSA_CHECK(c, hipMemsetAsync(c->w_j0.p, 0, c->w_j0.cap, st)); c->walk_ticket = 0; c->walk_epoch = 0; }
		unsigned long long *words = c->w_j0.as<unsigned long long>();
		hipLaunchKernelGGL(k_walk_chain, dim3(grid), dim3(WC_T), 0, st, na, candEx, clist, (const i32 *)c->d_flag2.as<i32>(), ws, (u32 *)words, c->walk_ticket, words + 4, c->walk_epoch + 1, mail + M_LBERR);
		GSA_CHECK(c, hipGetLastError());
		c->walk_epoch++; c->walk_ticket += grid;
	}
	ENS(unsigned long long, w_best, na + 1); ENS(unsigned long long, w_sum, na + 1); ENS(i32, w_n, na + 1);
	const i64 bmin = ((-(i64)c->qlen) >> 4) - 1;
	i32 *slot_of = c->a_runinfo.as<i32>();
	{ OpWindowBuckets op = { na, c->a_q.as<i32>(), c->a_r.as<i64>(), uniq, ws, bmin, (u32)cap, wsEx, slot_of, c->d_btab.as<Bucket>(),
	                         c->w_best.as<unsigned long long>(), c->w_sum.as<unsigned long long>(), c->w_n.as<i32>() }; RC((lb_launch<1, 4>(c, na, op))); }
	LAUNCH(k_window_mode, cap, cap, c->d_btab.as<Bucket>(), c->w_best.as<unsigned long long>());
	LAUNCH(k_window_avg, na, na, slot_of, c->d_btab.as<Bucket>(), c->a_q.as<i32>(), c->a_r.as<i64>(), c->w_best.as<unsigned long long>(), ws, wsEx,
	       c->w_sum.as<unsigned long long>(), c->w_n.as<i32>(), c->bnd);
	i32 *auEx = c->a_aurank.as<i32>(), *aulist = c->a_aulist.as<i32>();
	{ OpAliveUnique op = { na, uniq, alive, auEx, aulist, slot_of, c->d_btab.as<Bucket>(), c->a_q.as<i32>(), c->a_r.as<i64>(),
	                       c->w_best.as<unsigned long long>(), c->w_sum.as<unsigned long long>(), c->w_n.as<i32>(), c->G, c->prm.MaxIndelSize, c->bnd }; RC((lb_launch<1>(c, na, op))); }
	ENS(i32, b_q, na); ENS(i32, b_len, na); ENS(i64, b_r, na); ENS(i32, b_gb, na);
	{ OpCompactAlive op = { alive, c->a_q.as<i32>(), c->a_len.as<i32>(), c->a_r.as<i64>(), c->a_gb.as<i32>(), c->a_ge.as<i32>(), auEx, aulist, c->G, c->prm.MaxIndelSize, c->bnd,
	                        c->b_q.as<i32>(), c->b_len.as<i32>(), c->b_r.as<i64>(), c->b_gb.as<i32>(), mail, na }; RC((lb_launch<1>(c, na, op))); }
	ENS(i32, c_q, na); ENS(i32, c_len, na + 1); ENS(i64, c_r, na); ENS(i32, c_gb, na); ENS(i32, c_bid, na);
	{ OpNoise op = { c->b_q.as<i32>(), c->b_len.as<i32>(), c->b_r.as<i64>(), c->b_gb.as<i32>(),
	                 c->c_q.as<i32>(), c->c_len.as<i32>(), c->c_r.as<i64>(), c->c_gb.as<i32>(), mail, na }; RC((lb_launch<1>(c, na, op))); }
	i32 *bhead = c->a_uniq.as<i32>(), *bheadEx = c->a_cu.as<i32>(), *bstart = c->a_brk.as<i32>();
	{ OpBlockHeads op = { na, c->c_q.as<i32>(), c->c_len.as<i32>(), c->c_r.as<i64>(), c->c_gb.as<i32>(), bhead, bheadEx, bstart, c->d_flag2.as<u32>(), mail }; RC((lb_launch<2>(c, na, op))); }
	i32 *bkeep = c->a_ws.as<i32>(), *bkeepEx = c->a_wid.as<i32>();
	ENS(i32, blk_beg, na + 1); ENS(i32, blk_end, na + 1); ENS(i32, blk_score, na + 1);
	{ OpBlockFilter op = { na, bstart, c->c_q.as<i32>(), c->c_len.as<i32>(), c->d_flag2.as<u32>(), c->prm, bkeep, bkeepEx,
	                       c->blk_beg.as<i32>(), c->blk_end.as<i32>(), c->blk_score.as<i32>(), mail }; RC((lb_launch<1>(c, na, op))); }
	if (c->profiling) { hipEventRecord(c->ev[5], st); c->ev_pending |= 2; }
	ENS(i32, e_id, na + 2); ENS(i32, e_rec, na + 2); ENS(i32, e_list, 3 * (na + 1)); ENS(i64, e_off1, na + 1); ENS(i64, e_off2, na + 1); ENS(i64, e_opsoff, na + 2);
	if (!pin_ensure<i32>(c, c->p_early, 4 + 3 * (size_t)EARLY_CHUNK)) return GSA_ERR_NOMEM;
	{ OpEarlyGaps op = { c->c_q.as<i32>(), c->c_len.as<i32>(), c->c_r.as<i64>(), bhead, bheadEx, bkeep, bkeepEx, c->c_bid.as<i32>(), c->q_dev, c->di.ref,
	                     c->e_id.as<i32>(), c->e_list.as<i32>(), c->e_off1.as<i64>(), c->e_off2.as<i64>(), c->e_opsoff.as<i64>(), mail,
	                     c->blk_beg.as<i32>(), c->blk_end.as<i32>(), c->blk_score.as<i32>(), c->e_rec.as<i32>(),
	                     c->p_early.as<i32>(), (i32)std::min<i64>(na, EARLY_CHUNK) }; op.na = na; RC((lb_launch<2>(c, na, op))); }
	GSA_CHECK(c, hipEventRecord(c->ev[16], st));
	c->early_listed = true;
	return GSA_OK;
}

int stage2_fetch_host(gsa_ctx *c)
{
	if (c->s2_host) return GSA_OK;
	GSA_CHECK(c, hipStreamSynchronize(c->stream));
	GSA_CHECK(c, hipMemcpy(c->h_mail, c->d_mail.p, MAIL_N * sizeof(i32), hipMemcpyDeviceToHost));
	c->n_b = c->h_mail[M_NB]; c->n_c = c->h_mail[M_NC]; c->n_blocks2 = c->h_mail[M_NBLK];
	const i32 nblk = c->n_blocks2;
	c->h_blk_beg.resize(nblk); c->h_blk_end.resize(nblk); c->h_blk_score.resize(nblk);
	if (nblk > 0) {
		GSA_CHECK(c, hipMemcpy(c->h_blk_beg.data(), c->blk_beg.p, (size_t)nblk * 4, hipMemcpyDeviceToHost));
		GSA_CHECK(c, hipMemcpy(c->h_blk_end.data(), c->blk_end.p, (size_t)nblk * 4, hipMemcpyDeviceToHost));
		GSA_CHECK(c, hipMemcpy(c->h_blk_score.data(), c->blk_score.p, (size_t)nblk * 4, hipMemcpyDeviceToHost));
	}
	c->s2_host = true;
	return GSA_OK;
}

#ifdef LB_TIMING
extern "C" int gsa_debug_lb_prof(unsigned long long *out, int reset)
{
	if (hipMemcpyFromSymbol(out, HIP_SYMBOL(g_lb_prof), sizeof(g_lb_prof)) != hipSuccess) return -1;
	if (reset) { unsigned long long z[8] = { 0 }; if (hipMemcpyToSymbol(HIP_SYMBOL(g_lb_prof), z, sizeof(z)) != hipSuccess) return -1; }
	return 0;
}
#endif
```

Baseline: 33.70 Gbp/s.

## Store group id per seed and pack chain flags into bytes

Replaces the per-seed group begin/end arrays with a single group id and derives head/last from neighbouring ids. It merges the uniq, break and candidate flags into byte flag arrays, stores window starts and alive flags as u8, and adds a per-group prefix table g_cu. The k_pd_heads kernel is folded into k_pd_gather, which can also clear only the touched bitmap blocks from a list. The aim is to cut global memory traffic and one launch in the chaining stage, at the cost of extra neighbour loads and indirections through g_beg.

```diff
diff --git a/gsalign_amd/csrc/gsa_api.hip b/gsalign_amd/csrc/gsa_api.hip
--- a/gsalign_amd/csrc/gsa_api.hip
+++ b/gsalign_amd/csrc/gsa_api.hip
@@ -253,7 +253,7 @@
 	return GSA_OK;
 }
 
-#define GSA_DEVBUFS(X) X(d_bwt) X(d_bwt_ref) X(d_occ_base) X(d_sa) X(d_ref) X(d_chr_end) X(d_chr_of_end) X(qs[0].d_query) X(qs[1].d_query) X(qs[0].d_bndtab) X(qs[1].d_bndtab) X(tmp) X(d_cnt) X(d_zero) X(d_mail) X(d_lb_status[0]) X(d_lb_status[1]) X(d_sa_dense) X(d_kmer) X(d_kmer_lo) X(d_pres) X(d_ref2) X(d_cand_s) X(d_cand_len) X(d_cand_x0) X(d_cand_freq) X(d_onpath) X(d_cand_cnt) X(d_heavy) X(dn_lf) X(dn_x0) X(d_chunk_hits) X(d_chunk_base) X(d_key_a) X(d_key_b) X(d_val_a) X(d_val_b) X(s_q) X(s_len) X(s_r) X(s_gid) X(d_flag) X(d_scan) X(g_beg) X(w_j0) X(d_pdbm) X(d_pdby) X(d_pdcb) X(d_gpre) X(d_key_c) X(d_val_c) X(a_q) X(a_len) X(a_r) X(a_gb) X(a_ge) X(a_uniq) X(a_cu) X(a_alive) X(a_ws) X(a_wid) X(a_next) X(a_brk) X(a_aurank) X(a_aulist) X(a_runinfo) X(w_best) X(w_sum) X(w_n) X(d_btab) X(d_flag2) X(d_scan2) X(d_i64a) X(b_q) X(b_len) X(b_r) X(b_gb) X(b_ge) X(c_q) X(c_len) X(c_r) X(c_gb) X(c_ge) X(c_bid) X(blk_beg) X(blk_end) X(blk_score) X(r_q) X(r_len) X(r_r) X(r_bid) X(r_tmp_q) X(r_tmp_len) X(r_tmp_r) X(r_tmp_bid) X(r_cut4) X(r_cut5) X(r_simjob) X(r_simres) X(d_leaf) X(fb_seedbase) X(fb_sbeg) X(fb_fragbase) X(f_rec) X(f_rec16) X(f_type) X(f_mism) X(f_alnlen) X(f_job) X(f_score) X(d_dp_tiny) X(d_dp_bnd) X(d_dp_ctr) X(d_dp_jobs) X(d_dp_large) X(d_tail) X(e_id) X(e_rec) X(e_list) X(e_off1) X(e_off2) X(e_opsoff) X(e_nops) X(e_ops) X(e_rev) X(r_head) X(f_early) X(r_orig) X(r_tmp_orig) X(j_frag) X(j_opsoff) X(j_nops) X(d_ops) X(j_cells) X(d_alnoff) X(bl_alnlen) X(bl_score) X(d_bblk) X(d_dp_arena) X(leaf[0]) X(leaf[1]) X(leaf[2]) X(leaf[3]) X(leaf[4]) X(leaf[5]) X(leaf[6]) X(leaf[7]) X(leaf[8])
+#define GSA_DEVBUFS(X) X(d_bwt) X(d_bwt_ref) X(d_occ_base) X(d_sa) X(d_ref) X(d_chr_end) X(d_chr_of_end) X(qs[0].d_query) X(qs[1].d_query) X(qs[0].d_bndtab) X(qs[1].d_bndtab) X(tmp) X(d_cnt) X(d_zero) X(d_mail) X(d_lb_status[0]) X(d_lb_status[1]) X(d_sa_dense) X(d_kmer) X(d_kmer_lo) X(d_pres) X(d_ref2) X(d_cand_s) X(d_cand_len) X(d_cand_x0) X(d_cand_freq) X(d_onpath) X(d_cand_cnt) X(d_heavy) X(dn_lf) X(dn_x0) X(d_chunk_hits) X(d_chunk_base) X(d_key_a) X(d_key_b) X(d_val_a) X(d_val_b) X(s_q) X(s_len) X(s_r) X(s_gid) X(d_flag) X(d_scan) X(g_beg) X(w_j0) X(d_pdbm) X(d_pdby) X(d_pdcb) X(d_gpre) X(d_key_c) X(d_val_c) X(a_q) X(a_len) X(a_r) X(a_g) X(a_fl) X(a_cf) X(a_ws8) X(g_cu) X(a_uniq) X(a_cu) X(a_alive) X(a_ws) X(a_wid) X(a_next) X(a_brk) X(a_aurank) X(a_aulist) X(a_runinfo) X(w_best) X(w_sum) X(w_n) X(d_btab) X(d_flag2) X(d_scan2) X(d_i64a) X(b_q) X(b_len) X(b_r) X(b_gb) X(c_q) X(c_len) X(c_r) X(c_gb) X(c_bid) X(blk_beg) X(blk_end) X(blk_score) X(r_q) X(r_len) X(r_r) X(r_bid) X(r_tmp_q) X(r_tmp_len) X(r_tmp_r) X(r_tmp_bid) X(r_cut4) X(r_cut5) X(r_simjob) X(r_simres) X(d_leaf) X(fb_seedbase) X(fb_sbeg) X(fb_fragbase) X(f_rec) X(f_rec16) X(f_type) X(f_mism) X(f_alnlen) X(f_job) X(f_score) X(d_dp_tiny) X(d_dp_bnd) X(d_dp_ctr) X(d_dp_jobs) X(d_dp_large) X(d_tail) X(e_id) X(e_rec) X(e_list) X(e_off1) X(e_off2) X(e_opsoff) X(e_nops) X(e_ops) X(e_rev) X(r_head) X(f_early) X(r_orig) X(r_tmp_orig) X(j_frag) X(j_opsoff) X(j_nops) X(d_ops) X(j_cells) X(d_alnoff) X(bl_alnlen) X(bl_score) X(d_bblk) X(d_dp_arena) X(leaf[0]) X(leaf[1]) X(leaf[2]) X(leaf[3]) X(leaf[4]) X(leaf[5]) X(leaf[6]) X(leaf[7]) X(leaf[8])
 void gsa_destroy(gsa_ctx *c)
 {
 	if (!c) return;
diff --git a/gsalign_amd/csrc/gsa_ctx.h b/gsalign_amd/csrc/gsa_ctx.h
--- a/gsalign_amd/csrc/gsa_ctx.h
+++ b/gsalign_amd/csrc/gsa_ctx.h
@@ -149,15 +149,17 @@
 	DevBuf g_beg;
 
 	i64 n_a = 0;
-	DevBuf a_q, a_len, a_r, a_gb, a_ge;
-	DevBuf a_uniq, a_cu, a_alive, a_ws, a_wid;
+	DevBuf a_q, a_len, a_r, a_g;
+	DevBuf a_fl, a_cf, a_ws8, a_alive;
+	DevBuf g_cu;
+	DevBuf a_uniq, a_cu, a_ws, a_wid;
 	DevBuf a_next, a_brk, a_aurank, a_aulist, a_runinfo;
 	DevBuf w_best, w_sum, w_n;
 	DevBuf d_btab;
 	DevBuf d_flag2, d_scan2, d_i64a;
 	i64 n_b = 0, n_c = 0;
-	DevBuf b_q, b_len, b_r, b_gb, b_ge;
-	DevBuf c_q, c_len, c_r, c_gb, c_ge;
+	DevBuf b_q, b_len, b_r, b_gb;
+	DevBuf c_q, c_len, c_r, c_gb;
 	DevBuf c_bid;
 	i32 n_blocks2 = 0;
 	DevBuf blk_beg, blk_end, blk_score;
diff --git a/gsalign_amd/csrc/k_chain.hip b/gsalign_amd/csrc/k_chain.hip
--- a/gsalign_amd/csrc/k_chain.hip
+++ b/gsalign_amd/csrc/k_chain.hip
@@ -15,13 +15,12 @@
 }
 
 __global__ void k_gather_active(i64 na, const u32 *__restrict__ perm, const i32 *__restrict__ s_q, const i32 *__restrict__ s_len, const i64 *__restrict__ s_r,
-                                const i32 *__restrict__ s_gid, const i32 *__restrict__ g_beg, i32 *a_q, i32 *a_len, i64 *a_r, i32 *a_gb, i32 *a_ge)
+                                const i32 *__restrict__ s_gid, i32 *a_q, i32 *a_len, i64 *a_r, i32 *a_g)
 {
 	GID(na);
 	const u32 s = perm[i];
 	a_q[i] = s_q[s]; a_len[i] = s_len[s]; a_r[i] = s_r[s];
-	const i32 g = s_gid[s];
-	a_gb[i] = g_beg[g]; a_ge[i] = g_beg[g + 1];
+	a_g[i] = s_gid[s];
 }
 
 __device__ __forceinline__ u32 pd_starts(const u32 *__restrict__ bm, i64 w, int max_indel)
@@ -117,15 +116,9 @@
 	key[i] = ((u64)(u32)gid << (qbits + 7)) | ((u64)q << 7) | (hval[i] >> 16);
 	val[i] = (u32)i;
 }
-__global__ void k_pd_heads(i64 n, const u64 *__restrict__ key, int gshift, i32 *g_beg)
-{
-	GID(n);
-	const i32 g = (i32)(key[i] >> gshift);
-	if (i == 0 || (i32)(key[i - 1] >> gshift) != g) g_beg[g] = (i32)i;
-	if (i == n - 1) g_beg[g + 1] = (i32)n;
-}
+template <bool WIPE_LIST>
 __global__ void k_pd_gather(i64 n, const u64 *__restrict__ key, const u32 *__restrict__ perm, const u64 *__restrict__ hkey, const u32 *__restrict__ hval, int gshift, int qbits, Bundle bnd,
-                            const i32 *__restrict__ g_beg, i32 *a_q, i32 *a_len, i64 *a_r, i32 *a_gb, i32 *a_ge, u32 *bm, u32 *cb)
+                            i32 *g_beg, i32 *a_q, i32 *a_len, i64 *a_r, i32 *a_g, u32 *bm, u32 *cb, const i32 *__restrict__ tlist, const i32 *__restrict__ mail)
 {
 	GID(n);
 	const u32 src = perm[i];
@@ -134,9 +127,19 @@
 	i64 pd = pdk - bnd.lmax;
 	if (bnd.n) { const i32 ci = bnd.chunk_contig[q / GSA_CHUNK]; pd -= (i64)bnd.off[ci] + (i64)ci * bnd.pds; }
 	a_q[i] = q; a_len[i] = (i32)(hval[src] & 0xffffu); a_r[i] = pd + q;
-	bm[pdk >> 5] = 0; cb[pdk >> 15] = 0;
 	const i32 g = (i32)(key[i] >> gshift);
-	a_gb[i] = g_beg[g]; a_ge[i] = g_beg[g + 1];
+	a_g[i] = g;
+	if (i == 0 || (i32)(key[i - 1] >> gshift) != g) g_beg[g] = (i32)i;
+	if (i == n - 1) g_beg[g + 1] = (i32)n;
+	if constexpr (WIPE_LIST) {
+		if (i < mail[M_NTOUCH]) {
+			const i64 blk = tlist[i];
+			uint4 *p = (uint4 *)(bm + (blk << 5));
+#pragma unroll
+			for (int u = 0; u < 8; u++) p[u] = make_uint4(0u, 0u, 0u, 0u);
+			cb[blk >> 5] = 0;
+		}
+	} else { bm[pdk >> 5] = 0; cb[pdk >> 15] = 0; }
 }
 
 struct OpUniqBrk {
@@ -144,62 +147,68 @@
 	static constexpr int lb_id = 3;
 #endif
 	static constexpr bool clamped = true;
-	i64 na; const i32 *a_q; const i64 *a_r; const i32 *a_gb, *a_ge;
-	i32 *uniq, *brk, *alive, *cuEx, *brkEx, *blist;
-	struct Item { i32 gb, ge, q, qm, qp, u, b; i64 r, rm; };
+	i64 na; const i32 *a_q; const i64 *a_r; const i32 *a_g;
+	uint8_t *fl; i32 *cuEx, *brkEx, *blist, *g_cu;
+	struct Item { i32 g, gm, gp, q, qm, qp, u, b; i64 r, rm; };
 	__device__ Item load(i64 i) const
 	{
 		const i64 im = i > 0 ? i - 1 : 0, ip = i + 1 < na ? i + 1 : i;
-		Item it; it.gb = a_gb[i]; it.ge = a_ge[i]; it.q = a_q[i]; it.qm = a_q[im]; it.qp = a_q[ip]; it.r = a_r[i]; it.rm = a_r[im]; it.u = it.b = 0;
+		Item it; it.g = a_g[i]; it.gm = a_g[im]; it.gp = a_g[ip]; it.q = a_q[i]; it.qm = a_q[im]; it.qp = a_q[ip]; it.r = a_r[i]; it.rm = a_r[im]; it.u = it.b = 0;
 		return it;
 	}
 	__device__ void prep(Item &it, i64 i) const
 	{
-		const bool u = !(i > it.gb && it.qm == it.q) && !(i + 1 < it.ge && it.qp == it.q);
-		it.u = u ? 1 : 0; it.b = (u && i > it.gb && (it.r - it.q) != (it.rm - it.qm)) ? 1 : 0;
+		const bool head = i == 0 || it.gm != it.g, last = i + 1 >= na || it.gp != it.g;
+		const bool u = !(!head && it.qm == it.q) && !(!last && it.qp == it.q);
+		it.u = u ? 1 : 0; it.b = (u && !head && (it.r - it.q) != (it.rm - it.qm)) ? 1 : 0;
 	}
 	__device__ i32 value(const Item &it, i64, int c) const { return c == 0 ? it.u : it.b; }
-	__device__ void emit(const Item &, i64 i, const i32 *v, const i32 *ex) const
-	{
-		uniq[i] = v[0]; brk[i] = v[1]; alive[i] = 1; cuEx[i] = ex[0]; brkEx[i] = ex[1];
+	__device__ void emit(const Item &it, i64 i, const i32 *v, const i32 *ex) const
+	{
+		fl[i] = (uint8_t)(v[0] | (v[1] << 1)); cuEx[i] = ex[0]; brkEx[i] = ex[1];
+		if (i == 0 || it.gm != it.g) g_cu[it.g] = ex[0];
 		if (v[1]) blist[ex[1]] = (i32)i;
 	}
-	__device__ void done(const i32 *t) const { cuEx[na] = t[0]; brkEx[na] = t[1]; uniq[na] = 0; brk[na] = 0; }
-};
+	__device__ void done(const i32 *t) const { cuEx[na] = t[0]; brkEx[na] = t[1]; fl[na] = 0; g_cu[a_g[na - 1] + 1] = t[0]; }
+};
+#define FL_UNIQ 1
+#define FL_BRK 2
+#define FL_CAND 4
 
 struct OpCand {
 #ifdef LB_BISECT
 	static constexpr int lb_id = 4;
 #endif
 	static constexpr bool clamped = true;
-	i64 na; const i32 *a_gb, *a_ge, *cuEx, *brk;
-	i32 *candf, *candEx, *clist, *ws;
-	struct Item { i32 cand, head, gb, b, ce, cb; };
+	i64 na; const i32 *a_g, *g_cu; const uint8_t *fl;
+	uint8_t *cf; i32 *candEx, *clist; uint8_t *ws;
+	struct Item { i32 cand, head, g, gm, f, ce, cb; };
 	__device__ Item load(i64 i) const
 	{
-		Item it; it.gb = a_gb[i]; it.b = brk[i]; it.ce = cuEx[a_ge[i]]; it.cb = cuEx[it.gb]; it.cand = it.head = 0;
+		Item it; it.g = a_g[i]; it.gm = a_g[i > 0 ? i - 1 : 0]; it.f = fl[i]; it.ce = g_cu[it.g + 1]; it.cb = g_cu[it.g]; it.cand = it.head = 0;
 		return it;
 	}
-	__device__ void prep(Item &it, i64 i) const { it.head = i == it.gb ? 1 : 0; it.cand = (it.ce - it.cb >= GSA_WIN_SEEDS && (i == it.gb || it.b)) ? 1 : 0; }
+	__device__ void prep(Item &it, i64 i) const { it.head = (i == 0 || it.gm != it.g) ? 1 : 0; it.cand = (it.ce - it.cb >= GSA_WIN_SEEDS && (it.head || (it.f & FL_BRK))) ? 1 : 0; }
 	__device__ i32 value(const Item &it, i64, int) const { return it.cand; }
 	__device__ void emit(const Item &it, i64 i, const i32 *v, const i32 *ex) const
 	{
-		candf[i] = v[0]; candEx[i] = ex[0]; ws[i] = it.head;
+		cf[i] = (uint8_t)(it.f | (v[0] ? FL_CAND : 0)); candEx[i] = ex[0]; ws[i] = (uint8_t)it.head;
 		if (v[0]) clist[ex[0]] = (i32)i;
 	}
-	__device__ void done(const i32 *t) const { candEx[na] = t[0]; candf[na] = 0; ws[na] = 0; }
-};
-
-__global__ void k_next_window(i64 na, const i32 *__restrict__ a_q, const i32 *__restrict__ a_gb, const i32 *__restrict__ a_ge,
-                              const i32 *__restrict__ uniq, const i32 *__restrict__ cuEx, const i32 *__restrict__ brk, const i32 *__restrict__ brkEx,
-                              const i32 *__restrict__ blist, const i32 *__restrict__ candf, const i32 *__restrict__ candEx, const i32 *__restrict__ clist, i32 *next, i32 *nextk,
+	__device__ void done(const i32 *t) const { candEx[na] = t[0]; cf[na] = 0; ws[na] = 0; }
+};
+
+__global__ void k_next_window(i64 na, const i32 *__restrict__ a_q, const i32 *__restrict__ a_g, const i32 *__restrict__ g_beg,
+                              const uint8_t *__restrict__ cf, const i32 *__restrict__ cuEx, const i32 *__restrict__ brkEx,
+                              const i32 *__restrict__ blist, const i32 *__restrict__ candEx, const i32 *__restrict__ clist, i32 *next, i32 *nextk,
                               uint4 *tab_clear, i64 tab_cap)
 {
 	for (i64 j = (i64)blockIdx.x * blockDim.x + threadIdx.x; j < tab_cap; j += (i64)gridDim.x * blockDim.x) tab_clear[j] = make_uint4(~0u, ~0u, ~0u, ~0u);
 	GID(na);
-	if (!candf[i]) { next[i] = -1; return; }
-	const i32 gb = a_gb[i], ge = a_ge[i];
-	const i32 base = (i == gb) ? cuEx[gb] : cuEx[i] + uniq[i];
+	const i32 f = cf[i];
+	if (!(f & FL_CAND)) { next[i] = -1; return; }
+	const i32 g = a_g[i], gb = g_beg[g], ge = g_beg[g + 1];
+	const i32 base = (i == gb) ? cuEx[gb] : cuEx[i] + (f & FL_UNIQ);
 	i32 lo = (i32)i + 1, hi = ge;
 	while (lo < hi) { i32 mid = (lo + hi) >> 1; if (cuEx[mid + 1] - base >= GSA_WIN_SEEDS) hi = mid; else lo = mid + 1; }
 	const i32 j1 = lo;
@@ -217,7 +226,7 @@
 #define WALK_T 1024
 #define WALK_MAXTILES 8192
 #define WALK_LDS_CAND 20480
-__global__ void __launch_bounds__(WALK_T) k_walk_windows(i64 na, const i32 *__restrict__ candEx, const i32 *__restrict__ clist, const i32 *__restrict__ next, const i32 *__restrict__ nextk, i32 *ws)
+__global__ void __launch_bounds__(WALK_T) k_walk_windows(i64 na, const i32 *__restrict__ candEx, const i32 *__restrict__ clist, const i32 *__restrict__ next, const i32 *__restrict__ nextk, uint8_t *ws)
 {
 	__shared__ __attribute__((aligned(16))) i32 buf[2 * 2048 + 3 * WALK_LDS_CAND / 2 + 2 * WALK_LDS_CAND / 32];
 	static_assert(sizeof(buf) >= 2 * WALK_MAXTILES * sizeof(i32), "arena too small for the global-memory path");
@@ -322,10 +331,10 @@
 	static constexpr int lb_id = 5;
 #endif
 	static constexpr bool clamped = true;
-	i64 na; const i32 *a_q; const i64 *a_r; const i32 *uniq, *ws; i64 bmin; u32 cap;
+	i64 na; const i32 *a_q; const i64 *a_r; const uint8_t *fl, *ws; i64 bmin; u32 cap;
 	i32 *wsEx, *slot_of; Bucket *tab; unsigned long long *wbest, *wsum; i32 *wn;
 	struct Item { i32 ws, uniq; i64 pd; };
-	__device__ Item load(i64 i) const { Item it; it.ws = ws[i]; it.uniq = uniq[i]; it.pd = a_r[i] - a_q[i]; return it; }
+	__device__ Item load(i64 i) const { Item it; it.ws = ws[i]; it.uniq = fl[i] & FL_UNIQ; it.pd = a_r[i] - a_q[i]; return it; }
 	__device__ i32 value(const Item &it, i64, int) const { return it.ws; }
 	__device__ void emit(const Item &it, i64 i, const i32 *v, const i32 *ex) const
 	{
@@ -437,7 +446,7 @@
 }
 
 __global__ void k_window_avg(i64 na, const i32 *__restrict__ slot_of, const Bucket *__restrict__ tab, const i32 *__restrict__ a_q, const i64 *__restrict__ a_r,
-                             const unsigned long long *__restrict__ wbest, const i32 *__restrict__ ws, const i32 *__restrict__ wsEx, unsigned long long *wsum, i32 *wn, Bundle bnd)
+                             const unsigned long long *__restrict__ wbest, const uint8_t *__restrict__ ws, const i32 *__restrict__ wsEx, unsigned long long *wsum, i32 *wn, Bundle bnd)
 {
 	const i64 i = (i64)blockIdx.x * blockDim.x + threadIdx.x;
 	const int lane = threadIdx.x & 63;
@@ -463,12 +472,12 @@
 	static constexpr int lb_id = 6;
 #endif
 	static constexpr bool clamped = true;
-	i64 na; const i32 *uniq; i32 *alive, *auEx, *aulist;
+	i64 na; const uint8_t *fl; uint8_t *alive; i32 *auEx, *aulist;
 	const i32 *slot_of; const Bucket *tab; const i32 *a_q; const i64 *a_r; const unsigned long long *wbest, *wsum; const i32 *wn; i64 G; i32 max_indel; Bundle bnd;
 	struct Item { i32 alive, uniq, sl, q, wn, boff; u32 cnt; unsigned long long key, wbest, wsum; i64 r; };
 	__device__ Item load(i64 i) const
 	{
-		Item it; it.uniq = uniq[i]; it.alive = 1;
+		Item it; it.uniq = fl[i] & FL_UNIQ; it.alive = 1;
 		it.sl = slot_of[i]; it.q = a_q[i]; it.r = a_r[i];
 		const uint4 e = *(const uint4 *)&tab[it.sl < 0 ? 0 : it.sl];
 		it.key = ((unsigned long long)e.y << 32) | e.x; it.cnt = e.z;
@@ -487,7 +496,7 @@
 		if (d_llabs(avg - pd) > max_indel && cnt < 3) it.alive = 0;
 	}
 	__device__ i32 value(const Item &it, i64, int) const { return (it.uniq && it.alive) ? 1 : 0; }
-	__device__ void emit(const Item &it, i64 i, const i32 *v, const i32 *ex) const { alive[i] = it.alive; auEx[i] = ex[0]; if (v[0]) aulist[ex[0]] = (i32)i; }
+	__device__ void emit(const Item &it, i64 i, const i32 *v, const i32 *ex) const { alive[i] = (uint8_t)it.alive; auEx[i] = ex[0]; if (v[0]) aulist[ex[0]] = (i32)i; }
 	__device__ void done(const i32 *t) const { auEx[na] = t[0]; }
 };
 
@@ -512,20 +521,21 @@
 	static constexpr int lb_id = 7;
 #endif
 	static constexpr bool clamped = true;
-	const i32 *alive, *a_q, *a_len; const i64 *a_r; const i32 *a_gb, *a_ge, *auEx, *aulist; i64 G; i32 max_indel; Bundle bnd;
+	const uint8_t *alive; const i32 *a_q, *a_len; const i64 *a_r; const i32 *a_g, *g_beg, *auEx, *aulist; i64 G; i32 max_indel; Bundle bnd;
 	i32 *b_q, *b_len; i64 *b_r; i32 *b_g, *mail; i64 na;
-	struct Item { i32 alive, q, len, g, ge, qm, qp; i64 r; };
+	struct Item { i32 alive, q, len, g, gm, gp, qm, qp; i64 r; };
 	__device__ Item load(i64 i) const
 	{
 		const i64 im = i > 0 ? i - 1 : 0, ip = i + 1 < na ? i + 1 : i;
-		Item it; it.alive = alive[i]; it.q = a_q[i]; it.g = a_gb[i]; it.ge = a_ge[i]; it.len = a_len[i]; it.r = a_r[i]; it.qm = a_q[im]; it.qp = a_q[ip];
+		Item it; it.alive = alive[i]; it.q = a_q[i]; it.g = a_g[i]; it.gm = a_g[im]; it.gp = a_g[ip]; it.len = a_len[i]; it.r = a_r[i]; it.qm = a_q[im]; it.qp = a_q[ip];
 		return it;
 	}
 	__device__ void prep(Item &it, i64 i) const
 	{
 		it.alive = it.alive ? 1 : 0;
-		const bool multi = it.alive && ((i + 1 < it.ge && it.qp == it.q) || (i > it.g && it.qm == it.q));
-		if (multi && multihit_keep(i, a_q, a_r, it.g, it.ge, auEx, aulist, G, max_indel, bnd) != (i32)i) it.alive = 0;
+		const bool head = i == 0 || it.gm != it.g, last = i + 1 >= na || it.gp != it.g;
+		const bool multi = it.alive && ((!last && it.qp == it.q) || (!head && it.qm == it.q));
+		if (multi && multihit_keep(i, a_q, a_r, g_beg[it.g], g_beg[it.g + 1], auEx, aulist, G, max_indel, bnd) != (i32)i) it.alive = 0;
 	}
 	__device__ i32 value(const Item &it, i64, int) const { return it.alive; }
 	__device__ void emit(const Item &it, i64, const i32 *v, const i32 *ex) const
@@ -761,7 +771,7 @@
 #error "k_walk_chain keeps 4 x 32 KB of slice tables in LDS: gfx950 (160 KB of LDS per CU) only"
 #endif
 #define WC_T 1024
-__global__ void __launch_bounds__(WC_T) k_walk_chain(i64 na, const i32 *__restrict__ candEx, const i32 *__restrict__ clist, const i32 *__restrict__ nextk, i32 *ws,
+__global__ void __launch_bounds__(WC_T) k_walk_chain(i64 na, const i32 *__restrict__ candEx, const i32 *__restrict__ clist, const i32 *__restrict__ nextk, uint8_t *ws,
                                                      u32 *ticket, u32 ticket0, unsigned long long *entry_w, u32 epoch, i32 *err)
 {
 	__shared__ uint16_t h[WC_SL], E1[WC_SL], E2[WC_SL], E3[WC_SL];
@@ -856,7 +866,7 @@
 	const i64 na = n; c->n_a = na;
 	ENS(i64, d_i64a, n + 2); ENS(i32, d_flag2, n + 2); ENS(i32, d_scan2, n + 2); ENS(i32, d_flag, n + 1); ENS(i32, d_scan, n + 1);
 	const int gbits = ceil_log2_u64((u64)n + 1);
-	ENS(i32, a_q, na); ENS(i32, a_len, na); ENS(i64, a_r, na); ENS(i32, a_gb, na); ENS(i32, a_ge, na);
+	ENS(i32, a_q, na); ENS(i32, a_len, na); ENS(i64, a_r, na); ENS(i32, a_g, na);
 	if (c->pd_path && c->qbits + 7 + gbits <= 64) {
 		const i64 nw = c->pd_words;
 		const i64 nblk = (nw + 31) >> 5;
@@ -872,30 +882,34 @@
 		{}
 		LAUNCH(k_pd_keys, n, n, c->d_key_a.as<u64>(), c->d_val_a.as<u32>(), c->d_pdbm.as<u32>(), c->d_gpre.as<i32>(), c->prm.MaxIndelSize, c->qbits, c->d_key_c.as<u64>(), c->d_val_c.as<u32>());
 		RC(gsa_sort_pairs_u64_u32(c, c->d_key_c.as<u64>(), c->d_key_b.as<u64>(), c->d_val_c.as<u32>(), c->d_val_b.as<u32>(), (size_t)na, c->hits_sorted ? c->qbits + 7 : 0, c->qbits + 7 + gbits));
-		LAUNCH(k_pd_heads, n, n, c->d_key_b.as<u64>(), c->qbits + 7, c->g_beg.as<i32>());
-		LAUNCH(k_pd_gather, n, n, c->d_key_b.as<u64>(), c->d_val_b.as<u32>(), c->d_key_a.as<u64>(), c->d_val_a.as<u32>(), c->qbits + 7, c->qbits, c->bnd, c->g_beg.as<i32>(),
-		       c->a_q.as<i32>(), c->a_len.as<i32>(), c->a_r.as<i64>(), c->a_gb.as<i32>(), c->a_ge.as<i32>(), c->d_pdbm.as<u32>(), c->d_pdcb.as<u32>());
+		if (nblk > c->opt.pd_two_level_min)
+			LAUNCH(k_pd_gather<true>, n, n, c->d_key_b.as<u64>(), c->d_val_b.as<u32>(), c->d_key_a.as<u64>(), c->d_val_a.as<u32>(), c->qbits + 7, c->qbits, c->bnd, c->g_beg.as<i32>(),
+			       c->a_q.as<i32>(), c->a_len.as<i32>(), c->a_r.as<i64>(), c->a_g.as<i32>(), c->d_pdbm.as<u32>(), c->d_pdcb.as<u32>(), (const i32 *)c->d_flag.as<i32>(), (const i32 *)mail_);
+		else
+			LAUNCH(k_pd_gather<false>, n, n, c->d_key_b.as<u64>(), c->d_val_b.as<u32>(), c->d_key_a.as<u64>(), c->d_val_a.as<u32>(), c->qbits + 7, c->qbits, c->bnd, c->g_beg.as<i32>(),
+			       c->a_q.as<i32>(), c->a_len.as<i32>(), c->a_r.as<i64>(), c->a_g.as<i32>(), c->d_pdbm.as<u32>(), c->d_pdcb.as<u32>(), (const i32 *)nullptr, (const i32 *)mail_);
 		c->pdbm_dirty = false;
 	} else {
 		RC(seed_view_sort(c));
 		ENS(u64, d_key_a, n); ENS(u64, d_key_b, n); ENS(u32, d_val_a, n); ENS(u32, d_val_b, n);
 		LAUNCH(k_group_keys, n, n, c->s_q.as<i32>(), c->s_gid.as<i32>(), c->qbits, c->d_key_a.as<u64>(), c->d_val_a.as<u32>());
 		RC(gsa_sort_pairs_u64_u32(c, c->d_key_a.as<u64>(), c->d_key_b.as<u64>(), c->d_val_a.as<u32>(), c->d_val_b.as<u32>(), (size_t)na, 0, c->qbits + gbits));
-		LAUNCH(k_gather_active, na, na, c->d_val_b.as<u32>(), c->s_q.as<i32>(), c->s_len.as<i32>(), c->s_r.as<i64>(), c->s_gid.as<i32>(), c->g_beg.as<i32>(),
-		       c->a_q.as<i32>(), c->a_len.as<i32>(), c->a_r.as<i64>(), c->a_gb.as<i32>(), c->a_ge.as<i32>());
-	}
-	ENS(i32, a_uniq, na + 1); ENS(i32, a_cu, na + 1); ENS(i32, a_alive, na + 1); ENS(i32, a_brk, na + 1); ENS(i32, a_aurank, na + 1);
+		LAUNCH(k_gather_active, na, na, c->d_val_b.as<u32>(), c->s_q.as<i32>(), c->s_len.as<i32>(), c->s_r.as<i64>(), c->s_gid.as<i32>(),
+		       c->a_q.as<i32>(), c->a_len.as<i32>(), c->a_r.as<i64>(), c->a_g.as<i32>());
+	}
+	ENS(i32, a_uniq, na + 1); ENS(i32, a_cu, na + 1); ENS(i32, a_brk, na + 1); ENS(i32, a_aurank, na + 1);
+	ENS(uint8_t, a_fl, na + 1); ENS(uint8_t, a_cf, na + 1); ENS(uint8_t, a_ws8, na + 1); ENS(uint8_t, a_alive, na + 1); ENS(i32, g_cu, na + 2);
 	ENS(i32, a_aulist, na + 1); ENS(i32, a_next, na + 1); ENS(i32, a_ws, na + 1); ENS(i32, a_wid, na + 1); ENS(i32, a_runinfo, na + 1);
-	i32 *uniq = c->a_uniq.as<i32>(), *cuEx = c->a_cu.as<i32>(), *alive = c->a_alive.as<i32>(), *brk = c->a_brk.as<i32>();
-	i32 *brkEx = c->a_aurank.as<i32>(), *blist = c->a_aulist.as<i32>(), *next = c->a_next.as<i32>(), *ws = c->a_ws.as<i32>(), *wsEx = c->a_wid.as<i32>();
+	uint8_t *fl = c->a_fl.as<uint8_t>(), *cf = c->a_cf.as<uint8_t>(), *ws = c->a_ws8.as<uint8_t>(), *alive = c->a_alive.as<uint8_t>();
+	i32 *cuEx = c->a_cu.as<i32>(), *brkEx = c->a_aurank.as<i32>(), *blist = c->a_aulist.as<i32>(), *next = c->a_next.as<i32>(), *wsEx = c->a_wid.as<i32>();
 	i32 *mail = c->d_mail.as<i32>();
-	{ OpUniqBrk op = { na, c->a_q.as<i32>(), c->a_r.as<i64>(), c->a_gb.as<i32>(), c->a_ge.as<i32>(), uniq, brk, alive, cuEx, brkEx, blist }; RC((lb_launch<2>(c, na, op))); }
-	i32 *candf = c->d_flag.as<i32>(), *candEx = c->d_scan.as<i32>(), *clist = c->a_runinfo.as<i32>();
-	{ OpCand op = { na, c->a_gb.as<i32>(), c->a_ge.as<i32>(), cuEx, brk, candf, candEx, clist, ws }; RC((lb_launch<1>(c, na, op))); }
+	{ OpUniqBrk op = { na, c->a_q.as<i32>(), c->a_r.as<i64>(), c->a_g.as<i32>(), fl, cuEx, brkEx, blist, c->g_cu.as<i32>() }; RC((lb_launch<2>(c, na, op))); }
+	i32 *candEx = c->d_scan.as<i32>(), *clist = c->a_runinfo.as<i32>();
+	{ OpCand op = { na, c->a_g.as<i32>(), c->g_cu.as<i32>(), fl, cf, candEx, clist, ws }; RC((lb_launch<1>(c, na, op))); }
 	const i64 cap = na + na / 4 + 1024;
 	ENS(Bucket, d_btab, cap);
 	static_assert(sizeof(Bucket) == 16, "the table is cleared as uint4s");
-	LAUNCH(k_next_window, na, na, c->a_q.as<i32>(), c->a_gb.as<i32>(), c->a_ge.as<i32>(), uniq, cuEx, brk, brkEx, blist, candf, candEx, clist, next, c->d_flag2.as<i32>(), c->d_btab.as<uint4>(), cap);
+	LAUNCH(k_next_window, na, na, c->a_q.as<i32>(), c->a_g.as<i32>(), c->g_beg.as<i32>(), cf, cuEx, brkEx, blist, candEx, clist, next, c->d_flag2.as<i32>(), c->d_btab.as<uint4>(), cap);
 	if (na <= c->opt.walk_chain_min) hipLaunchKernelGGL(k_walk_windows, dim3(1), dim3(WALK_T), 0, st, na, candEx, clist, next, c->d_flag2.as<i32>(), ws);
 	else {
 		const u32 grid = (u32)((na + WC_SL - 1) / WC_SL);
@@ -910,16 +924,16 @@
 	ENS(unsigned long long, w_best, na + 1); ENS(unsigned long long, w_sum, na + 1); ENS(i32, w_n, na + 1);
 	const i64 bmin = ((-(i64)c->qlen) >> 4) - 1;
 	i32 *slot_of = c->a_runinfo.as<i32>();
-	{ OpWindowBuckets op = { na, c->a_q.as<i32>(), c->a_r.as<i64>(), uniq, ws, bmin, (u32)cap, wsEx, slot_of, c->d_btab.as<Bucket>(),
+	{ OpWindowBuckets op = { na, c->a_q.as<i32>(), c->a_r.as<i64>(), fl, ws, bmin, (u32)cap, wsEx, slot_of, c->d_btab.as<Bucket>(),
 	                         c->w_best.as<unsigned long long>(), c->w_sum.as<unsigned long long>(), c->w_n.as<i32>() }; RC((lb_launch<1, 4>(c, na, op))); }
 	LAUNCH(k_window_mode, cap, cap, c->d_btab.as<Bucket>(), c->w_best.as<unsigned long long>());
 	LAUNCH(k_window_avg, na, na, slot_of, c->d_btab.as<Bucket>(), c->a_q.as<i32>(), c->a_r.as<i64>(), c->w_best.as<unsigned long long>(), ws, wsEx,
 	       c->w_sum.as<unsigned long long>(), c->w_n.as<i32>(), c->bnd);
 	i32 *auEx = c->a_aurank.as<i32>(), *aulist = c->a_aulist.as<i32>();
-	{ OpAliveUnique op = { na, uniq, alive, auEx, aulist, slot_of, c->d_btab.as<Bucket>(), c->a_q.as<i32>(), c->a_r.as<i64>(),
+	{ OpAliveUnique op = { na, fl, alive, auEx, aulist, slot_of, c->d_btab.as<Bucket>(), c->a_q.as<i32>(), c->a_r.as<i64>(),
 	                       c->w_best.as<unsigned long long>(), c->w_sum.as<unsigned long long>(), c->w_n.as<i32>(), c->G, c->prm.MaxIndelSize, c->bnd }; RC((lb_launch<1>(c, na, op))); }
 	ENS(i32, b_q, na); ENS(i32, b_len, na); ENS(i64, b_r, na); ENS(i32, b_gb, na);
-	{ OpCompactAlive op = { alive, c->a_q.as<i32>(), c->a_len.as<i32>(), c->a_r.as<i64>(), c->a_gb.as<i32>(), c->a_ge.as<i32>(), auEx, aulist, c->G, c->prm.MaxIndelSize, c->bnd,
+	{ OpCompactAlive op = { alive, c->a_q.as<i32>(), c->a_len.as<i32>(), c->a_r.as<i64>(), c->a_g.as<i32>(), c->g_beg.as<i32>(), auEx, aulist, c->G, c->prm.MaxIndelSize, c->bnd,
 	                        c->b_q.as<i32>(), c->b_len.as<i32>(), c->b_r.as<i64>(), c->b_gb.as<i32>(), mail, na }; RC((lb_launch<1>(c, na, op))); }
 	ENS(i32, c_q, na); ENS(i32, c_len, na + 1); ENS(i64, c_r, na); ENS(i32, c_gb, na); ENS(i32, c_bid, na);
 	{ OpNoise op = { c->b_q.as<i32>(), c->b_len.as<i32>(), c->b_r.as<i64>(), c->b_gb.as<i32>(),
```

Result: slower. 33.15 Gbp/s (-1.6%).
